# 2025-comprehensive-design/AudioLDM-with-LoRA

Hardware: AMD Instinct MI355X
Metric: unet_denoise_steps_per_sec (higher is better)
Workload: dtype bf16; 1 GPU; audioldm-s-full-v2 UNet + rank-4 LoRA (q,k,v,out), DDIM 200-step schedule, batch 4 x 10 s clips (latent 250x16), CFG 2.5 (UNet batch 8), bf16; per_gpu_batch=4, parallelism=prompt-sharded x1, hip_graph=True, graph_chains=1

## Files before the change

### audioldm_with_lora_amd/_lib.py

```python
import ctypes as C
import os

_HERE = os.path.dirname(os.path.abspath(__file__))
LIB_PATH = os.environ.get("ALDM_LIB") or os.path.join(_HERE, "libaldm_hip.so")

ACT_NONE, ACT_SILU, ACT_LRELU, ACT_TANH, ACT_GELU = 0, 1, 2, 3, 4
OUT_BF16, OUT_F32 = 0, 1
TILE_AUTO, TILE_128x128, TILE_64x64, TILE_128x64, TILE_64x128 = 0, 1, 2, 3, 4


class IgemmArgs(C.Structure):
    _fields_ = [
        ("x", C.c_void_p), ("x2", C.c_void_p),
        ("B", C.c_int), ("IH", C.c_int), ("IW", C.c_int), ("Cin", C.c_int), ("Cin2", C.c_int),
        ("UH", C.c_int), ("UW", C.c_int),
        ("in_dilate", C.c_int),
        ("w", C.c_void_p),
        ("Kpad", C.c_int),
        ("KH", C.c_int), ("KW", C.c_int), ("stride_h", C.c_int), ("stride_w", C.c_int),
        ("pad_h", C.c_int), ("pad_w", C.c_int), ("dil_h", C.c_int), ("dil_w", C.c_int),
        ("OH", C.c_int), ("OW", C.c_int), ("Cout", C.c_int),
        ("in_act", C.c_int), ("in_slope", C.c_float),
        ("ln_s", C.c_void_p), ("ln_sa", C.c_void_p), ("ln_ca", C.c_void_p), ("ln_eps", C.c_float),
        ("lora_a", C.c_void_p), ("lora_b", C.c_void_p),
        ("Rp", C.c_int),
        ("lora_t_out", C.c_void_p),
        ("bias", C.c_void_p), ("rowbias", C.c_void_p),
        ("rowbias_ld", C.c_int),
        ("geglu", C.c_int),
        ("out_act", C.c_int), ("out_slope", C.c_float),
        ("res", C.c_void_p), ("res2", C.c_void_p),
        ("alpha", C.c_float),
        ("post_act", C.c_int), ("post_slope", C.c_float), ("out2", C.c_void_p),
        ("out", C.c_void_p), ("out_dtype", C.c_int), ("out_ld", C.c_int),
        ("out_batch_stride", C.c_longlong),
        ("out_pix_stride", C.c_int), ("out_pix_offset", C.c_int),
        ("vt", C.c_void_p), ("vt_col0", C.c_int), ("vt_ld", C.c_int), ("vt_batch_stride", C.c_longlong),
        ("splits", C.c_int), ("workspace", C.c_void_p),
        ("tile", C.c_int),
        ("ring", C.c_int),
        ("defer_reduce", C.c_int),
        ("rowstat_out", C.c_void_p), ("ln_parts", C.c_void_p), ("ln_nparts", C.c_int),
        ("qstat_out", C.c_void_p),
        ("x3", C.c_void_p), ("x4", C.c_void_p), ("Cin3", C.c_int), ("Cin4", C.c_int),
        ("vt_dual", C.c_int),
        ("gnin_gamma", C.c_void_p), ("gnin_beta", C.c_void_p), ("gnin_q1", C.c_void_p), ("gnin_q2", C.c_void_p),
        ("gnin_bm1", C.c_int), ("gnin_tpi1", C.c_int), ("gnin_bm2", C.c_int), ("gnin_tpi2", C.c_int),
        ("gnin_groups", C.c_int), ("gnin_act", C.c_int), ("gnin_eps", C.c_float),
        ("xcd_map", C.c_int),
        ("lora_gate", C.c_void_p), ("gate_rows", C.c_int),
    ]


class PgemmArgs(C.Structure):
    _fields_ = [
        ("x", C.c_void_p), ("w", C.c_void_p),
        ("M", C.c_int), ("N", C.c_int), ("K", C.c_int),
        ("bias", C.c_void_p),
        ("ln_s", C.c_void_p), ("ln_sa", C.c_void_p), ("ln_ca", C.c_void_p), ("ln_eps", C.c_float),
        ("ln_parts", C.c_void_p), ("ln_nparts", C.c_int),
        ("lora_a", C.c_void_p), ("lora_b", C.c_void_p),
        ("Rp", C.c_int), ("ranks_used", C.c_int),
        ("geglu", C.c_int),
        ("res", C.c_void_p),
        ("out", C.c_void_p), ("out_ld", C.c_int),
        ("vt", C.c_void_p), ("vt_col0", C.c_int), ("vt_ld", C.c_int), ("vt_batch_stride", C.c_longlong), ("OHW", C.c_int),
        ("rowstat_out", C.c_void_p),
        ("mi", C.c_int), ("nt", C.c_int), ("tiles_per_range", C.c_int),
        ("max_ranges", C.c_int),
        ("waves", C.c_int),
        ("lora_t_out", C.c_void_p),
        ("vt_dual", C.c_int),
        ("lora_gate", C.c_void_p), ("gate_rows", C.c_int),
    ]


PROTOTYPES = {
    "aldm_version": (C.c_char_p, []),
    "aldm_last_error": (C.c_char_p, []),
    "aldm_igemm": (C.c_int, [C.POINTER(IgemmArgs), C.c_void_p]),
    "aldm_igemm_workspace_bytes": (C.c_size_t, [C.POINTER(IgemmArgs)]),
    "aldm_igemm_effective_splits": (C.c_int, [C.POINTER(IgemmArgs)]),
    "aldm_pgemm_supported": (C.c_int, [C.c_int]),
    "aldm_pgemm_plan": (C.c_int, [C.POINTER(PgemmArgs)]),
    "aldm_pgemm": (C.c_int, [C.POINTER(PgemmArgs), C.c_void_p]),
    "aldm_groupnorm_partials": (C.c_int, [C.c_void_p, C.c_int, C.c_int, C.c_int, C.c_int, C.c_void_p, C.c_void_p, C.c_int,
                                          C.c_void_p, C.c_void_p, C.c_void_p, C.c_int, C.c_int, C.c_float, C.c_void_p,
                                          C.c_void_p, C.c_int, C.c_void_p, C.c_void_p]),
    "aldm_groupnorm": (C.c_int, [C.c_void_p, C.c_void_p, C.c_int, C.c_int, C.c_int, C.c_int, C.c_int, C.c_float,
                                 C.c_void_p, C.c_void_p, C.c_int, C.c_void_p, C.c_void_p]),
    "aldm_groupnorm_apply": (C.c_int, [C.c_void_p, C.c_void_p, C.c_int, C.c_int, C.c_void_p, C.c_void_p, C.c_int, C.c_int, C.c_int,
                                       C.c_int, C.c_int, C.c_int, C.c_int, C.c_float, C.c_void_p, C.c_void_p, C.c_int, C.c_void_p,
                                       C.c_void_p, C.c_void_p]),
    "aldm_gn_silu_conv3x3_small": (C.c_int, [C.c_void_p, C.c_void_p, C.c_int, C.c_int, C.c_int, C.c_int, C.c_int, C.c_int, C.c_int, C.c_float,
                                             C.c_void_p, C.c_void_p, C.c_void_p, C.c_int, C.c_void_p, C.c_int, C.c_void_p, C.c_void_p]),
    "aldm_layernorm": (C.c_int, [C.c_void_p, C.c_int, C.c_int, C.c_void_p, C.c_void_p, C.c_float, C.c_void_p,
                                 C.c_void_p]),
    "aldm_attention": (C.c_int, [C.c_void_p, C.c_int, C.c_void_p, C.c_int, C.c_void_p, C.c_int, C.c_longlong,
                                 C.c_int, C.c_int, C.c_int, C.c_int, C.c_float, C.c_void_p, C.c_int, C.c_void_p]),
    "aldm_attention_prescaled": (C.c_int, [C.c_void_p, C.c_int, C.c_void_p, C.c_int, C.c_void_p, C.c_int, C.c_longlong,
                                           C.c_int, C.c_int, C.c_int, C.c_int, C.c_void_p, C.c_int, C.c_void_p]),
    "aldm_attn_block64": (C.c_int, [C.c_void_p, C.c_void_p, C.c_int, C.c_void_p, C.c_int, C.c_void_p, C.c_void_p, C.c_void_p, C.c_void_p,
                                    C.c_int, C.c_int, C.c_void_p, C.c_void_p, C.c_float, C.c_int, C.c_int, C.c_int, C.c_int, C.c_void_p,
                                    C.c_void_p]),
    "aldm_attn_block64_fp8": (C.c_int, [C.c_void_p, C.c_void_p, C.c_int, C.c_void_p, C.c_int, C.c_void_p, C.c_void_p, C.c_void_p, C.c_void_p,
                                    C.c_int, C.c_int, C.c_void_p, C.c_void_p, C.c_float, C.c_int, C.c_int, C.c_int, C.c_int, C.c_void_p,
                                    C.c_void_p]),
    "aldm_attn_block64_gated": (C.c_int, [C.c_void_p, C.c_void_p, C.c_int, C.c_void_p, C.c_int, C.c_void_p, C.c_void_p, C.c_void_p, C.c_void_p,
                                     C.c_int, C.c_int, C.c_void_p, C.c_void_p, C.c_float, C.c_int, C.c_int, C.c_int, C.c_int, C.c_void_p,
                                     C.c_void_p, C.c_void_p]),
    "aldm_attn_block64_fp8_gated": (C.c_int, [C.c_void_p, C.c_void_p, C.c_int, C.c_void_p, C.c_int, C.c_void_p, C.c_void_p, C.c_void_p, C.c_void_p,
                                     C.c_int, C.c_int, C.c_void_p, C.c_void_p, C.c_float, C.c_int, C.c_int, C.c_int, C.c_int, C.c_void_p,
                                     C.c_void_p, C.c_void_p]),
    "aldm_attn_block256_gated": (C.c_int, [C.c_void_p, C.c_void_p, C.c_int, C.c_void_p, C.c_int, C.c_void_p, C.c_void_p, C.c_void_p, C.c_void_p,
                                     C.c_int, C.c_int, C.c_void_p, C.c_void_p, C.c_float, C.c_int, C.c_int, C.c_int, C.c_int, C.c_void_p,
                                     C.c_void_p, C.c_void_p]),
    "aldm_attn_block256": (C.c_int, [C.c_void_p, C.c_void_p, C.c_int, C.c_void_p, C.c_int, C.c_void_p, C.c_void_p, C.c_void_p, C.c_void_p,
                                     C.c_int, C.c_int, C.c_void_p, C.c_void_p, C.c_float, C.c_int, C.c_int, C.c_int, C.c_int, C.c_void_p,
                                     C.c_void_p]),
    "aldm_hifigan_respair_supported": (C.c_int, [C.c_int, C.c_int, C.c_int]),
    "aldm_hifigan_respair": (C.c_int, [C.c_void_p, C.c_int, C.c_int, C.c_int, C.c_void_p, C.c_int, C.c_void_p, C.c_int, C.c_void_p, C.c_int,
                                       C.c_void_p, C.c_int, C.c_float, C.c_float, C.c_void_p, C.c_int, C.c_float, C.c_void_p, C.c_void_p]),
    "aldm_conv1d_to1": (C.c_int, [C.c_void_p, C.c_int, C.c_int, C.c_int, C.c_void_p, C.c_void_p, C.c_int, C.c_int, C.c_void_p, C.c_void_p]),
    "aldm_attention_wide": (C.c_int, [C.c_void_p, C.c_int, C.c_void_p, C.c_int, C.c_void_p, C.c_int, C.c_longlong,
                                      C.c_int, C.c_int, C.c_int, C.c_void_p, C.c_int, C.c_void_p]),
    "aldm_attention_fp8": (C.c_int, [C.c_void_p, C.c_int, C.c_void_p, C.c_int, C.c_void_p, C.c_int, C.c_longlong,
                                     C.c_int, C.c_int, C.c_int, C.c_int, C.c_float, C.c_void_p, C.c_int, C.c_void_p]),
    "aldm_attention_varlen": (C.c_int, [C.c_void_p, C.c_int, C.c_void_p, C.c_int, C.c_void_p, C.c_int, C.c_longlong,
                                        C.c_int, C.c_int, C.c_int, C.c_int, C.c_float, C.c_void_p, C.c_void_p, C.c_int,
                                        C.c_void_p]),
    "aldm_embed_layernorm": (C.c_int, [C.c_void_p, C.c_int, C.c_int, C.c_int, C.c_void_p, C.c_int, C.c_void_p, C.c_int,
                                       C.c_void_p, C.c_void_p, C.c_void_p, C.c_float, C.c_int, C.c_void_p, C.c_void_p]),
    "aldm_attention_lse": (C.c_int, [C.c_void_p, C.c_int, C.c_void_p, C.c_int, C.c_void_p, C.c_int, C.c_longlong,
                                     C.c_int, C.c_int, C.c_int, C.c_int, C.c_float, C.c_void_p, C.c_int, C.c_void_p,
                                     C.c_void_p]),
    "aldm_attention_bwd": (C.c_int, [C.c_void_p, C.c_void_p, C.c_void_p, C.c_int, C.c_void_p, C.c_void_p, C.c_void_p,
                                     C.c_int, C.c_longlong, C.c_longlong, C.c_longlong, C.c_void_p, C.c_void_p, C.c_int,
                                     C.c_void_p, C.c_void_p, C.c_int, C.c_int, C.c_int, C.c_int, C.c_float, C.c_void_p,
                                     C.c_void_p, C.c_void_p, C.c_int, C.c_void_p]),
    "aldm_groupnorm_bwd": (C.c_int, [C.c_void_p, C.c_void_p, C.c_void_p, C.c_int, C.c_int, C.c_int, C.c_int, C.c_int,
                                     C.c_float, C.c_void_p, C.c_void_p, C.c_int, C.c_void_p, C.c_void_p, C.c_void_p, C.c_void_p,
                                     C.c_void_p]),
    "aldm_groupnorm_bwd_partials": (C.c_int, [C.c_void_p, C.c_void_p, C.c_void_p, C.c_int, C.c_int, C.c_int, C.c_int, C.c_int,
                                              C.c_int, C.c_float, C.c_void_p, C.c_void_p, C.c_int, C.c_void_p, C.c_void_p,
                                              C.c_void_p, C.c_void_p, C.c_void_p]),
    "aldm_layernorm_bwd": (C.c_int, [C.c_void_p, C.c_void_p, C.c_int, C.c_int, C.c_void_p, C.c_float, C.c_void_p, C.c_void_p,
                                     C.c_void_p]),
    "aldm_geglu_fwd": (C.c_int, [C.c_void_p, C.c_longlong, C.c_int, C.c_void_p, C.c_void_p]),
    "aldm_geglu_bwd": (C.c_int, [C.c_void_p, C.c_void_p, C.c_longlong, C.c_int, C.c_void_p, C.c_void_p]),
    "aldm_add_bf16": (C.c_int, [C.c_void_p, C.c_void_p, C.c_longlong, C.c_void_p, C.c_void_p]),
    "aldm_upsample_nearest_bwd": (C.c_int, [C.c_void_p, C.c_int, C.c_int, C.c_int, C.c_int, C.c_int, C.c_int, C.c_void_p,
                                            C.c_void_p]),
    "aldm_tn_small": (C.c_int, [C.c_void_p, C.c_int, C.c_void_p, C.c_int, C.c_int, C.c_int, C.c_void_p, C.c_void_p]),
    "aldm_tn_batched": (C.c_int, [C.c_void_p, C.c_int, C.c_int, C.c_int, C.c_void_p]),
    "aldm_lora_pack": (C.c_int, [C.c_void_p, C.c_int, C.c_void_p]),
    "aldm_transpose_tokens": (C.c_int, [C.c_void_p, C.c_int, C.c_int, C.c_int, C.c_int, C.c_int, C.c_void_p, C.c_void_p]),
    "aldm_mse_grad": (C.c_int, [C.c_void_p, C.c_void_p, C.c_longlong, C.c_float, C.c_void_p, C.c_void_p, C.c_void_p]),
    "aldm_softmax_rows": (C.c_int, [C.c_void_p, C.c_int, C.c_int, C.c_int, C.c_float, C.c_void_p, C.c_int,
                                    C.c_void_p]),
    "aldm_timestep_embedding": (C.c_int, [C.c_void_p, C.c_int, C.c_int, C.c_int, C.c_void_p, C.c_void_p]),
    "aldm_silu": (C.c_int, [C.c_void_p, C.c_longlong, C.c_void_p, C.c_void_p]),
    "aldm_nchw_f32_to_nhwc": (C.c_int, [C.c_void_p, C.c_int, C.c_int, C.c_int, C.c_void_p, C.c_int, C.c_void_p]),
    "aldm_nhwc_to_nchw_f32": (C.c_int, [C.c_void_p, C.c_int, C.c_int, C.c_int, C.c_int, C.c_void_p, C.c_void_p]),
    "aldm_f32_to_bf16": (C.c_int, [C.c_void_p, C.c_longlong, C.c_float, C.c_void_p, C.c_void_p]),
    "aldm_cfg_ddim_step": (C.c_int, [C.c_void_p, C.c_void_p, C.c_int, C.c_longlong, C.c_int, C.c_float,
                                     C.c_void_p, C.c_void_p, C.c_void_p, C.c_void_p]),
    "aldm_ddim_step_fused": (C.c_int, [C.c_void_p, C.c_void_p, C.c_int, C.c_longlong, C.c_int, C.c_float, C.c_void_p, C.c_void_p, C.c_void_p,
                                       C.c_void_p, C.c_longlong, C.c_void_p, C.c_void_p, C.c_int, C.c_void_p, C.c_void_p, C.c_void_p]),
    "aldm_dpm_step_fused": (C.c_int, [C.c_void_p, C.c_void_p, C.c_int, C.c_longlong, C.c_int, C.c_float, C.c_void_p, C.c_void_p, C.c_void_p,
                                      C.c_void_p, C.c_void_p, C.c_longlong, C.c_void_p, C.c_void_p, C.c_int, C.c_void_p, C.c_void_p,
                                      C.c_void_p]),
# ... 67 lines not shown
```

### audioldm_with_lora_amd/csrc/igemm.hip

```cpp
#include "igemm_core.h"

using namespace aldm_igemm_detail;

int aldm_launch_tile_128x128(const IgemmDev& d, int Rp, bool vt, int ring, hipStream_t st);
int aldm_launch_tile_128x64(const IgemmDev& d, int Rp, bool vt, int ring, hipStream_t st);
int aldm_launch_tile_64x128(const IgemmDev& d, int Rp, bool vt, int ring, hipStream_t st);
int aldm_launch_tile_64x64(const IgemmDev& d, int Rp, bool vt, int ring, hipStream_t st);
int aldm_launch_tile_128x128w8(const IgemmDev& d, int Rp, bool vt, int ring, hipStream_t st);
int aldm_launch_tile_256x128w8(const IgemmDev& d, int Rp, bool vt, int ring, hipStream_t st);
int aldm_launch_tile_256x128ws(const IgemmDev& d, int Rp, bool vt, int ring, hipStream_t st);
int aldm_launch_tile_64x128ws(const IgemmDev& d, int Rp, bool vt, int ring, hipStream_t st);
int aldm_launch_tile_128x64ws(const IgemmDev& d, int Rp, bool vt, int ring, hipStream_t st);
int aldm_launch_tile_64x128w8(const IgemmDev& d, int Rp, bool vt, int ring, hipStream_t st);
int aldm_launch_tile_128x64w8(const IgemmDev& d, int Rp, bool vt, int ring, hipStream_t st);
int aldm_launch_halo(const IgemmDev& d, int tile, int ring, hipStream_t st);

static int pick_tile(int M, int N) {
  auto tiles = [&](int bm, int bn) { return (long long)cdiv(M, bm) * cdiv(N, bn); };
  if (N <= 64) return M >= 4096 ? ALDM_TILE_128x64 : ALDM_TILE_64x64;
  if (tiles(128, 128) >= 224) return ALDM_TILE_128x128;
  if (tiles(128, 64) >= 224) return ALDM_TILE_128x64;
  return ALDM_TILE_64x64;
}


extern "C" size_t aldm_igemm_workspace_bytes(const aldm_igemm_t* p) {
  if (!p || p->splits <= 1) return 0;
  const long long M = (long long)p->B * p->OH * p->OW;
  return (size_t)p->splits * M * p->Cout * sizeof(float);
}

extern "C" int aldm_igemm_effective_splits(const aldm_igemm_t* p) {
  if (!p || p->splits <= 1) return 1;
  const int nkt = cdiv(p->KH * p->KW * (p->Cin + p->Cin2), BK) + (p->x3 ? (p->Cin3 + (p->x4 ? p->Cin4 : 0)) / BK : 0);
  if (p->tile == ALDM_TILE_HALO_128x128 || p->tile == ALDM_TILE_HALO_64x128 || p->tile == ALDM_TILE_HALO_128x128_WS ||
      p->tile == ALDM_TILE_HALO_64x128_WS) {
    const int nch = (p->Cin + p->Cin2) / BK;
    return cdiv(nch, cdiv(nch, p->splits > nch ? nch : p->splits));
  }
  int splits = p->splits > nkt ? nkt : p->splits;
  const int per = cdiv(nkt, splits);
  return cdiv(nkt, per);
}

extern "C" int aldm_igemm(const aldm_igemm_t* p, void* stream) {
  ALDM_CHECK_ARG(p && p->x && p->w && p->out, "igemm: null x/w/out");
  ALDM_CHECK_ARG(p->B > 0 && p->IH > 0 && p->IW > 0 && p->OH > 0 && p->OW > 0 && p->Cout > 0, "igemm: bad dims");
  ALDM_CHECK_ARG(p->Cin > 0 && p->Cin % 8 == 0 && p->Cin2 >= 0 && p->Cin2 % 8 == 0, "igemm: Cin/Cin2 must be multiples of 8 (got %d,%d)", p->Cin, p->Cin2);
  ALDM_CHECK_ARG(p->Cin2 == 0 || p->x2, "igemm: Cin2 without x2");
  ALDM_CHECK_ARG(p->KH > 0 && p->KW > 0, "igemm: bad filter");
  const int Ctot = p->Cin + p->Cin2;
  const int Ktot = p->KH * p->KW * Ctot;
  const int Cext = p->x3 ? p->Cin3 + (p->x4 ? p->Cin4 : 0) : 0;
  ALDM_CHECK_ARG(p->Kpad % BK == 0 && p->Kpad >= Ktot + Cext, "igemm: Kpad %d must be a multiple of 64 and >= %d", p->Kpad, Ktot + Cext);
  ALDM_CHECK_ARG(!p->x3 || (p->Cin3 > 0 && p->Cin3 % 64 == 0 && (!p->x4 || (p->Cin4 > 0 && p->Cin4 % 64 == 0)) && Ktot % 64 == 0 &&
                            p->Cin % 64 == 0 && p->Cin2 % 64 == 0 && p->in_act == ALDM_ACT_NONE && !p->ln_s && !p->vt && !p->geglu &&
                            p->in_dilate == 0 && p->Rp == 0),
                 "igemm: the fused 1x1 second-source segment (x3 | x4) needs the plain LDS-DMA path: every channel count and KH*KW*(Cin+Cin2) a multiple of 64");
  ALDM_CHECK_ARG(p->x3 || !p->x4, "igemm: x4 without x3");
  ALDM_CHECK_ARG(!p->vt_dual || (p->vt && !p->res && !p->res2 && !p->out2 && p->out_act == ALDM_ACT_NONE && p->post_act == ALDM_ACT_NONE &&
                                 p->alpha == 1.f && !p->rowbias && p->out_dtype == ALDM_OUT_BF16),
                 "igemm: vt_dual needs vt and the plain bf16 epilogue (bias only)");
  ALDM_CHECK_ARG(p->Rp == 0 || p->Rp == 32 || p->Rp == 64, "igemm: Rp must be 0/32/64");
  ALDM_CHECK_ARG(p->Rp == 0 || (p->lora_a && p->lora_b), "igemm: Rp without lora_a/lora_b");
  ALDM_CHECK_ARG(!p->lora_gate || p->Rp, "igemm: lora_gate without an adapter");
  ALDM_CHECK_ARG(!p->lora_gate || p->Rp == 32, "igemm: lora_gate needs Rp == 32 (the gate table's width; got %d)", p->Rp);
  ALDM_CHECK_ARG(!p->lora_gate || !p->lora_t_out, "igemm: lora_t_out (the trainer's copy of T) is not combined with lora_gate");
  ALDM_CHECK_ARG(!p->lora_gate || (p->gate_rows > 0 && (p->B * p->OH * p->OW) % p->gate_rows == 0),
                 "igemm: lora_gate needs gate_rows > 0 dividing M (got %d rows per sample, M %d)", p->gate_rows, p->B * p->OH * p->OW);
  ALDM_CHECK_ARG(!p->geglu || (p->Cout % 32 == 0 && !p->rowbias), "igemm: GEGLU needs Cout %% 32 == 0");
  ALDM_CHECK_ARG(!p->vt || (p->vt_col0 % 16 == 0 && p->splits <= 1 && !p->geglu), "igemm: bad vt config");
  ALDM_CHECK_ARG(!p->vt || p->vt_col0 > 0 || p->out, "igemm: out required");
  ALDM_CHECK_ARG(p->splits <= 1 || (p->workspace && p->Cout % 4 == 0), "igemm: split-K needs workspace and Cout %% 4 == 0");
  ALDM_CHECK_ARG(p->out_ld > 0, "igemm: out_ld");
  ALDM_CHECK_ARG(!p->defer_reduce || (!p->geglu && !p->res2 && !p->out2 && p->out_act == ALDM_ACT_NONE && p->post_act == ALDM_ACT_NONE && p->alpha == 1.f),
                 "igemm: defer_reduce leaves bias / row bias / res to the consumer and supports nothing else in the epilogue");
  ALDM_CHECK_ARG(!(p->geglu && p->out2) || (p->Rp == 0 && p->splits <= 1 && !p->res && !p->res2 && p->out_dtype == ALDM_OUT_BF16 &&
                                            p->out_act == ALDM_ACT_NONE && p->post_act == ALDM_ACT_NONE && p->alpha == 1.f &&
                                            p->in_act == ALDM_ACT_NONE && p->Cin % 64 == 0 && p->Cin2 % 64 == 0 && p->Cout % 32 == 0),
                 "igemm: GEGLU with out2 (pre-activation copy) needs the plain LDS-DMA GEGLU launch (no residual / activation / split-K)");
  ALDM_CHECK_ARG(!p->ln_s || (p->KH == 1 && p->KW == 1 && p->Cin2 == 0 && p->splits <= 1 && (p->Rp == 0 || (p->ln_sa && p->ln_ca))),
                 "igemm: folded LayerNorm needs a 1x1 single-source GEMM without split-K (and ln_sa/ln_ca with LoRA)");
  ALDM_CHECK_ARG(!p->rowstat_out || (!p->vt && p->splits <= 1 && !p->geglu && p->out_dtype == ALDM_OUT_BF16 && p->Cout % 64 == 0 && !p->out2),
                 "igemm: rowstat_out needs the standard bf16 epilogue (no V^T / split-K / GEGLU / out2) and Cout %% 64 == 0");
  ALDM_CHECK_ARG(!p->qstat_out || (!p->vt && p->splits <= 1 && !p->geglu && p->out_dtype == ALDM_OUT_BF16 && p->Cout % 8 == 0 &&
                                   p->out_pix_stride <= 1 && p->Rp == 0 && !p->ln_s && !p->rowstat_out),
                 "igemm: qstat_out needs the standard bf16 epilogue (no V^T / split-K / GEGLU / LoRA / LayerNorm hand-over) and Cout %% 8 == 0");
  ALDM_CHECK_ARG(!p->ln_parts || (p->ln_s && p->ln_nparts > 0 && p->ln_nparts <= 64), "igemm: ln_parts needs ln_s and 1..64 partials per row");
  ALDM_CHECK_ARG(p->ring == 0 || (p->ring >= 2 && p->ring <= 4), "igemm: ring must be 0 (auto) or 2..4");
  ALDM_CHECK_ARG(p->in_dilate == 0 || (p->in_dilate == 2 && p->UH == 0), "igemm: in_dilate must be 0 or 2 (and excludes UH/UW)");

  IgemmDev d;
  d.x = (const bf16*)p->x; d.x2 = (const bf16*)p->x2; d.w = (const bf16*)p->w;
  d.lora_a = (const bf16*)p->lora_a; d.lora_b = (const bf16*)p->lora_b; d.lora_t_out = (bf16*)p->lora_t_out;
  d.bias = p->bias; d.rowbias = p->rowbias; d.res = (const bf16*)p->res; d.res2 = (const bf16*)p->res2;
  d.out = p->out; d.vt = (bf16*)p->vt; d.ws = p->workspace;
  d.B = p->B; d.IH = p->IH; d.IW = p->IW; d.Cin = p->Cin; d.Cin2 = p->Cin2; d.Ctot = Ctot; d.UH = p->UH; d.UW = p->UW; d.dilate = p->in_dilate;
  d.KH = p->KH; d.KW = p->KW; d.sh = p->stride_h; d.sw = p->stride_w; d.ph = p->pad_h; d.pw = p->pad_w;
  d.dh = p->dil_h; d.dw = p->dil_w;
  d.OH = p->OH; d.OW = p->OW; d.OHW = p->OH * p->OW; d.N = p->Cout; d.M = p->B * p->OH * p->OW; d.Kpad = p->Kpad;
  d.in_act = p->in_act; d.in_slope = p->in_slope;
  d.rowbias_ld = p->rowbias_ld; d.geglu = p->geglu; d.out_act = p->out_act; d.out_slope = p->out_slope;
  d.alpha = p->alpha;
  d.post_act = p->post_act; d.post_slope = p->post_slope; d.out2 = (bf16*)p->out2;
  d.out_f32 = p->out_dtype == ALDM_OUT_F32; d.out_ld = p->out_ld;
  d.out_bs = p->out_batch_stride; d.out_ps = p->out_pix_stride > 0 ? p->out_pix_stride : 1; d.out_po = p->out_pix_offset;
  d.vt_col0 = p->vt_col0; d.vt_ld = p->vt_ld; d.vt_bs = p->vt_batch_stride; d.vt_dual = p->vt ? p->vt_dual : 0;
  d.x3 = (const bf16*)p->x3; d.x4 = (const bf16*)p->x4; d.Cin3 = p->x3 ? p->Cin3 : 0; d.Cin4 = (p->x3 && p->x4) ? p->Cin4 : 0;
  d.C3tot = d.Cin3 + d.Cin4;
  d.nkt = cdiv(Ktot, BK) + d.C3tot / BK;
  d.splits = p->splits > 1 ? p->splits : 1;
  if (d.splits > d.nkt) d.splits = d.nkt;
  d.kt_per_split = cdiv(d.nkt, d.splits);
  d.splits = cdiv(d.nkt, d.kt_per_split);
  d.ws_rows = d.M;
  d.lora_gate = p->lora_gate; d.fd_gate = make_fastdiv((unsigned)(p->lora_gate ? p->gate_rows : 1)); d.gate_m1 = d.M - 1;
  d.tiles_n = 0; d.tiles_m = 0; d.nwg = 0;
  ALDM_CHECK_ARG(p->xcd_map >= 0 && p->xcd_map <= 2, "igemm: xcd_map must be 0 (auto), 1 (activation-stationary) or 2 (weight-stationary)");
  {
    const unsigned long long act = 2ull * p->B * p->IH * p->IW * Ctot + 2ull * p->B * p->OH * p->OW * Cext;
    const unsigned long long wgt = 2ull * p->Cout * p->Kpad;
    d.xmap = p->xcd_map ? p->xcd_map - 1 : ((wgt > act && p->splits <= 1) ? 1 : 0);
  }
  {
    const unsigned long long xb = 2ull * p->B * p->IH * p->IW * p->Cin, x2b = 2ull * p->B * p->IH * p->IW * p->Cin2;
    const unsigned long long wb = 2ull * p->Cout * p->Kpad, lb = 2ull * p->Rp * p->Kpad;
    ALDM_CHECK_ARG(wb < 0xFFFFFFFFull, "igemm: weight matrix too large for 32-bit offsets");
    const unsigned long long x3b = 2ull * p->B * p->OH * p->OW * d.Cin3, x4b = 2ull * p->B * p->OH * p->OW * d.Cin4;
    ALDM_CHECK_ARG(x3b < 0x80000000ull && x4b < 0x80000000ull, "igemm: x3 / x4 too large for 32-bit offsets");
    d.x3_bytes = (unsigned)x3b; d.x4_bytes = (unsigned)x4b;
    d.x_bytes = xb < 0xFFFFFFFFull ? (unsigned)xb : 0xFFFFFFFFu;
    d.x2_bytes = x2b < 0xFFFFFFFFull ? (unsigned)x2b : 0xFFFFFFFFu;
    d.w_bytes = (unsigned)wb;
    d.la_bytes = (unsigned)lb;
    d.lb_bytes = (unsigned)(2ull * p->Cout * p->Rp);
    d.fd_ohw = make_fastdiv((unsigned)d.OHW); d.fd_ow = make_fastdiv((unsigned)d.OW); d.fd_halo = make_fastdiv((unsigned)d.OW + 2u);
    d.fd_ctot = make_fastdiv((unsigned)d.Ctot); d.fd_kw = make_fastdiv((unsigned)d.KW);
    d.ln_s = p->ln_s; d.ln_sa = p->ln_sa; d.ln_ca = p->ln_ca; d.ln_eps = p->ln_eps;
    d.rowstat = p->rowstat_out; d.ln_parts = p->ln_parts; d.ln_np = p->ln_nparts;
    d.qstat = p->qstat_out; d.qtile = -1;
    d.gi_gamma = p->gnin_gamma; d.gi_beta = p->gnin_beta; d.gi_q1 = p->gnin_q1; d.gi_q2 = p->gnin_q2;
    d.gi_bm1 = p->gnin_bm1; d.gi_tpi1 = p->gnin_tpi1; d.gi_bm2 = p->gnin_bm2; d.gi_tpi2 = p->gnin_tpi2;
    d.gi_groups = p->gnin_groups; d.gi_act = p->gnin_act; d.gi_eps = p->gnin_eps;
#ifdef ALDM_DIAG
    d.diag = (p->splits <= 1) ? (unsigned long long*)p->workspace : nullptr;
#else
    d.diag = nullptr;
#endif
  }
  hipStream_t st = (hipStream_t)stream;

  int tile = p->tile ? p->tile : pick_tile(d.M, d.N);
  if (p->gnin_gamma) {
    ALDM_CHECK_ARG(tile == ALDM_TILE_HALO_128x128 || tile == ALDM_TILE_HALO_64x128 || tile == ALDM_TILE_HALO_128x128_WS || tile == ALDM_TILE_HALO_64x128_WS, "igemm: gnin_* (GroupNorm of the input inside the launch) needs a halo tile");
    const int Ct = p->Cin + p->Cin2;
    ALDM_CHECK_ARG(p->gnin_beta && p->gnin_q1 && (p->Cin2 == 0 || p->gnin_q2) && p->gnin_groups > 0 && p->gnin_groups <= 64 && Ct % p->gnin_groups == 0 &&
                   (Ct / p->gnin_groups) % 4 == 0 && Ct <= 512 && p->UH == 0 &&
                   (p->gnin_tpi1 > 0 || (p->gnin_bm1 > 0 && p->gnin_bm1 <= p->IH * p->IW)) &&
                   (p->Cin2 == 0 || p->gnin_tpi2 > 0 || (p->gnin_bm2 > 0 && p->gnin_bm2 <= p->IH * p->IW)) &&
                   (p->gnin_act == ALDM_ACT_NONE || p->gnin_act == ALDM_ACT_SILU),
                   "igemm: gnin_*: tables for every source, group width a multiple of 4, at most 512 input channels, no up-sampling, act NONE / SILU");
  }
  const bool vt = p->vt != nullptr;
  int rc;
  switch (tile) {
    case ALDM_TILE_128x128: rc = aldm_launch_tile_128x128(d, p->Rp, vt, p->ring, st); break;
    case ALDM_TILE_128x64: rc = aldm_launch_tile_128x64(d, p->Rp, vt, p->ring, st); break;
    case ALDM_TILE_64x128: rc = aldm_launch_tile_64x128(d, p->Rp, vt, p->ring, st); break;
    case ALDM_TILE_64x64: rc = aldm_launch_tile_64x64(d, p->Rp, vt, p->ring, st); break;
    case ALDM_TILE_128x128_W8: rc = aldm_launch_tile_128x128w8(d, p->Rp, vt, p->ring, st); break;
    case ALDM_TILE_256x128_W8: rc = aldm_launch_tile_256x128w8(d, p->Rp, vt, p->ring, st); break;
    case ALDM_TILE_256x128_WS: rc = aldm_launch_tile_256x128ws(d, p->Rp, vt, p->ring, st); break;
    case ALDM_TILE_64x128_WS: rc = aldm_launch_tile_64x128ws(d, p->Rp, vt, p->ring, st); break;
    case ALDM_TILE_128x64_WS: rc = aldm_launch_tile_128x64ws(d, p->Rp, vt, p->ring, st); break;
    case ALDM_TILE_64x128_W8: rc = aldm_launch_tile_64x128w8(d, p->Rp, vt, p->ring, st); break;
    case ALDM_TILE_128x64_W8: rc = aldm_launch_tile_128x64w8(d, p->Rp, vt, p->ring, st); break;
    case ALDM_TILE_HALO_128x128:
    case ALDM_TILE_HALO_64x128:
    case ALDM_TILE_HALO_128x128_WS:
    case ALDM_TILE_HALO_64x128_WS:
      if (p->Rp || vt || p->rowstat_out || (p->x3 && tile != ALDM_TILE_HALO_128x128_WS && tile != ALDM_TILE_HALO_64x128_WS)) {
        aldm_set_error("igemm: the halo tiles take no LoRA / V^T / row statistics (and a second-source segment only in the wave-specialised forms)");
        return ALDM_E_UNSUPPORTED;
      }
      if (d.splits > 1) {
        const int nch = (d.Cin + d.Cin2) / BK;
        const int cps = cdiv(nch, d.splits > nch ? nch : d.splits);
        d.kt_per_split = d.KH * d.KW * cps;
        d.splits = cdiv(nch, cps);
      }
      rc = aldm_launch_halo(d, tile, p->ring, st);
      break;
    default: aldm_set_error("igemm: unknown tile %d", tile); return ALDM_E_UNSUPPORTED;
  }
  if (rc != ALDM_OK) return rc;
  if (d.splits > 1 && !p->defer_reduce) {
    const int ncols = d.geglu ? d.N / 2 : d.N;
    const long long work = (long long)d.M * (ncols / 4);
    hipLaunchKernelGGL(igemm_reduce_kernel, dim3((unsigned)cdivll(work, 256)), dim3(256), 0, st, d);
    return aldm_launch_status("igemm_reduce");
  }
  return ALDM_OK;
}
```

### audioldm_with_lora_amd/csrc/igemm_core.h

```cpp
#pragma once
#include <type_traits>

#include "common.h"

namespace aldm_igemm_detail {

constexpr int BK = 64;
constexpr int THREADS = 256;

struct FastDiv { unsigned mul, shift; };
__device__ __forceinline__ int fdiv(int n, FastDiv d) {
  return (int)(((unsigned long long)__umulhi((unsigned)n, d.mul) + (unsigned)n) >> d.shift);
}
static inline FastDiv make_fastdiv(unsigned d) {
  FastDiv f;
  unsigned s = 0;
  while ((1ull << s) < d) ++s;
  f.shift = s;
  f.mul = (unsigned)((((1ull << s) - d) << 32) / d + 1);
  return f;
}

struct IgemmDev {
  const bf16* x; const bf16* x2; const bf16* w; const bf16* lora_a; const bf16* lora_b;
  bf16* lora_t_out;
  const float* bias; const float* rowbias; const bf16* res; const bf16* res2;
  void* out; bf16* vt; float* ws;
  int B, IH, IW, Cin, Cin2, Ctot, UH, UW, dilate;
  int KH, KW, sh, sw, ph, pw, dh, dw;
  int OH, OW, OHW, N, M, Kpad;
  int in_act; float in_slope;
  int rowbias_ld, geglu, out_act; float out_slope; float alpha;
  int post_act; float post_slope; bf16* out2;
  int out_f32, out_ld; long long out_bs; int out_ps, out_po;
  int vt_col0, vt_ld; long long vt_bs; int vt_dual;
  int splits, kt_per_split, nkt;
  int tiles_n;
  int tiles_m, nwg, xmap;
  FastDiv fd_tiles_m, fd_splits;
  unsigned x_bytes, x2_bytes, w_bytes, la_bytes, lb_bytes;
  unsigned long long* diag;
  FastDiv fd_ohw, fd_ow, fd_halo;
  FastDiv fd_tiles_n, fd_ctot, fd_kw;
  const float* ln_s; const float* ln_sa; const float* ln_ca; float ln_eps;
  const bf16* x3; const bf16* x4; int Cin3, Cin4, C3tot; unsigned x3_bytes, x4_bytes;
  float* qstat; int qtile;
  float* rowstat;
  const float* ln_parts; int ln_np;
  const float* gi_gamma; const float* gi_beta; const float* gi_q1; const float* gi_q2;
  int gi_bm1, gi_tpi1, gi_bm2, gi_tpi2, gi_groups, gi_act; float gi_eps;
  int ws_rows;
  const float* lora_gate;
  FastDiv fd_gate;
  int gate_m1;
};

__device__ __forceinline__ int swz(int row, int chunk) { return chunk ^ ((row >> 1) & 7); }

__device__ __forceinline__ void igemm_work_item(const IgemmDev& p, int& tile_m, int& tile_n, int& split) {
  const int nwg = p.nwg, bid = blockIdx.x;
  const int xcd = bid & 7, q = nwg >> 3, r = nwg & 7;
  const int w = (xcd < r ? xcd * (q + 1) : r * (q + 1) + (xcd - r) * q) + (bid >> 3);
  if (p.xmap) {
    const int sn = fdiv(w, p.fd_tiles_m);
    tile_m = w - sn * p.tiles_m;
    split = fdiv(sn, p.fd_tiles_n);
    tile_n = sn - split * p.tiles_n;
  } else {
    const int t = fdiv(w, p.fd_splits);
    split = w - t * p.splits;
    tile_m = fdiv(t, p.fd_tiles_n);
    tile_n = t - tile_m * p.tiles_n;
  }
}

__device__ __forceinline__ void igemm_gate4(const IgemmDev& p, f32x4& t, int m, int col, int rp) {
  const int mm = m < p.gate_m1 ? m : p.gate_m1;
  const f32x4 g = *reinterpret_cast<const f32x4*>(p.lora_gate + (long long)fdiv(mm, p.fd_gate) * rp + col);
#pragma unroll
  for (int e = 0; e < 4; ++e) t[e] *= g[e];
}

__device__ __forceinline__ void finish_store4(const IgemmDev& p, int m, int n, int ncols, float* v) {
  const int b = m / p.OHW;
  const int pix = m - b * p.OHW;
  const long long row = (long long)b * p.out_bs + (long long)(pix * p.out_ps + p.out_po) * p.out_ld;
  const bool vec = (n + 3 < ncols) && ((p.out_ld & 3) == 0) && ((p.out_bs & 3) == 0);
#pragma unroll
  for (int j = 0; j < 4; ++j) v[j] = apply_act(v[j], p.out_act, p.out_slope);
  if (p.res) {
    if (vec) {
      bf16x4 r = *reinterpret_cast<const bf16x4*>(p.res + row + n);
#pragma unroll
      for (int j = 0; j < 4; ++j) v[j] += (float)r[j];
    } else {
      for (int j = 0; j < 4; ++j) if (n + j < ncols) v[j] += (float)p.res[row + n + j];
    }
  }
#pragma unroll
  for (int j = 0; j < 4; ++j) v[j] *= p.alpha;
  if (p.res2) {
    if (vec) {
      bf16x4 r = *reinterpret_cast<const bf16x4*>(p.res2 + row + n);
#pragma unroll
      for (int j = 0; j < 4; ++j) v[j] += (float)r[j];
    } else {
      for (int j = 0; j < 4; ++j) if (n + j < ncols) v[j] += (float)p.res2[row + n + j];
    }
  }
  if (p.out2) {
    bf16* o2 = p.out2 + row + n;
    if (vec) {
      *reinterpret_cast<bf16x4*>(o2) = bf16x4{(bf16)apply_act(v[0], p.post_act, p.post_slope), (bf16)apply_act(v[1], p.post_act, p.post_slope),
                                              (bf16)apply_act(v[2], p.post_act, p.post_slope), (bf16)apply_act(v[3], p.post_act, p.post_slope)};
    } else {
      for (int j = 0; j < 4; ++j) if (n + j < ncols) o2[j] = (bf16)apply_act(v[j], p.post_act, p.post_slope);
    }
  } else if (p.post_act) {
#pragma unroll
    for (int j = 0; j < 4; ++j) v[j] = apply_act(v[j], p.post_act, p.post_slope);
  }
  if (p.out_f32) {
    float* o = reinterpret_cast<float*>(p.out) + row + n;
    if (vec) {
      *reinterpret_cast<f32x4*>(o) = f32x4{v[0], v[1], v[2], v[3]};
    } else {
      for (int j = 0; j < 4; ++j) if (n + j < ncols) o[j] = v[j];
    }
  } else {
    bf16* o = reinterpret_cast<bf16*>(p.out) + row + n;
    if (vec) {
      *reinterpret_cast<bf16x4*>(o) = bf16x4{(bf16)v[0], (bf16)v[1], (bf16)v[2], (bf16)v[3]};
    } else {
      for (int j = 0; j < 4; ++j) if (n + j < ncols) o[j] = (bf16)v[j];
    }
  }
}

// ... 19 lines not shown

__device__ __forceinline__ void epi8(const IgemmDev& p, int m, int n, int ncols, float* v) {
  const int b = fdiv(m, p.fd_ohw);
  const int pix = m - b * p.OHW;
  const long long row = (long long)b * p.out_bs + (long long)(pix * p.out_ps + p.out_po) * p.out_ld;
  const bool vec = (n + 7 < ncols) && ((p.out_ld & 7) == 0) && ((p.out_bs & 7) == 0);
  if (p.out_act) {
#pragma unroll
    for (int j = 0; j < 8; ++j) v[j] = apply_act(v[j], p.out_act, p.out_slope);
  }
  if (p.res) {
    if (vec) {
      const bf16x8 r = *reinterpret_cast<const bf16x8*>(p.res + row + n);
#pragma unroll
      for (int j = 0; j < 8; ++j) v[j] += (float)r[j];
    } else {
      for (int j = 0; j < 8; ++j) if (n + j < ncols) v[j] += (float)p.res[row + n + j];
    }
  }
#pragma unroll
  for (int j = 0; j < 8; ++j) v[j] *= p.alpha;
  if (p.res2) {
    if (vec) {
      const bf16x8 r = *reinterpret_cast<const bf16x8*>(p.res2 + row + n);
#pragma unroll
      for (int j = 0; j < 8; ++j) v[j] += (float)r[j];
    } else {
      for (int j = 0; j < 8; ++j) if (n + j < ncols) v[j] += (float)p.res2[row + n + j];
    }
  }
  if (p.out2) {
    bf16* o2 = p.out2 + row + n;
    if (vec) {
      bf16x8 t;
#pragma unroll
      for (int j = 0; j < 8; ++j) t[j] = (bf16)apply_act(v[j], p.post_act, p.post_slope);
      *reinterpret_cast<bf16x8*>(o2) = t;
    } else {
      for (int j = 0; j < 8; ++j) if (n + j < ncols) o2[j] = (bf16)apply_act(v[j], p.post_act, p.post_slope);
    }
  } else if (p.post_act) {
#pragma unroll
    for (int j = 0; j < 8; ++j) v[j] = apply_act(v[j], p.post_act, p.post_slope);
  }
  if (p.out_f32) {
    float* o = reinterpret_cast<float*>(p.out) + row + n;
    if (vec) {
      *reinterpret_cast<f32x4*>(o) = f32x4{v[0], v[1], v[2], v[3]};
      *reinterpret_cast<f32x4*>(o + 4) = f32x4{v[4], v[5], v[6], v[7]};
    } else {
      for (int j = 0; j < 8; ++j) if (n + j < ncols) o[j] = v[j];
    }
  } else {
    bf16* o = reinterpret_cast<bf16*>(p.out) + row + n;
    if (vec) {
      bf16x8 t;
#pragma unroll
      for (int j = 0; j < 8; ++j) t[j] = (bf16)v[j];
      *reinterpret_cast<bf16x8*>(o) = t;
    } else {
      for (int j = 0; j < 8; ++j) if (n + j < ncols) o[j] = (bf16)v[j];
    }
  }
}

template <int BM, int BN>
struct EpiCfg {
  static constexpr int LD = BN + 4;
  static constexpr int LDT = BM + 4;
  static constexpr int BYTES = (BM * LD > BN * LDT ? BM * LD : BN * LDT) * 4;
};

template <int BM, int BN, int MI, int NI, bool VT, int NT = 256, int EPI = 0>
__device__ __forceinline__ void igemm_epilogue(const IgemmDev& p, f32x4 (&acc)[MI][NI], char* smem, bool vt_wg, int m0,
                                               int n0, int wm_off, int wn_off, int lrow, int lq, int split, int tid,
                                               const float* lnst = nullptr) {
  using E = EpiCfg<BM, BN>;
  constexpr bool LEAN = EPI == 1 || EPI == 4, GLEAN = EPI == 2, SLEAN = EPI == 3;
  constexpr bool QS = EPI == 0 || EPI == 4;
#ifndef ALDM_NO_KA_PREFETCH
  aldm_prefetch_next_kernargs<sizeof(IgemmDev)>(tid);
#endif
  if constexpr (SLEAN) {
#pragma unroll
    for (int i = 0; i < MI; ++i) {
      const int m = m0 + wm_off + i * 16 + lrow;
#pragma unroll
      for (int j = 0; j < NI; ++j) {
        const int n = n0 + wn_off + j * 16 + lq * 4;
        if (m < p.M && n < p.N) *reinterpret_cast<f32x4*>(p.ws + ((long long)split * p.ws_rows + m) * p.N + n) = acc[i][j];
      }
    }
    return;
  }
  float* Cs = reinterpret_cast<float*>(smem);
  if constexpr (LEAN && !VT) lnst = nullptr;

  constexpr int GPR = BN / 8, RSTEP = NT / GPR, ITERS = BM / RSTEP, CH = ITERS < 4 ? ITERS : 4;
  static_assert(NT % GPR == 0 && BM % RSTEP == 0 && ITERS % CH == 0, "epilogue row walk");
  const int r0 = tid / GPR, c = (tid % GPR) * 8, n = n0 + c;
  const bool dual = VT && vt_wg && p.vt_dual;
  const bool std_path = !GLEAN && !SLEAN && (!(VT && vt_wg) || dual) && (LEAN || (p.splits <= 1 && !p.geglu));
  const bool vec = (n + 7 < p.N) && ((p.out_ld & 7) == 0) && ((p.out_bs & 7) == 0);
  const bool rbvec = vec && ((p.rowbias_ld & 3) == 0);
  float colb[8], lns[8];
  long long rowo[CH];
  bool ok[CH];
  f32x4 rb0[CH], rb1[CH];
  bf16x8 r1[CH], r2[CH];
  int slot[CH];
  float qacc[2][2][2] = {{{0.f, 0.f}, {0.f, 0.f}}, {{0.f, 0.f}, {0.f, 0.f}}};
  const int qb0 = (QS && p.qstat) ? fdiv(min(m0, p.M - 1), p.fd_ohw) : 0;
  auto phaseA = [&](int it0) {
#pragma unroll
    for (int u = 0; u < CH; ++u) {
      const int m = m0 + r0 + (it0 + u) * RSTEP;
      ok[u] = m < p.M;
      rb0[u] = rb1[u] = f32x4{0.f, 0.f, 0.f, 0.f};
      r1[u] = r2[u] = bf16x8{0, 0, 0, 0, 0, 0, 0, 0};
      rowo[u] = 0;
      slot[u] = 0;
      if (!ok[u]) continue;
      const int b = fdiv(m, p.fd_ohw);
      const int pix = m - b * p.OHW;
      slot[u] = b != qb0;
      rowo[u] = (long long)b * p.out_bs + (long long)(pix * p.out_ps + p.out_po) * p.out_ld;
      if (p.rowbias) {
        const float* rb = p.rowbias + (long long)b * p.rowbias_ld + n;
        if (rbvec) {
          rb0[u] = *reinterpret_cast<const f32x4*>(rb);
          rb1[u] = *reinterpret_cast<const f32x4*>(rb + 4);
        } else {
#pragma unroll
          for (int q = 0; q < 4; ++q) {
            if (n + q < p.N) rb0[u][q] = rb[q];
            if (n + 4 + q < p.N) rb1[u][q] = rb[4 + q];
          }
        }
      }
      if (vec) {
        if (p.res) r1[u] = *reinterpret_cast<const bf16x8*>(p.res + rowo[u] + n);
        if (p.res2) r2[u] = *reinterpret_cast<const bf16x8*>(p.res2 + rowo[u] + n);
      } else {
#pragma unroll
        for (int q = 0; q < 8; ++q) {
          if (p.res && n + q < p.N) r1[u][q] = p.res[rowo[u] + n + q];
          if (p.res2 && n + q < p.N) r2[u][q] = p.res2[rowo[u] + n + q];
        }
      }
    }
  };
  auto phaseB = [&](auto ACT, int it0) {
    constexpr bool kAct = decltype(ACT)::value;
#pragma unroll
    for (int u = 0; u < CH; ++u) {
      if (!ok[u]) continue;
      const int r = r0 + (it0 + u) * RSTEP;
      float v[8];
      if (VT && vt_wg) {
#pragma unroll
        for (int q = 0; q < 8; ++q) v[q] = Cs[(c + q) * E::LDT + r];
      } else {
        const float* src = Cs + r * E::LD + c;
#pragma unroll
        for (int q = 0; q < 8; ++q) v[q] = src[q];
      }
      if (lnst) {
        const float mu = lnst[r], rs = lnst[BM + r];
#pragma unroll
        for (int q = 0; q < 8; ++q) v[q] = rs * (v[q] - mu * lns[q]);
      }
#pragma unroll
      for (int q = 0; q < 4; ++q) { v[q] += colb[q] + rb0[u][q]; v[4 + q] += colb[4 + q] + rb1[u][q]; }
// ... 68 lines not shown
  if (std_path && n < p.N) {
#pragma unroll
    for (int q = 0; q < 8; ++q) colb[q] = lns[q] = 0.f;
    if (n + 7 < p.N) {
      if (p.bias) {
        const f32x4 b0 = *reinterpret_cast<const f32x4*>(p.bias + n), b1 = *reinterpret_cast<const f32x4*>(p.bias + n + 4);
#pragma unroll
        for (int q = 0; q < 4; ++q) { colb[q] = b0[q]; colb[4 + q] = b1[q]; }
      }
      if (lnst) {
        const f32x4 s0 = *reinterpret_cast<const f32x4*>(p.ln_s + n), s1 = *reinterpret_cast<const f32x4*>(p.ln_s + n + 4);
#pragma unroll
        for (int q = 0; q < 4; ++q) { lns[q] = s0[q]; lns[4 + q] = s1[q]; }
      }
    } else {
      for (int q = 0; q < 8; ++q) {
        if (p.bias && n + q < p.N) colb[q] = p.bias[n + q];
        if (lnst && n + q < p.N) lns[q] = p.ln_s[n + q];
      }
    }
    phaseA(0);
  }

  __syncthreads();
  if (VT && vt_wg) {
#pragma unroll
    for (int i = 0; i < MI; ++i)
#pragma unroll
      for (int j = 0; j < NI; ++j)
        *reinterpret_cast<f32x4*>(Cs + (wn_off + j * 16 + lrow) * E::LDT + wm_off + i * 16 + lq * 4) = acc[i][j];
  } else {
#pragma unroll
    for (int i = 0; i < MI; ++i)
#pragma unroll
      for (int j = 0; j < NI; ++j)
        *reinterpret_cast<f32x4*>(Cs + (wm_off + i * 16 + lrow) * E::LD + wn_off + j * 16 + lq * 4) = acc[i][j];
  }
  __syncthreads();

  if (VT && vt_wg) {
    for (int g = tid; g < BN * (BM / 8); g += NT) {
      const int rn = g / (BM / 8), cm = (g - rn * (BM / 8)) * 8;
      const int n = n0 + rn, m = m0 + cm;
      if (n >= p.N || m >= p.M) continue;
      const float bb = p.bias ? p.bias[n] : 0.f;
      const float lsn = lnst ? p.ln_s[n] : 0.f;
      const float* src = Cs + rn * E::LDT + cm;
      const int b = fdiv(m, p.fd_ohw), pix = m - b * p.OHW;
      bf16* o = p.vt + (long long)b * p.vt_bs + (long long)(n - p.vt_col0) * p.vt_ld + pix;
      if (m + 7 < p.M && pix + 7 < p.OHW && ((p.vt_ld & 7) == 0) && ((pix & 7) == 0) && ((p.vt_bs & 7) == 0)) {
        bf16x8 t;
        float mu8[8], rs8[8];
        if (lnst) {
          const f32x4 m0v = *reinterpret_cast<const f32x4*>(lnst + cm), m1v = *reinterpret_cast<const f32x4*>(lnst + cm + 4);
          const f32x4 r0v = *reinterpret_cast<const f32x4*>(lnst + BM + cm), r1v = *reinterpret_cast<const f32x4*>(lnst + BM + cm + 4);
#pragma unroll
          for (int q = 0; q < 4; ++q) { mu8[q] = m0v[q]; mu8[4 + q] = m1v[q]; rs8[q] = r0v[q]; rs8[4 + q] = r1v[q]; }
        } else {
#pragma unroll
          for (int q = 0; q < 8; ++q) { mu8[q] = 0.f; rs8[q] = 1.f; }
        }
#pragma unroll
        for (int q = 0; q < 8; ++q) t[q] = (bf16)(rs8[q] * (src[q] - mu8[q] * lsn) + bb);
        *reinterpret_cast<bf16x8*>(o) = t;
      } else {
        for (int q = 0; q < 8; ++q) {
          const int mq = m + q;
          if (mq >= p.M) break;
          const int bq = fdiv(mq, p.fd_ohw), pq = mq - bq * p.OHW;
          float val = src[q];
          if (lnst) val = lnst[BM + cm + q] * (val - lnst[cm + q] * lsn);
          p.vt[(long long)bq * p.vt_bs + (long long)(n - p.vt_col0) * p.vt_ld + pq] = (bf16)(val + bb);
        }
      }
    }
    if (!dual) return;
  }
  if constexpr (!LEAN) {
  if (!GLEAN && (SLEAN || p.splits > 1)) {
    for (int g = tid; g < BM * (BN / 8); g += NT) {
      const int r = g / (BN / 8), c = (g - r * (BN / 8)) * 8;
      const int m = m0 + r, n = n0 + c;
      if (m >= p.M || n >= p.N) continue;
      float* o = p.ws + ((long long)split * p.ws_rows + m) * p.N + n;
      const float* src = Cs + r * E::LD + c;
      if (n + 7 < p.N) {
        *reinterpret_cast<f32x4*>(o) = *reinterpret_cast<const f32x4*>(src);
        *reinterpret_cast<f32x4*>(o + 4) = *reinterpret_cast<const f32x4*>(src + 4);
      } else {
        for (int q = 0; q < 8; ++q) if (n + q < p.N) o[q] = src[q];
      }
    }
    return;
  }
  if (!SLEAN && (GLEAN || p.geglu)) {
    constexpr int CG = BN / 16, RS = NT / CG;
    static_assert(NT % CG == 0 && BM % RS == 0, "GEGLU row walk");
    const int jo = (tid % CG) * 8;
    const int cv = ((jo >> 4) << 5) + (jo & 15);
    const int nv = n0 + cv;
    if (nv >= p.N) return;
    float bv[8], bg[8], sv[8], sg[8];
#pragma unroll
    for (int q = 0; q < 8; ++q) bv[q] = bg[q] = sv[q] = sg[q] = 0.f;
    if (p.bias) {
      const f32x4 a0 = *reinterpret_cast<const f32x4*>(p.bias + nv), a1 = *reinterpret_cast<const f32x4*>(p.bias + nv + 4);
      const f32x4 g0 = *reinterpret_cast<const f32x4*>(p.bias + nv + 16), g1 = *reinterpret_cast<const f32x4*>(p.bias + nv + 20);
#pragma unroll
      for (int q = 0; q < 4; ++q) { bv[q] = a0[q]; bv[4 + q] = a1[q]; bg[q] = g0[q]; bg[4 + q] = g1[q]; }
    }
    if (lnst) {
      const f32x4 a0 = *reinterpret_cast<const f32x4*>(p.ln_s + nv), a1 = *reinterpret_cast<const f32x4*>(p.ln_s + nv + 4);
      const f32x4 g0 = *reinterpret_cast<const f32x4*>(p.ln_s + nv + 16), g1 = *reinterpret_cast<const f32x4*>(p.ln_s + nv + 20);
#pragma unroll
      for (int q = 0; q < 4; ++q) { sv[q] = a0[q]; sv[4 + q] = a1[q]; sg[q] = g0[q]; sg[4 + q] = g1[q]; }
    }
    for (int r = tid / CG; r < BM; r += RS) {
      const int m = m0 + r;
      if (m >= p.M) break;
      const float* src = Cs + r * E::LD + cv;
      const float mu = lnst ? lnst[r] : 0.f, rs = lnst ? lnst[BM + r] : 1.f;
      float val[8], gate[8], v[8];
#pragma unroll
      for (int q = 0; q < 8; ++q) {
        val[q] = rs * (src[q] - mu * sv[q]) + bv[q];
        gate[q] = rs * (src[16 + q] - mu * sg[q]) + bg[q];
        v[q] = val[q] * gelu_erf_f(gate[q]);
      }
      if constexpr (GLEAN) {
        if (p.out2) {
          bf16* hrow = p.out2 + (long long)m * p.N + nv;
          bf16x8 hv, hg;
#pragma unroll
          for (int q = 0; q < 8; ++q) { hv[q] = (bf16)val[q]; hg[q] = (bf16)gate[q]; }
          *reinterpret_cast<bf16x8*>(hrow) = hv;
          *reinterpret_cast<bf16x8*>(hrow + 16) = hg;
        }
        const int b = fdiv(m, p.fd_ohw), pix = m - b * p.OHW, no = (n0 >> 1) + jo, ncols = p.N >> 1;
        bf16* o = reinterpret_cast<bf16*>(p.out) + (long long)b * p.out_bs + (long long)(pix * p.out_ps + p.out_po) * p.out_ld + no;
        bf16x8 t;
#pragma unroll
        for (int q = 0; q < 8; ++q) t[q] = (bf16)v[q];
        if (no + 7 < ncols && ((p.out_ld & 7) == 0) && ((p.out_bs & 7) == 0)) *reinterpret_cast<bf16x8*>(o) = t;
        else
          for (int q = 0; q < 8; ++q) if (no + q < ncols) o[q] = t[q];
      } else {
        epi8(p, m, (n0 >> 1) + jo, p.N >> 1, v);
      }
    }
    return;
  }
  }
  if (n >= p.N) return;
  if (!LEAN && (p.out_act | p.post_act)) {
    phaseB(std::true_type{}, 0);
#pragma unroll
    for (int it0 = CH; it0 < ITERS; it0 += CH) {
      phaseA(it0);
      phaseB(std::true_type{}, it0);
    }
  } else {
    phaseB(std::false_type{}, 0);
#pragma unroll
    for (int it0 = CH; it0 < ITERS; it0 += CH) {
      phaseA(it0);
      phaseB(std::false_type{}, it0);
    }
  }
// ... 755 lines not shown
```

### audioldm_with_lora_amd/csrc/norm.hip

```cpp
#include <cstdlib>
#include "common.h"
#include "gn_stats.h"

namespace {

constexpr int GN_THREADS = 512;
constexpr int GN_MAXCG = 256;
constexpr int GN_LDS_QUADS = 16384;

__device__ __forceinline__ float block_sum(float v, float* red, int tid, int nthreads) {
  v = wave_sum(v);
  __syncthreads();
  if ((tid & 63) == 0) red[tid >> 6] = v;
  __syncthreads();
  float t = 0.f;
  for (int i = 0; i < nthreads / 64; ++i) t += red[i];
  return t;
}

__device__ __forceinline__ void block_sum_pair(float& a, float& b, float* red, int tid, int nthreads) {
  a = wave_sum(a);
  b = wave_sum(b);
  __syncthreads();
  const int nw = nthreads / 64;
// ... 51 lines not shown
    const int pix = aldm_div(q, dqpp), j = q - pix * qpp;
    const int c = c0 + 4 * j;
    bf16x4 o;
#pragma unroll
    for (int k = 0; k < 4; ++k) {
      const float gm = gamma[c + k] * rstd;
      float t = ((float)v[k] - mean) * gm + beta[c + k];
      if (act == ALDM_ACT_SILU) t = silu_f(t);
      o[k] = (bf16)t;
    }
    *reinterpret_cast<bf16x4*>(y + ((long long)b * HW + pix) * C + c) = o;
  }
}

template <int QPT>
__global__ __launch_bounds__(GN_THREADS) void groupnorm_reg_kernel(const bf16* __restrict__ x, const bf16* __restrict__ x2,
                                                                   int HW, int C1, int C2, int groups, float eps,
                                                                   const float* __restrict__ gamma,
                                                                   const float* __restrict__ beta, int act,
                                                                   bf16* __restrict__ y, AldmDiv dqpp) {
  aldm_touch_kernargs<96>();
#ifndef ALDM_NO_KA_PREFETCH
  aldm_prefetch_next_kernargs<96>(threadIdx.x);
#endif
  __shared__ float red[2 * GN_THREADS / 64];
  __shared__ __attribute__((aligned(16))) float sgm[GN_MAXCG], sbt[GN_MAXCG];
  const int C = C1 + C2;
  const int Cg = C / groups, qpp = Cg >> 2;
  const int nb = gridDim.x / groups;
  const int g = blockIdx.x / nb, b = blockIdx.x - g * nb;
  const int c0 = g * Cg;
  const int nquads = HW * qpp;
  const int tid = threadIdx.x;
  if (tid < Cg) { sgm[tid] = gamma[c0 + tid]; sbt[tid] = beta[c0 + tid]; }
  const float pivot = (float)((c0 < C1) ? x[(long long)b * HW * C1 + c0] : x2[(long long)b * HW * C2 + (c0 - C1)]);

  bf16x4 v[QPT];
  float s = 0.f;
#pragma unroll
  for (int i = 0; i < QPT; ++i) {
    const int q = tid + i * GN_THREADS;
    bf16x4 t = {0, 0, 0, 0};
    if (q < nquads) {
      const int pix = aldm_div(q, dqpp), j = q - pix * qpp;
      const int c = c0 + 4 * j;
      t = (c < C1) ? *reinterpret_cast<const bf16x4*>(x + ((long long)b * HW + pix) * C1 + c)
                   : *reinterpret_cast<const bf16x4*>(x2 + ((long long)b * HW + pix) * C2 + (c - C1));
    }
    v[i] = t;
  }
  float ss = 0.f;
#pragma unroll
  for (int i = 0; i < QPT; ++i) {
    if (tid + i * GN_THREADS < nquads) {
#pragma unroll
      for (int k = 0; k < 4; ++k) { const float d = (float)v[i][k] - pivot; s += d; ss = fmaf(d, d, ss); }
    }
  }
  const float n = (float)nquads * 4.f;
  block_sum_pair(s, ss, red, tid, GN_THREADS);
  const float dm = s / n;
  const float mean = pivot + dm;
  const float rstd = rsqrtf(fmaxf(ss / n - dm * dm, 0.f) + eps);
#pragma unroll
  for (int i = 0; i < QPT; ++i) {
    const int q = tid + i * GN_THREADS;
    if (q < nquads) {
      const int pix = aldm_div(q, dqpp), j = q - pix * qpp;
      const int c = c0 + 4 * j;
      const f32x4 gm = *reinterpret_cast<const f32x4*>(sgm + 4 * j);
      const f32x4 bt = *reinterpret_cast<const f32x4*>(sbt + 4 * j);
      bf16x4 o;
#pragma unroll
      for (int k = 0; k < 4; ++k) {
        float t = ((float)v[i][k] - mean) * (gm[k] * rstd) + bt[k];
        if (act == ALDM_ACT_SILU) t = silu_f(t);
        o[k] = (bf16)t;
      }
      *reinterpret_cast<bf16x4*>(y + ((long long)b * HW + pix) * C + c) = o;
    }
  }
}

template <int QPT>
__global__ __launch_bounds__(GN_THREADS) void groupnorm_partials_kernel(const float* __restrict__ ws, int splits, long long sstride,
                                                                        int HW, int C, int groups, float eps,
                                                                        const float* __restrict__ bias,
                                                                        const float* __restrict__ rowbias, int rowbias_ld,
                                                                        const bf16* __restrict__ res, bf16* __restrict__ sum_out,
                                                                        const bf16* __restrict__ x2, int C2,
                                                                        const float* __restrict__ gamma,
                                                                        const float* __restrict__ beta, int act,
                                                                        bf16* __restrict__ y, AldmDiv dqpp) {
  aldm_touch_kernargs<160>();
#ifndef ALDM_NO_KA_PREFETCH
  aldm_prefetch_next_kernargs<160>(threadIdx.x);
#endif
  __shared__ float red[2 * GN_THREADS / 64];
  __shared__ __attribute__((aligned(16))) float sgm[GN_MAXCG], sbt[GN_MAXCG], sadd[GN_MAXCG];
  const int Ct = C + C2;
  const int Cg = Ct / groups, qpp = Cg >> 2;
  const int nb = gridDim.x / groups;
  const int g = blockIdx.x / nb, b = blockIdx.x - g * nb;
  const int c0 = g * Cg;
  const int nquads = HW * qpp;
  const int tid = threadIdx.x;
  if (tid < Cg) {
    const int c = c0 + tid;
    sgm[tid] = gamma[c];
    sbt[tid] = beta[c];
    float a = 0.f;
    if (c < C) {
      if (bias) a = bias[c];
      if (rowbias) a += rowbias[(long long)b * rowbias_ld + c];
    }
    sadd[tid] = a;
  }

  f32x4 v[QPT];
  bf16x4 rv[QPT];
  long long off[QPT], yoff[QPT];
  int ch[QPT];
  const bool second = c0 >= C;
#pragma unroll
  for (int i = 0; i < QPT; ++i) {
    const int q = tid + i * GN_THREADS;
    const int qq = q < nquads ? q : 0;
    const int pix = aldm_div(qq, dqpp), j = qq - pix * qpp;
    ch[i] = c0 + 4 * j;
    off[i] = ((long long)b * HW + pix) * C + ch[i];
    yoff[i] = ((long long)b * HW + pix) * Ct + ch[i];
    v[i] = f32x4{0.f, 0.f, 0.f, 0.f};
    rv[i] = bf16x4{0, 0, 0, 0};
    if (second) {
      if (q < nquads) rv[i] = *reinterpret_cast<const bf16x4*>(x2 + ((long long)b * HW + pix) * C2 + (ch[i] - C));
    } else if (res && q < nquads) {
      rv[i] = *reinterpret_cast<const bf16x4*>(res + off[i]);
    }
  }
  if (second) splits = 0;
  int sp = 0;
  for (; sp + 4 <= splits; sp += 4) {
#pragma unroll
    for (int i = 0; i < QPT; ++i) {
      if (tid + i * GN_THREADS < nquads) {
        const float* w0 = ws + off[i] + sp * sstride;
        const f32x4 a0 = *reinterpret_cast<const f32x4*>(w0), a1 = *reinterpret_cast<const f32x4*>(w0 + sstride);
        const f32x4 a2 = *reinterpret_cast<const f32x4*>(w0 + 2 * sstride), a3 = *reinterpret_cast<const f32x4*>(w0 + 3 * sstride);
#pragma unroll
        for (int k = 0; k < 4; ++k) v[i][k] = (((v[i][k] + a0[k]) + a1[k]) + a2[k]) + a3[k];
      }
    }
  }
  if (sp < splits) {
    const int rem = splits - sp;
#pragma unroll
    for (int i = 0; i < QPT; ++i) {
      if (tid + i * GN_THREADS < nquads) {
        const float* w0 = ws + off[i] + sp * sstride;
        const f32x4 a0 = *reinterpret_cast<const f32x4*>(w0);
        const f32x4 a1 = *reinterpret_cast<const f32x4*>(w0 + (rem > 1 ? 1 : 0) * sstride);
        const f32x4 a2 = *reinterpret_cast<const f32x4*>(w0 + (rem > 2 ? 2 : 0) * sstride);
        v[i] += a0;
        if (rem > 1) v[i] += a1;
        if (rem > 2) v[i] += a2;
      }
    }
  }
  __syncthreads();
  const float pivot = sadd[0];
  float s = 0.f, ss = 0.f;
#pragma unroll
  for (int i = 0; i < QPT; ++i) {
    if (tid + i * GN_THREADS < nquads) {
      const int c = ch[i];
      if (!second) v[i] += *reinterpret_cast<const f32x4*>(sadd + (c - c0));
      if (second || res) {
#pragma unroll
        for (int k = 0; k < 4; ++k) v[i][k] += (float)rv[i][k];
      }
      if (sum_out && !second) {
        bf16x4 o;
#pragma unroll
        for (int k = 0; k < 4; ++k) o[k] = (bf16)v[i][k];
        *reinterpret_cast<bf16x4*>(sum_out + off[i]) = o;
      }
#pragma unroll
      for (int k = 0; k < 4; ++k) { const float d = v[i][k] - pivot; s += d; ss = fmaf(d, d, ss); }
    }
  }
  const float n = (float)nquads * 4.f;
  block_sum_pair(s, ss, red, tid, GN_THREADS);
  const float dm = s / n;
  const float mean = pivot + dm;
  const float rstd = rsqrtf(fmaxf(ss / n - dm * dm, 0.f) + eps);
#pragma unroll
  for (int i = 0; i < QPT; ++i) {
    if (tid + i * GN_THREADS < nquads) {
      const int c = ch[i];
      const f32x4 gm = *reinterpret_cast<const f32x4*>(sgm + (c - c0));
      const f32x4 bt = *reinterpret_cast<const f32x4*>(sbt + (c - c0));
      bf16x4 o;
#pragma unroll
      for (int k = 0; k < 4; ++k) {
        float t = (v[i][k] - mean) * (gm[k] * rstd) + bt[k];
        if (act == ALDM_ACT_SILU) t = silu_f(t);
        o[k] = (bf16)t;
      }
      *reinterpret_cast<bf16x4*>(y + yoff[i]) = o;
    }
  }
}

constexpr int LN_MAXC = 4;
template <int LPR>
__device__ __forceinline__ float row_sum(float v) {
#pragma unroll
  for (int o = LPR / 2; o > 0; o >>= 1) v += __shfl_xor(v, o, 64);
  return v;
}
template <int LPR>
__global__ __launch_bounds__(256) void layernorm_kernel(const bf16* __restrict__ x, int M, int C,
                                                        const float* __restrict__ gamma,
                                                        const float* __restrict__ beta, float eps,
                                                        bf16* __restrict__ y) {
  constexpr int RPW = 64 / LPR;
  const int lane = threadIdx.x & (LPR - 1);
  const int row = (blockIdx.x * (blockDim.x >> 6) + (threadIdx.x >> 6)) * RPW + ((threadIdx.x & 63) / LPR);
  const bool live = row < M;
  const int nch = C >> 3;
  const bf16* xr = x + (long long)(live ? row : 0) * C;
  bf16x8 v[LN_MAXC];
  f32x4 g0[LN_MAXC], g1[LN_MAXC], b0[LN_MAXC], b1[LN_MAXC];
  float s = 0.f;
#pragma unroll
  for (int i = 0; i < LN_MAXC; ++i) {
    const int ch = lane + LPR * i;
    if (ch < nch) {
      v[i] = *reinterpret_cast<const bf16x8*>(xr + ch * 8);
      g0[i] = *reinterpret_cast<const f32x4*>(gamma + ch * 8); g1[i] = *reinterpret_cast<const f32x4*>(gamma + ch * 8 + 4);
      b0[i] = *reinterpret_cast<const f32x4*>(beta + ch * 8); b1[i] = *reinterpret_cast<const f32x4*>(beta + ch * 8 + 4);
    }
// ... 228 lines not shown
  __syncthreads();
  {
    const int gA = c / Cg, gB = (c + 4) / Cg;
    const float mA = sm[gA], rA = sr[gA], mB = sm[gB], rB = sr[gB];
    const f32x4 g0 = *reinterpret_cast<const f32x4*>(gamma + c), g1 = *reinterpret_cast<const f32x4*>(gamma + c + 4);
    const f32x4 b0 = *reinterpret_cast<const f32x4*>(beta + c), b1 = *reinterpret_cast<const f32x4*>(beta + c + 4);
    float sc[8], sh[8];
#pragma unroll
    for (int k = 0; k < 4; ++k) {
      sc[k] = g0[k] * rA; sh[k] = b0[k] - mA * sc[k];
      sc[4 + k] = g1[k] * rB; sh[4 + k] = b1[k] - mB * sc[4 + k];
    }
#pragma unroll
    for (int j = 0; j < PPT; ++j) {
      const int pl = (tid >> 4) + 16 * j;
      const int rowi = pl / GC_W, col = pl % GC_W;
      bf16x8 o;
#pragma unroll
      for (int k = 0; k < 8; ++k) o[k] = inimg[j] ? (bf16)silu_f(fmaf((float)v[j][k], sc[k], sh[k])) : (bf16)0.f;
      *reinterpret_cast<bf16x8*>(Xs + (rowi * (GC_W + 2) + col + 1) * GC_PIX + cu * 16) = o;
    }
  }
  __syncthreads();
  const int m = lane & 15, q = lane >> 4;
  f32x4 acc[2] = {f32x4{0.f, 0.f, 0.f, 0.f}, f32x4{0.f, 0.f, 0.f, 0.f}};
  const bf16x8 zero8 = {0, 0, 0, 0, 0, 0, 0, 0};
#pragma unroll
  for (int tap = 0; tap < 9; ++tap) {
    const int dy = tap / 3, dx = tap % 3;
#pragma unroll
    for (int ks = 0; ks < C / 32; ++ks) {
      const bf16x8 wf = m < Cout ? *reinterpret_cast<const bf16x8*>(Ws + m * WROW + (tap * C + ks * 32 + q * 8) * 2) : zero8;
#pragma unroll
      for (int t = 0; t < 2; ++t) {
        const int rowi = 2 * wave + t + dy;
        const bf16x8 xf = *reinterpret_cast<const bf16x8*>(Xs + (rowi * (GC_W + 2) + m + dx) * GC_PIX + (ks * 32 + q * 8) * 2);
        acc[t] = __builtin_amdgcn_mfma_f32_16x16x32_bf16(xf, wf, acc[t], 0, 0, 0);
      }
    }
  }
  if (m < Cout) {
    const float bb = bias ? bias[m] : 0.f;
#pragma unroll
    for (int t = 0; t < 2; ++t) {
      const int row = r0 + 2 * wave + t;
      if (row < H) {
#pragma unroll
        for (int i = 0; i < 4; ++i)
          out[((long long)b * HW + (long long)row * GC_W + 4 * q + i) * Cout + m] = acc[t][i] + bb;
      }
    }
  }
}

}

extern "C" int aldm_groupnorm(const void* x, const void* x2, int B, int HW, int C1, int C2, int groups, float eps,
                              const float* gamma, const float* beta, int act, void* y, void* stream) {
  ALDM_CHECK_ARG(x && y && gamma && beta, "groupnorm: null pointer");
  ALDM_CHECK_ARG(B > 0 && HW > 0 && C1 > 0 && C2 >= 0 && groups > 0, "groupnorm: bad dims");
  const int C = C1 + C2;
  ALDM_CHECK_ARG(C % groups == 0 && (C / groups) % 4 == 0 && C1 % 4 == 0, "groupnorm: group width %d / C1 %d must be multiples of 4", C / groups, C1);
  ALDM_CHECK_ARG(C2 == 0 || x2, "groupnorm: C2 without x2");
  const size_t lds = (size_t)GN_LDS_QUADS * 8 + 64;
  static unsigned long long attr_done = 0;
  if (int rc = aldm_set_max_lds(reinterpret_cast<const void*>(groupnorm_kernel), (int)lds, &attr_done, "groupnorm")) return rc;
  const long long nquads = (long long)HW * (C / groups / 4);
  const AldmDiv dq = aldm_make_div((unsigned)(C / groups / 4));
#define ALDM_GN_REG(QPT)                                                                                               \
  hipLaunchKernelGGL(groupnorm_reg_kernel<QPT>, dim3(B * groups), dim3(GN_THREADS), 0, (hipStream_t)stream,            \
                     (const bf16*)x, (const bf16*)x2, HW, C1, C2, groups, eps, gamma, beta, act, (bf16*)y, dq)
  const bool reg_ok = C / groups <= GN_MAXCG;
  if (reg_ok && nquads <= 4 * GN_THREADS) ALDM_GN_REG(4);
  else if (reg_ok && nquads <= 8 * GN_THREADS) ALDM_GN_REG(8);
  else if (reg_ok && nquads <= 16 * GN_THREADS) ALDM_GN_REG(16);
  else if (reg_ok && nquads <= 32 * GN_THREADS) ALDM_GN_REG(32);
  else
    hipLaunchKernelGGL(groupnorm_kernel, dim3(B * groups), dim3(GN_THREADS), lds, (hipStream_t)stream, (const bf16*)x,
                       (const bf16*)x2, HW, C1, C2, groups, eps, gamma, beta, act, (bf16*)y, dq);
#undef ALDM_GN_REG
  return aldm_launch_status("groupnorm");
}

extern "C" int aldm_groupnorm_partials(const float* ws, int splits, int B, int HW, int C, const float* bias,
                                       const float* rowbias, int rowbias_ld, const void* res, void* sum_out,
                                       const void* x2, int C2, int groups, float eps, const float* gamma, const float* beta,
                                       int act, void* y, void* stream) {
  ALDM_CHECK_ARG(ws && y && gamma && beta && splits >= 1, "groupnorm_partials: null pointer / bad splits");
  ALDM_CHECK_ARG(B > 0 && HW > 0 && C > 0 && C2 >= 0 && groups > 0 && (C2 == 0 || x2), "groupnorm_partials: bad dims");
  const int Ct = C + C2;
  ALDM_CHECK_ARG(Ct % groups == 0 && (Ct / groups) % 4 == 0 && C % (Ct / groups) == 0,
                 "groupnorm_partials: group width %d must be a multiple of 4 and divide the first source's %d channels", Ct / groups, C);
  ALDM_CHECK_ARG(!rowbias || rowbias_ld >= C, "groupnorm_partials: rowbias_ld");
  ALDM_CHECK_ARG(Ct / groups <= GN_MAXCG, "groupnorm_partials: at most %d channels per group", GN_MAXCG);
  const long long nquads = (long long)HW * (Ct / groups / 4);
  ALDM_CHECK_ARG(nquads <= 8 * GN_THREADS, "groupnorm_partials: strip of %lld quads exceeds the register-resident limit %d", nquads, 8 * GN_THREADS);
  const AldmDiv dq = aldm_make_div((unsigned)(Ct / groups / 4));
  const long long sstride = (long long)B * HW * C;
#define ALDM_GNP(QPT)                                                                                                  \
  hipLaunchKernelGGL(groupnorm_partials_kernel<QPT>, dim3(B * groups), dim3(GN_THREADS), 0, (hipStream_t)stream, ws,   \
                     splits, sstride, HW, C, groups, eps, bias, rowbias, rowbias_ld, (const bf16*)res, (bf16*)sum_out,        \
                     (const bf16*)x2, C2, gamma, beta, act, (bf16*)y, dq)
  if (nquads <= GN_THREADS) ALDM_GNP(1);
  else if (nquads <= 2 * GN_THREADS) ALDM_GNP(2);
  else if (nquads <= 4 * GN_THREADS) ALDM_GNP(4);
  else ALDM_GNP(8);
#undef ALDM_GNP
  return aldm_launch_status("groupnorm_partials");
}

extern "C" int aldm_layernorm(const void* x, int M, int C, const float* gamma, const float* beta, float eps, void* y,
                              void* stream) {
  ALDM_CHECK_ARG(x && y && gamma && beta && M > 0, "layernorm: null pointer / bad M");
  ALDM_CHECK_ARG(C % 8 == 0 && C <= 64 * 8 * LN_MAXC, "layernorm: C=%d must be a multiple of 8 and <= %d", C, 64 * 8 * LN_MAXC);
  if (C <= 256)
    hipLaunchKernelGGL(layernorm_kernel<32>, dim3(cdiv(M, 8)), dim3(256), 0, (hipStream_t)stream, (const bf16*)x, M, C, gamma,
                       beta, eps, (bf16*)y);
  else
    hipLaunchKernelGGL(layernorm_kernel<64>, dim3(cdiv(M, 4)), dim3(256), 0, (hipStream_t)stream, (const bf16*)x, M, C, gamma,
                       beta, eps, (bf16*)y);
  return aldm_launch_status("layernorm");
}

extern "C" int aldm_embed_layernorm(const long long* ids, int B, int L, int C, const float* word, int vocab,
                                    const float* pos, int npos, const float* type0, const float* gamma,
                                    const float* beta, float eps, int pad_idx, void* y, void* stream) {
  ALDM_CHECK_ARG(ids && word && pos && type0 && gamma && beta && y && B > 0 && L > 0, "embed_layernorm: null pointer / bad dims");
  ALDM_CHECK_ARG(C % 8 == 0 && C <= 64 * 8 * LN_MAXC, "embed_layernorm: C=%d must be a multiple of 8 and <= %d", C, 64 * 8 * LN_MAXC);
  ALDM_CHECK_ARG(vocab > 0 && npos > pad_idx + 1 && L + pad_idx + 1 <= npos, "embed_layernorm: %d tokens do not fit %d positions (pad %d)", L, npos, pad_idx);
  const int M = B * L;
  hipLaunchKernelGGL(embed_layernorm_kernel, dim3(cdiv(M, 4)), dim3(256), 0, (hipStream_t)stream, ids, M, L, C, word, vocab,
                     pos, npos, type0, gamma, beta, eps, pad_idx, (bf16*)y);
  return aldm_launch_status("embed_layernorm");
}

static int gn_apply_bytes() {
  static const int v = getenv("ALDM_GN_APPLY_BYTES") ? atoi(getenv("ALDM_GN_APPLY_BYTES")) : 32768;
  return v;
}

extern "C" int aldm_groupnorm_apply(const void* x, const float* qstat, int bm, int tpi, const void* x2, const float* qstat2, int bm2,
                                    int tpi2, int B, int HW, int C1, int C2, int groups, float eps, const float* gamma,
                                    const float* beta, int act, void* y, float* stat_ws, void* stream) {
  ALDM_CHECK_ARG(x && qstat && y && gamma && beta, "groupnorm_apply: null pointer");
  ALDM_CHECK_ARG(B > 0 && HW > 0 && C1 > 0 && C2 >= 0 && groups > 0 && groups <= 64 && (C2 == 0 || (x2 && qstat2)), "groupnorm_apply: bad dims");
  const int C = C1 + C2;
  ALDM_CHECK_ARG(C % groups == 0 && (C / groups) % 4 == 0 && C1 % 8 == 0 && C2 % 8 == 0,
                 "groupnorm_apply: group width %d must be a multiple of 4; C1 = %d, C2 = %d multiples of 8", C / groups, C1, C2);
  ALDM_CHECK_ARG(C / 8 <= 256, "groupnorm_apply: at most 2048 channels (a workgroup walks %d 16-byte units per pixel with 256 threads)", C / 8);
  ALDM_CHECK_ARG((tpi > 0 || (bm > 0 && bm <= HW)) && (C2 == 0 || tpi2 > 0 || (bm2 > 0 && bm2 <= HW)),
                 "groupnorm_apply: an M-tile of the producer may span at most two images (tile rows <= H*W)");
  int lpg = 1;
  while (lpg * 2 * groups <= 256 && lpg < 64) lpg *= 2;
  int pxb = 16;
  while (pxb < 256 && pxb * C * 2 < gn_apply_bytes()) pxb *= 2;
  GnSrc s1{(const bf16*)x, qstat, C1, bm, tpi}, s2{(const bf16*)x2, qstat2, C2, bm2, tpi2};
  const int tiles = max(tpi > 0 ? tpi : HW / bm + 1, C2 ? (tpi2 > 0 ? tpi2 : HW / bm2 + 1) : 0);
  const bool two_phase = stat_ws && tiles >= ALDM_GN_FINALIZE_MIN_TILES;
  if (two_phase) {
    hipLaunchKernelGGL(groupnorm_finalize_kernel, dim3(B), dim3(256), 0, (hipStream_t)stream, s1, s2, HW, groups, eps, lpg, stat_ws);
    if (int rc = aldm_launch_status("groupnorm_finalize")) return rc;
  }
  hipLaunchKernelGGL(groupnorm_apply_kernel, dim3(cdiv(HW, pxb), B), dim3(256), 0, (hipStream_t)stream, s1, s2, HW, groups, eps, gamma,
                     beta, act, (bf16*)y, pxb, lpg, aldm_make_div((unsigned)(C >> 3)), two_phase ? (const float*)stat_ws : nullptr);
  return aldm_launch_status("groupnorm_apply");
}

extern "C" int aldm_gn_silu_conv3x3_small(const void* x, const float* qstat, int bm, int tpi, int B, int H, int W, int C, int groups,
                                          float eps, const float* gamma, const float* beta, const void* w, int w_ld, const float* bias,
                                          int Cout, float* out, void* stream) {
  ALDM_CHECK_ARG(x && qstat && gamma && beta && w && out, "gn_silu_conv3x3_small: null pointer");
  ALDM_CHECK_ARG(B > 0 && H > 0 && W == GC_W && C == 128 && Cout >= 1 && Cout <= 16 && w_ld >= 9 * C && w_ld % 8 == 0,
                 "gn_silu_conv3x3_small: built for W = 16, C = 128, Cout <= 16 (got W %d, C %d, Cout %d)", W, C, Cout);
  ALDM_CHECK_ARG(groups > 0 && groups <= 64 && C % groups == 0 && (C / groups) % 4 == 0, "gn_silu_conv3x3_small: bad groups");
  ALDM_CHECK_ARG(tpi > 0 || (bm > 0 && bm <= H * W), "gn_silu_conv3x3_small: an M-tile of the producer may span at most two images");
  int lpg = 1;
  while (lpg * 2 * groups <= 256 && lpg < 64) lpg *= 2;
  const int lds = (GC_RB + 2) * (GC_W + 2) * GC_PIX + 16 * (9 * 128 * 2 + 16);
  auto kern = gn_silu_conv3x3_small_kernel<128>;
  static unsigned long long attr_done = 0;
  if (int rc = aldm_set_max_lds(reinterpret_cast<const void*>(kern), lds, &attr_done, "gn_silu_conv3x3_small")) return rc;
  GnSrc s1{(const bf16*)x, qstat, C, bm, tpi};
  hipLaunchKernelGGL(kern, dim3(cdiv(H, GC_RB), B), dim3(256), lds, (hipStream_t)stream, s1, H, groups, eps, gamma, beta, (const bf16*)w, w_ld,
                     bias, Cout, out, lpg);
  return aldm_launch_status("gn_silu_conv3x3_small");
}
```

### audioldm_with_lora_amd/ops.py

```python
import ctypes as C
import json
import math
import os
import sys
from dataclasses import dataclass
from typing import Optional

import torch

from . import _lib
from ._lib import (ACT_GELU, ACT_LRELU, ACT_NONE, ACT_SILU, ACT_TANH, OUT_BF16, OUT_F32, IgemmArgs, check)

BK = 64


def _stream():
    return C.c_void_p(torch.cuda.current_stream().cuda_stream)


def _p(t: Optional[torch.Tensor]):
    return None if t is None else C.c_void_p(t.data_ptr())


def _require_gpu(t):
# ... 161 lines not shown
    fit = ((160 * 1024) // per_cu - extra) // stage
    want = 4 if nwg <= 512 else (2 if ktiles <= 24 else 3)
    return max(2, min(want, fit))


TILE_DIMS = {1: (128, 128), 2: (64, 64), 3: (128, 64), 4: (64, 128), 6: (128, 128), 7: (128, 128), 8: (64, 128), 9: (256, 128), 10: (64, 128), 11: (128, 64), 12: (256, 128), 13: (64, 128), 14: (128, 64), 15: (128, 128), 16: (64, 128)}
HALO_ROWS = {7: 320, 8: 128, 15: 320, 16: 128}


def halo_tiles(OW, eligible):
    if not eligible:
        return []
    return [t for t in (7, 8, 15, 16) if TILE_DIMS[t][0] % OW == 0 and (TILE_DIMS[t][0] // OW + 2) * (OW + 2) <= HALO_ROWS[t]]

TUNED_PATH = os.path.join(os.path.dirname(os.path.abspath(__file__)), "tuned_gfx950.json")
TUNED = {}
TUNED_LEGACY_KEYS = False
TUNER = None
if os.path.exists(TUNED_PATH) and os.environ.get("ALDM_NO_TUNED") != "1":
    with open(TUNED_PATH) as _f:
        TUNED = {k: tuple(v) for k, v in json.load(_f)["igemm"].items()}
if os.environ.get("ALDM_TUNED_PATCH"):
    with open(os.environ["ALDM_TUNED_PATCH"]) as _f:
        TUNED.update({k: tuple(v) for k, v in json.load(_f).items()})
TUNED_LEGACY_KEYS = any(" k3x3 " in k and " ow" not in k for k in TUNED)


def tune_key(M, N, c1, c2, kh, kw, stride, up, dilate, rp, vt, geglu, ln, fast, ow=None, pad=None, dil=None):
    key = (f"M{M} N{N} C{c1}+{c2} k{kh}x{kw} s{stride[0]} up{int(up)} d{dilate} r{rp} vt{int(vt)} g{int(bool(geglu))} "
           f"ln{int(ln)} f{int(fast)}")
    if ow is not None and (kh > 1 or kw > 1):
        key += f" ow{ow} p{pad[0]}x{pad[1]} dl{dil[0]}x{dil[1]}"
    return key


def heuristic_cfg(M, pw, ktiles, can_split, fast_path, has_vt, splits=None):
    if splits is None:
        splits = auto_splits(M, pw.N, ktiles) if can_split else 1
    tile = _lib.TILE_64x64 if pw.Rp else pick_tile(M, pw.N)
    if tile == 6 and (not fast_path or has_vt or ktiles < 16):
        tile = _lib.TILE_128x64
    bm, bn = TILE_DIMS[tile]
    nwg = math.ceil(M / bm) * math.ceil(pw.N / bn) * max(1, splits)
    return tile, pick_ring(tile, bm, bn, pw.Rp, nwg, ktiles), splits


class Tuner:

    def __init__(self, shortlist=5, reps=4, verbose=False):
        self.shortlist, self.reps, self.verbose = shortlist, reps, verbose
        self.cands = {}
        self.times = {}
        self.slot = None

    def isolated(self, a, key, M, pw, ktiles, can_split, forced_splits, fast_path, has_vt, device, halo=()):
        lib = _lib.load()
        default = heuristic_cfg(M, pw, ktiles, can_split, fast_path, has_vt, forced_splits)
        cands = []
        for t in [2, 3, 1, 4] + ([6] if (fast_path and not has_vt and ktiles >= 8) else []) + (
                [9, 12] if (fast_path and not has_vt and not pw.Rp and ktiles >= 8 and M >= 32768 and pw.N % 128 == 0 and pw.ln_s is None
                            and not pw.geglu and not pw.Cext) else []) + (
                [10, 11] if (fast_path and not has_vt and not pw.Rp and ktiles >= 8 and M <= 8192) else []) + (
                [13, 14] if (fast_path and not has_vt and not pw.Rp and ktiles >= 8 and M <= 8192 and pw.ln_s is None and not pw.geglu) else []):
            bm, bn = TILE_DIMS[t]
            if has_vt and a.vt_col0 % bn:
                continue
            base = math.ceil(M / bm) * math.ceil(pw.N / bn)
            sp_list = [forced_splits or 1]
            if can_split and base <= 640:
                sp_list += [sp for sp in (2, 3, 4, 6, 8, 12, 16)
                            if sp <= ktiles // 2 and base * sp <= 2560 and sp * M * pw.N * 4 <= (1 << 28)]
            for sp in sp_list:
                for rg in ((3,) if t == 12 else (3, 4) if t in (13, 14) else (2, 3) if t in (6, 9) else (2, 3, 4)):
                    cands.append((t, rg, sp))
        if forced_splits in (None, 1):
            cands += [(t, rg, 1) for t in halo for rg in (2, 3, 4)]
            if can_split and " gi" not in key:
                nch = ktiles // 9
                for t in halo:
                    base = math.ceil(M / TILE_DIMS[t][0]) * math.ceil(pw.N / TILE_DIMS[t][1])
                    cands += [(t, rg, sp) for sp in (2, 3, 4, 5, 6, 8, 10) for rg in (3, 4)
                              if sp <= nch and base * sp <= 2560 and sp * M * pw.N * 4 <= (1 << 28)]
        max_sp = max(c[2] for c in cands)
        ws = _workspace(max_sp * M * pw.N * 4, device) if max_sp > 1 else None
        results = []
        for t, rg, sp in cands:
            a.tile, a.ring, a.splits = t, rg, sp
            a.workspace = ws.data_ptr() if sp > 1 else None
            a.defer_reduce = 1 if (sp > 1 and key.endswith(" gn")) else 0
            if lib.aldm_igemm(C.byref(a), _stream()) != 0:
                continue
            e0, e1 = torch.cuda.Event(enable_timing=True), torch.cuda.Event(enable_timing=True)
            sleep_us(60)
            e0.record()
            for _ in range(self.reps):
                lib.aldm_igemm(C.byref(a), _stream())
            e1.record()
            results.append(((t, rg, sp), e0, e1))
        torch.cuda.synchronize()
        ranked = sorted(results, key=lambda r: r[1].elapsed_time(r[2]))
        short = [default] + [r[0] for r in ranked if r[0] != default][: self.shortlist]
        self.cands[key] = short
        if self.verbose:
            print(f"[autotune] {key}: isolated best {ranked[0][0]} {ranked[0][1].elapsed_time(ranked[0][2]) / self.reps * 1e3:.1f} us, "
                  f"default {default}, {len(results)} valid", flush=True)
        return default

    def choose(self, key, *args):
        if key not in self.cands:
            return self.isolated(args[0], key, *args[1:])
        c = self.cands[key]
        return c[self.slot % len(c)] if self.slot is not None else c[0]

    def record(self, key, cfg, e0, e1):
        self.times.setdefault(key, {}).setdefault(cfg, []).append((e0, e1))

    def finish(self):
        torch.cuda.synchronize()
        out = {}
        for key, per in self.times.items():
            avg = {cfg: sum(a.elapsed_time(b) for a, b in evs) / len(evs) for cfg, evs in per.items()}
            best = min(avg, key=avg.get)
            default = self.cands[key][0]
            if default in avg and avg[best] > 0.97 * avg[default]:
                best = default
            out[key] = (best, avg[best], avg.get(default))
        return out


def save_tuned(path=TUNED_PATH):
    with open(path, "w") as f:
        json.dump({"device": "MI355X gfx950", "format": "key -> [tile, ring, splits]",
                   "igemm": {k: list(v) for k, v in sorted(TUNED.items())}}, f, indent=0)


TILE_NAMES = {1: "128x128", 2: "64x64", 3: "128x64", 4: "64x128", 6: "128x128w8", 7: "halo128x128", 8: "halo64x128", 9: "256x128w8", 10: "64x128w8", 11: "128x64w8", 12: "256x128ws", 13: "64x128ws", 14: "128x64ws", 15: "halo128x128ws", 16: "halo64x128ws"}

PROFILE = None
SITE = None

LORA_GATE = None


class lora_gate_scope:

    def __init__(self, table):
        self.table = table

    def __enter__(self):
        global LORA_GATE
        self.prev, LORA_GATE = LORA_GATE, self.table
        return self.table

    def __exit__(self, *exc):
        global LORA_GATE
        LORA_GATE = self.prev
        return False


def _gate_for(pw, M, lora_gate, lora_t_out=None):
    g = lora_gate if lora_gate is not None else LORA_GATE
    if g is None or not pw.Rp:
        if lora_gate is not None:
            raise _lib.AldmError("lora_gate given for a weight pack without an adapter")
        return None, 0
    if lora_t_out is not None:
        raise _lib.AldmError("lora_t_out (the trainer's copy of T) is not combined with a gate table")
    if not (g.is_cuda and g.dtype == torch.float32 and g.is_contiguous() and g.dim() == 2 and g.shape[1] == pw.Rp):
        raise _lib.AldmError(f"gate table must be a contiguous fp32 device tensor [samples][{pw.Rp}] (got {tuple(g.shape)} {g.dtype})")
    if M % g.shape[0]:
        raise _lib.AldmError(f"gate table has {g.shape[0]} rows, which does not divide the launch's {M} rows")
    return g, M // g.shape[0]
KEYLOG = None


def _launch(label, flops, nbytes, fn):
    if PROFILE is None:
        return fn()
    s, e = torch.cuda.Event(enable_timing=True), torch.cuda.Event(enable_timing=True)
    s.record()
    rc = fn()
    e.record()
    PROFILE.append((label, flops, nbytes, s, e, SITE))
    return rc


_ws_cache = {}


def _workspace(nbytes, device):
    key = (device, torch.cuda.current_stream().cuda_stream)
    t = _ws_cache.get(key)
    if t is None or t.numel() * 4 < nbytes:
        t = torch.empty(max(nbytes // 4, 1 << 22), dtype=torch.float32, device=device)
        _ws_cache[key] = t
    return t


GN_FINALIZE_MIN_TILES = 96


@dataclass
class QStats:
    table: torch.Tensor
    bm: int
    tpi: int


QSTATS_MIN_HW = 2048


XCD_MAP = int(os.environ.get("ALDM_XCD_MAP", "0"))


class Deferred:
    __slots__ = ("out", "ws", "eff", "bias", "rowbias", "rowbias_ld", "res", "keep")

    def __init__(self, out, ws, eff, bias, rowbias, rowbias_ld, res, keep):
        global DEFERRED_COUNT
        DEFERRED_COUNT += 1
        self.out, self.ws, self.eff, self.bias, self.rowbias, self.rowbias_ld, self.res = out, ws, eff, bias, rowbias, rowbias_ld, res
        self.keep = keep

    @property
    def shape(self):
        return self.out.shape


DEFERRED_COUNT = 0


class _PendingMap(dict):

    def key(self, t):
        return (t.device.index, torch.cuda.current_stream(t.device).cuda_stream)


_PENDING_BY_STREAM = _PendingMap()


def _pending_get(t):
    return _PENDING_BY_STREAM.get(_PENDING_BY_STREAM.key(t))


def _pending_set(t, d):
    k = _PENDING_BY_STREAM.key(t)
    if d is None:
        _PENDING_BY_STREAM.pop(k, None)
    else:
        _PENDING_BY_STREAM[k] = d


def drop_pending(t=None):
    if t is None:
        _PENDING_BY_STREAM.clear()
    else:
        _pending_set(t, None)


def tensor_of(x):
    return x.out if isinstance(x, Deferred) else x


def conv(x: torch.Tensor, pw: PackedW, *, x2: Optional[torch.Tensor] = None, stride=(1, 1), pad=(0, 0), dil=(1, 1),
         up_size=None, in_dilate=0, out_hw=None, in_act=ACT_NONE, in_slope=0.0, rowbias=None, rowbias_ld=0, out_act=ACT_NONE,
         out_slope=0.0, res=None, res2=None, alpha=1.0, post_act=ACT_NONE, post_slope=0.0, out2=None, out=None, out_f32=False, out_ld=None, out_batch_stride=None,
         out_pix_stride=1, out_pix_offset=0, vt=None, vt_col0=0, vt_ld=0, vt_batch_stride=0, lora_t_out=None,
         splits=None, tile=0, ring=0, gn=None, gn_keep=False, defer=False, rowstats=False, ln_parts=None, x3=None, x4=None,
         vt_dual=False, qstats=False, gn_in=None, lora_gate=None):
    _require_gpu(x)
    if _pending_get(x) is not None:
        raise _lib.AldmError("conv: a deferred split-K reduce is pending on this stream -- its consumer groupnorm() must be the next launch")
    assert x.dtype == torch.bfloat16 and x.is_contiguous() and x.dim() == 4
    B, IH, IW, C1 = x.shape
    C2 = 0
    if x2 is not None:
        assert x2.dtype == torch.bfloat16 and x2.is_contiguous() and x2.shape[:3] == x.shape[:3]
        C2 = x2.shape[3]
    assert C1 + C2 == pw.Cin, f"conv: input channels {C1}+{C2} != packed {pw.Cin}"
    C3 = x3.shape[3] if x3 is not None else 0
    C4 = x4.shape[3] if x4 is not None else 0
    assert C3 + C4 == pw.Cext, f"conv: fused 1x1 segment channels {C3}+{C4} != packed {pw.Cext}"
    KH, KW = pw.KH, pw.KW
    VH, VW = (up_size if up_size is not None else (IH, IW))
    if out_hw is None:
        OH = (VH + 2 * pad[0] - dil[0] * (KH - 1) - 1) // stride[0] + 1
        OW = (VW + 2 * pad[1] - dil[1] * (KW - 1) - 1) // stride[1] + 1
    else:
        OH, OW = out_hw
    ncols = pw.N // 2 if pw.geglu else pw.N
    if vt is not None and not vt_dual:
        ncols = vt_col0
    if out_ld is None:
        out_ld = ncols
    if out is None:
        out = torch.empty(B, OH, OW, out_ld, dtype=torch.float32 if out_f32 else torch.bfloat16, device=x.device)
    if out_batch_stride is None:
        assert out_pix_stride == 1 and out_pix_offset == 0, "strided output rows need an explicit batch stride"
        out_batch_stride = OH * OW * out_ld
    if (PGEMM and tile == 0 and ring == 0 and KH == 1 and KW == 1 and stride == (1, 1) and pad == (0, 0) and up_size is None
            and not in_dilate and in_act == ACT_NONE and x2 is None and x3 is None and pw.Kpad == C1 and C1 in PGEMM_K
            and pw.N % 64 == 0 and out.dtype == torch.bfloat16 and out_pix_stride == 1 and out_pix_offset == 0
            and out_batch_stride == OH * OW * out_ld and out_ld % 8 == 0 and rowbias is None and out_act == ACT_NONE
            and post_act == ACT_NONE and res2 is None and out2 is None and alpha == 1.0 and (lora_t_out is None or pw.Rp)
            and splits in (None, 1) and gn is None and (not vt_dual or vt is not None)
            and not (qstats and OH * OW >= QSTATS_MIN_HW)
            and (not pw.Rp or getattr(pw, "ranks_used", 99) <= 32)
            and (pw.ln_s is None or (ln_parts is not None and ln_parts.shape[1] <= 16))
            and not (pw.geglu and (res is not None or vt is not None or pw.Rp or rowstats))
            and not (vt is not None and (res is not None or rowstats or vt_col0 % 32 or (vt_col0 <= 0 and not vt_dual) or vt_col0 < 0))
            and (res is None or (res.is_contiguous() and res.numel() == B * OH * OW * out_ld))
            and PGEMM_CFG.get(_pgemm_key(B * OH * OW, pw, C1, res, vt, rowstats, lora_t_out is not None, vt_dual)) != PGEMM_USE_IGEMM):
        return _pgemm(x, pw, out, out_ld, B * OH * OW, C1, OH * OW, res, vt, vt_col0, vt_ld, vt_batch_stride, rowstats, ln_parts, lora_t_out, vt_dual,
                      lora_gate=lora_gate)
    a = IgemmArgs()
    if x3 is not None:
        for t in (x3, x4):
            assert t is None or (t.dtype == torch.bfloat16 and t.is_contiguous() and tuple(t.shape[:3]) == (B, OH, OW))
        a.x3, a.Cin3 = x3.data_ptr(), C3
        if x4 is not None:
            a.x4, a.Cin4 = x4.data_ptr(), C4
    a.x, a.x2 = x.data_ptr(), (x2.data_ptr() if x2 is not None else None)
    a.B, a.IH, a.IW, a.Cin, a.Cin2 = B, IH, IW, C1, C2
    a.UH, a.UW = (up_size if up_size is not None else (0, 0))
    a.in_dilate = in_dilate
    a.w, a.Kpad = pw.w.data_ptr(), pw.Kpad
    a.KH, a.KW = KH, KW
    a.stride_h, a.stride_w = stride
    a.pad_h, a.pad_w = pad
    a.dil_h, a.dil_w = dil
    a.OH, a.OW, a.Cout = OH, OW, pw.N
    a.in_act, a.in_slope = in_act, in_slope
    if pw.Rp:
        a.lora_a, a.lora_b, a.Rp = pw.lora_a.data_ptr(), pw.lora_b.data_ptr(), pw.Rp
        a.lora_t_out = lora_t_out.data_ptr() if lora_t_out is not None else None
    gate, gate_rows = _gate_for(pw, B * OH * OW, lora_gate, lora_t_out)
    if gate is not None:
        a.lora_gate, a.gate_rows = gate.data_ptr(), gate_rows
    a.bias = pw.bias.data_ptr() if pw.bias is not None else None
    if pw.ln_s is not None:
        a.ln_s, a.ln_eps = pw.ln_s.data_ptr(), pw.ln_eps
        if pw.Rp:
            a.ln_sa, a.ln_ca = pw.ln_sa.data_ptr(), pw.ln_ca.data_ptr()
        if ln_parts is not None:
            assert ln_parts.dtype == torch.float32 and ln_parts.is_contiguous() and ln_parts.dim() == 3 and ln_parts.shape[2] == 2
            assert ln_parts.shape[0] == B * IH * IW and KH == 1 and KW == 1, "ln_parts: one row of partials per GEMM row"
            a.ln_parts, a.ln_nparts = ln_parts.data_ptr(), ln_parts.shape[1]
    elif ln_parts is not None:
        raise _lib.AldmError("conv: ln_parts without a LayerNorm-folded weight pack (pack_linear_ln)")
    if rowstats:
        if vt is not None or pw.geglu or out_f32 or out2 is not None or pw.N % 64 or gn is not None or defer:
            raise _lib.AldmError("conv: rowstats needs the standard bf16 epilogue and N % 64 == 0")
# ... 25 lines not shown
        gn_defer = pw.N % gn[2] == 0 and (pw.N // gn[2]) % 4 == 0 and OH * OW * (pw.N // gn[2] // 4) <= 4096
    elif gn_defer:
        ct, ng = defer if isinstance(defer, tuple) else (pw.N, 32)
        cg = ct // ng
        gn_defer = ct % ng == 0 and cg % 4 == 0 and pw.N % cg == 0 and OH * OW * (cg // 4) <= 4096
    fast_path = not (pw.Cin % 64 or (x2 is not None and x2.shape[3] % 64) or in_act)
    tuning = False
    key = None
    if tile == 0 and ring == 0:
        sfx = (("" if splits is None else f" sp{splits}") + (" gn" if gn_defer else "") + (" rs" if rowstats else "")
               + (" lp" if ln_parts is not None else "") + (f" e{C3}+{C4}" if x3 is not None else "") + (" vd" if vt_dual else "")
               + (" gi" if gn_in is not None else ""))
        key = tune_key(M, pw.N, C1, C2, KH, KW, stride, up_size is not None, in_dilate, pw.Rp, vt is not None, pw.geglu,
                       pw.ln_s is not None, fast_path, OW, pad, dil) + sfx
        halo = halo_tiles(OW, KH == 3 and KW == 3 and stride == (1, 1) and pad == (1, 1) and dil == (1, 1) and fast_path
                          and not in_dilate and not pw.Rp and vt is None and not pw.geglu and pw.ln_s is None)
        if (KH == 1 and IH == 1 and KW % 2 == 1 and KW > 1 and stride == (1, 1) and pad == (0, (KW - 1) * dil[1] // 2) and dil[0] == 1 and fast_path
                and not in_dilate and not pw.Rp and vt is None and not pw.geglu and pw.ln_s is None and up_size is None and x3 is None and gn_in is None):
            halo = [t for t in (15, 16) if TILE_DIMS[t][0] + (KW - 1) * dil[1] <= HALO_ROWS[t]]
        if x3 is not None:
            halo = [t for t in halo if t in (15, 16) and up_size is None and C3 % 64 == 0 and C4 % 64 == 0
                    and (TILE_DIMS[t][0] // OW + 2) * (OW + 2) <= (192 if t == 15 else 128)]
        cfg = TUNED.get(key)
        if cfg is None and TUNED_LEGACY_KEYS:
            cfg = TUNED.get(tune_key(M, pw.N, C1, C2, KH, KW, stride, up_size is not None, in_dilate, pw.Rp, vt is not None,
                                     pw.geglu, pw.ln_s is not None, fast_path) + sfx)
        if cfg is not None and cfg[0] in HALO_ROWS and cfg[0] not in halo:
            if os.environ.get("ALDM_VERBOSE_TUNED") == "1":
                print(f"[ops] table entry {cfg} of '{key}' names a halo tile this geometry cannot take: heuristics instead", file=sys.stderr)
            cfg = None
        tuning = TUNER is not None and not torch.cuda.is_current_stream_capturing()
        if tuning:
            cfg = TUNER.choose(key, a, M, pw, ktiles, can_split and splits is None, splits, fast_path, vt is not None, x.device, halo)
        if cfg is not None:
            tile, ring, splits = cfg
            if x3 is not None and tile in HALO_ROWS:
                ring = 3
    if gn_in is not None:
        q1, q2 = getattr(x, "qstats", None), (getattr(x2, "qstats", None) if x2 is not None else None)
        if not gn_in_ok(x, x2, pw, stride, pad, dil, up_size, x3):
            raise _lib.AldmError("conv: gn_in needs a 3x3 / stride 1 / pad 1 launch that fits a halo tile and inputs with .qstats (gn_in_ok)")
        if tile not in HALO_ROWS:
            tile, ring = (15 if (128 % OW == 0 and (128 // OW + 2) * (OW + 2) <= HALO_ROWS[15]) else 16), GNIN_RING
        splits = 1
        gm_, bt_, a.gnin_groups, a.gnin_eps, a.gnin_act = gn_in
        a.gnin_gamma, a.gnin_beta = gm_.data_ptr(), bt_.data_ptr()
        a.gnin_q1, a.gnin_bm1, a.gnin_tpi1 = q1.table.data_ptr(), q1.bm, q1.tpi
        if q2 is not None:
            a.gnin_q2, a.gnin_bm2, a.gnin_tpi2 = q2.table.data_ptr(), q2.bm, q2.tpi
    if splits is None:
        splits = auto_splits(M, pw.N, ktiles) if (can_split and tile not in HALO_ROWS) else 1
    if tile == 0:
        tile = heuristic_cfg(M, pw, ktiles, can_split, fast_path, vt is not None, splits)[0]
    if not ring:
        bm, bn = TILE_DIMS[tile]
        ring = pick_ring(tile, bm, bn, pw.Rp, math.ceil(M / bm) * math.ceil(pw.N / bn) * max(1, splits), ktiles)
    qs = None
    if (qstats and splits == 1 and vt is None and not pw.geglu and not out_f32 and out2 is None and out_pix_stride == 1
            and not pw.Rp and pw.ln_s is None and not rowstats
            and pw.N % 8 == 0 and pw.N % TILE_DIMS[tile][1] == 0 and out_ld == pw.N and OH * OW >= QSTATS_MIN_HW):
        bm = TILE_DIMS[tile][0]
        if tile in HALO_ROWS:
            tpi = math.ceil(OH / (bm // OW))
            qs = QStats(torch.empty(B * tpi, 2, pw.N // 4, 2, dtype=torch.float32, device=x.device), 0, tpi)
        elif OH * OW >= bm:
            qs = QStats(torch.empty(math.ceil(M / bm), 2, pw.N // 4, 2, dtype=torch.float32, device=x.device), bm, 0)
        if qs is not None:
            a.qstat_out = qs.table.data_ptr()
    stats = None
    if rowstats:
        if tile in HALO_ROWS or pw.N % TILE_DIMS[tile][1] or splits != 1:
            tile, splits = _lib.TILE_64x64, 1
            ring = pick_ring(tile, 64, 64, pw.Rp, math.ceil(M / 64) * (pw.N // 64), ktiles)
        stats = torch.empty(M, pw.N // TILE_DIMS[tile][1], 2, dtype=torch.float32, device=x.device)
        a.rowstat_out = stats.data_ptr()
    a.splits = splits
    if splits > 1:
        a.workspace = _workspace(splits * M * pw.N * 4, x.device).data_ptr()
    a.tile = tile
    a.ring = ring
    a.xcd_map = XCD_MAP
    lib = _lib.load()
    eff = lib.aldm_igemm_effective_splits(C.byref(a)) if (gn_defer and splits > 1) else 1
    a.defer_reduce = 1 if eff > 1 else 0
    ktot = KH * KW * pw.Cin + pw.Cext
    flops = 2.0 * M * pw.N * ktot + (2.0 * M * pw.Rp * (ktot + pw.N) if pw.Rp else 0.0)
    nbytes = 2.0 * (B * IH * IW * pw.Cin + M * pw.Cext + pw.N * ktot + M * ncols)
    label = (f"igemm_{TILE_NAMES[tile]}_r{pw.Rp}{'_vt' if vt is not None else ''}{'_sk' if splits > 1 else ''}"
             f"|M{M} N{pw.N} K{ktot}{' geglu' if pw.geglu else ''}")

    if qs is not None:
        out.qstats = qs
    elif hasattr(out, "qstats"):
        del out.qstats

    def finish():
        if gn is None:
            if eff > 1:
                d = Deferred(out, a.workspace, eff, a.bias, a.rowbias, a.rowbias_ld, a.res, (pw, rowbias, res, x3, x4))
                _pending_set(out, d)
                return d
            return (out, stats) if rowstats else out
        gamma, beta, groups, eps, act = gn
        if eff <= 1:
            y = groupnorm(out, gamma, beta, groups, eps, act)
            return (out, y) if gn_keep else y
        y = torch.empty(B, OH, OW, pw.N, dtype=torch.bfloat16, device=x.device)
        n = M * pw.N
        check(_launch(f"groupnorm_partials|HW{OH * OW} C{pw.N} S{eff}", 10.0 * n, (4.0 * eff + 2.0) * n, lambda: lib.aldm_groupnorm_partials(
            a.workspace, eff, B, OH * OW, pw.N, a.bias, a.rowbias, a.rowbias_ld, a.res, (a.out if gn_keep else None), None, 0,
            groups, eps, _p(gamma), _p(beta), act, _p(y), _stream())), "aldm_groupnorm_partials")
        return (out, y) if gn_keep else y

    if tuning and TUNER.slot is not None:
        e0, e1 = torch.cuda.Event(enable_timing=True), torch.cuda.Event(enable_timing=True)
        e0.record()
        rc = lib.aldm_igemm(C.byref(a), _stream())
        check(rc, "aldm_igemm")
        y = finish() if gn_defer else None
        e1.record()
        TUNER.record(key, (tile, ring, splits), e0, e1)
        return y if gn_defer else finish()
    if KEYLOG is not None and PROFILE is not None:
        KEYLOG.append((len(PROFILE), (key, (tile, ring, splits))))
    check(_launch(label, flops, nbytes, lambda: lib.aldm_igemm(C.byref(a), _stream())), "aldm_igemm")
    return finish()


PGEMM = os.environ.get("ALDM_NO_PGEMM") != "1"
PGEMM_K = (256, 384, 640)
PGEMM_CFG = {}
PGEMM_TUNED_PATH = os.path.join(os.path.dirname(os.path.abspath(__file__)), "pgemm_gfx950.json")
if os.path.exists(PGEMM_TUNED_PATH) and os.environ.get("ALDM_NO_TUNED") != "1":
    with open(PGEMM_TUNED_PATH) as _f:
        for _k, _v in json.load(_f)["pgemm"].items():
            _m, _n, _kk, _kind = _k.split("|")
            PGEMM_CFG[(int(_m), int(_n), int(_kk), _kind)] = tuple(_v)


if os.environ.get("ALDM_PGEMM_PATCH"):
    with open(os.environ["ALDM_PGEMM_PATCH"]) as _f:
        for _k, _v in json.load(_f).items():
            _m, _n, _kk, _kind = _k.split("|")
            if _v is None:
                PGEMM_CFG.pop((int(_m), int(_n), int(_kk), _kind), None)
            else:
                PGEMM_CFG[(int(_m), int(_n), int(_kk), _kind)] = tuple(_v)
PGEMM_USE_IGEMM = (0, 0, 0, 0)


def _pgemm_key(M, pw, K, res, vt, rowstats=False, lora_t=False, dual=False):
    kind = (("g" if pw.geglu else "") + ("v" if vt is not None else "") + ("r" if res is not None else "") + (f"l{pw.Rp}" if pw.Rp else "")
            + ("s" if rowstats else "") + ("t" if lora_t else "") + ("d" if dual else ""))
    return (M, pw.N, K, kind)


def _pgemm(x, pw, out, out_ld, M, K, OHW, res, vt, vt_col0, vt_ld, vt_bs, rowstats, ln_parts, lora_t_out=None, vt_dual=False, lora_gate=None):
    lib = _lib.load()
    a = _lib.PgemmArgs()
    a.x, a.w, a.M, a.N, a.K = x.data_ptr(), pw.w.data_ptr(), M, pw.N, K
    a.bias = pw.bias.data_ptr() if pw.bias is not None else None
    if pw.ln_s is not None:
        assert ln_parts.dtype == torch.float32 and ln_parts.is_contiguous() and ln_parts.dim() == 3 and ln_parts.shape[2] == 2
        assert ln_parts.shape[0] == M, "ln_parts: one row of partials per GEMM row"
        a.ln_s, a.ln_eps, a.ln_parts, a.ln_nparts = pw.ln_s.data_ptr(), pw.ln_eps, ln_parts.data_ptr(), ln_parts.shape[1]
        if pw.Rp:
            a.ln_sa, a.ln_ca = pw.ln_sa.data_ptr(), pw.ln_ca.data_ptr()
    elif ln_parts is not None:
        raise _lib.AldmError("conv: ln_parts without a LayerNorm-folded weight pack (pack_linear_ln)")
    if pw.Rp:
        a.lora_a, a.lora_b, a.Rp, a.ranks_used = pw.lora_a.data_ptr(), pw.lora_b.data_ptr(), pw.Rp, pw.ranks_used
        if lora_t_out is not None:
            assert lora_t_out.dtype == torch.bfloat16 and lora_t_out.is_contiguous() and tuple(lora_t_out.shape) == (M, pw.Rp)
            a.lora_t_out = lora_t_out.data_ptr()
    gate, gate_rows = _gate_for(pw, M, lora_gate, lora_t_out)
    if gate is not None:
        a.lora_gate, a.gate_rows = gate.data_ptr(), gate_rows
    a.geglu = 1 if pw.geglu else 0
    a.res = res.data_ptr() if res is not None else None
    a.out, a.out_ld = out.data_ptr(), out_ld
    if vt is not None:
        a.vt, a.vt_col0, a.vt_ld, a.vt_batch_stride, a.OHW = vt.data_ptr(), vt_col0, vt_ld, vt_bs, OHW
        a.vt_dual = 1 if vt_dual else 0
    cfg = PGEMM_CFG.get(_pgemm_key(M, pw, K, res, vt, rowstats, lora_t_out is not None, vt_dual))
    if cfg is not None and rowstats and pw.N // (cfg[1] * cfg[2]) > 16:
        cfg = None
    if cfg is not None:
        a.mi, a.nt, a.tiles_per_range = cfg[:3]
        a.waves = cfg[3] if len(cfg) > 3 else 4
    if rowstats:
        a.max_ranges = 16
    check(lib.aldm_pgemm_plan(C.byref(a)), "aldm_pgemm_plan")
    stats = None
    if rowstats:
        stats = torch.empty(M, pw.N // (a.nt * a.tiles_per_range), 2, dtype=torch.float32, device=x.device)
        a.rowstat_out = stats.data_ptr()
    ncols = pw.N // 2 if pw.geglu else (vt_col0 if (vt is not None and not vt_dual) else pw.N)
    flops = 2.0 * M * pw.N * K + (2.0 * M * pw.Rp * (K + pw.N) if pw.Rp else 0.0)
    nbytes = 2.0 * (M * K + pw.N * K + M * ncols)
    label = (f"pgemm_{16 * a.mi * a.waves}x{a.nt}x{a.tiles_per_range}w{a.waves}_r{pw.Rp}{'_vt' if vt is not None else ''}{'d' if vt_dual else ''}"
             f"|M{M} N{pw.N} K{K}{' geglu' if pw.geglu else ''}")
    if hasattr(out, "qstats"):
        del out.qstats
    if KEYLOG is not None and PROFILE is not None:
        KEYLOG.append((len(PROFILE), ("pg:" + "|".join(str(v) for v in _pgemm_key(M, pw, K, res, vt, rowstats, lora_t_out is not None, vt_dual)),
                                      (a.mi, a.nt, a.tiles_per_range, a.waves))))
    check(_launch(label, flops, nbytes, lambda: lib.aldm_pgemm(C.byref(a), _stream())), "aldm_pgemm")
    return (out, stats) if rowstats else out


def linear(x2d: torch.Tensor, pw: PackedW, **kw):
    M, K = x2d.shape
    out = kw.pop("out", None)
    y = conv(x2d.view(1, 1, M, K), pw, out=(None if out is None else out), **kw)
    if kw.get("rowstats"):
        return (y[0] if out is not None else y[0].view(M, -1)), y[1]
    return y if out is not None else y.view(M, -1)


def groupnorm(x, gamma, beta, groups, eps, act=ACT_NONE, x2=None):
    if isinstance(x, Deferred):
        if x is not _pending_get(x.out):
            raise _lib.AldmError("groupnorm: this deferred convolution's partial tiles are gone (not the one pending on this stream)")
        B, H, W, C1 = x.out.shape
        C2 = x2.shape[3] if x2 is not None else 0
        Cg = (C1 + C2) // groups
        if (C1 + C2) % groups or Cg % 4 or C1 % Cg or H * W * (Cg // 4) > 4096:
            raise _lib.AldmError(f"groupnorm: deferred input [{B} x {H * W} x {C1}+{C2} / {groups} groups] does not fit aldm_groupnorm_partials")
        y = torch.empty(B, H, W, C1 + C2, dtype=torch.bfloat16, device=x.out.device)
        lib = _lib.load()
        n = B * H * W * (C1 + C2)
        check(_launch(f"groupnorm_partials|HW{H * W} C{C1}+{C2} S{x.eff}", 10.0 * n, (4.0 * x.eff + 2.0) * n, lambda: lib.aldm_groupnorm_partials(
            x.ws, x.eff, B, H * W, C1, x.bias, x.rowbias, x.rowbias_ld, x.res, _p(x.out), _p(x2), C2, groups, eps,
            _p(gamma), _p(beta), act, _p(y), _stream())), "aldm_groupnorm_partials")
        _pending_set(x.out, None)
        return y
    _require_gpu(x)
    B, H, W, C1 = x.shape
    C2 = x2.shape[3] if x2 is not None else 0
    y = torch.empty(B, H, W, C1 + C2, dtype=torch.bfloat16, device=x.device)
    lib = _lib.load()
    n = B * H * W * (C1 + C2)
    q1, q2 = getattr(x, "qstats", None), (getattr(x2, "qstats", None) if x2 is not None else None)
    Cg = (C1 + C2) // groups
    if (q1 is not None and (x2 is None or q2 is not None) and (C1 + C2) % groups == 0 and Cg % 4 == 0
            and C1 % 8 == 0 and C2 % 8 == 0 and groups <= 64 and (C1 + C2) // 8 <= 256
            and x.is_contiguous() and (x2 is None or x2.is_contiguous())):
        tiles = max(q.tpi if q.tpi > 0 else H * W // q.bm + 1 for q in (q1, q2) if q is not None)
        ws = torch.empty(B, 64, 2, dtype=torch.float32, device=x.device) if tiles >= GN_FINALIZE_MIN_TILES else None
        check(_launch(f"groupnorm_apply|HW{H * W} C{C1 + C2}", 10.0 * n, 4.0 * n, lambda: lib.aldm_groupnorm_apply(
            _p(x), _p(q1.table), q1.bm, q1.tpi, _p(x2), _p(q2.table) if q2 is not None else None, q2.bm if q2 is not None else 0,
            q2.tpi if q2 is not None else 0, B, H * W, C1, C2, groups, eps, _p(gamma), _p(beta), act, _p(y), _p(ws), _stream())),
            "aldm_groupnorm_apply")
        return y
    check(_launch(f"groupnorm|HW{H * W} C{C1 + C2}", 10.0 * n, 4.0 * n, lambda: lib.aldm_groupnorm(
        _p(x), _p(x2), B, H * W, C1, C2, groups, eps, _p(gamma), _p(beta), act, _p(y), _stream())), "aldm_groupnorm")
    return y


GNIN_RING = int(os.environ.get("ALDM_GNIN_RING", "0"))


def gn_in_ok(x, x2, pw, stride=(1, 1), pad=(1, 1), dil=(1, 1), up_size=None, x3=None):
    if not isinstance(x, torch.Tensor) or getattr(x, "qstats", None) is None or x.dim() != 4:
        return False
    if x2 is not None and (not isinstance(x2, torch.Tensor) or getattr(x2, "qstats", None) is None):
        return False
    B, IH, IW, C1 = x.shape
    C2 = x2.shape[3] if x2 is not None else 0
    hw = IH * IW
    for q in (x.qstats, x2.qstats if x2 is not None else None):
        if q is not None and not (q.tpi > 0 or q.bm <= hw):
            return False
    fits = any(bm % IW == 0 and (bm // IW + 2) * (IW + 2) <= HALO_ROWS[t] for t, bm in ((7, 128), (8, 64)))
    return (pw.KH == 3 and pw.KW == 3 and tuple(stride) == (1, 1) and tuple(pad) == (1, 1) and tuple(dil) == (1, 1) and up_size is None
            and x3 is None and not pw.Rp and not pw.geglu and pw.ln_s is None and C1 % 64 == 0 and C2 % 64 == 0 and C1 + C2 <= 512
            and pw.Cin == C1 + C2 and fits)


def gn_silu_conv_out_ok(x, pw, groups):
    q = getattr(x, "qstats", None) if isinstance(x, torch.Tensor) else None
    return (q is not None and x.dim() == 4 and x.shape[2] == 16 and x.shape[3] == 128 and x.is_contiguous() and x.dtype == torch.bfloat16
            and pw.KH == 3 and pw.KW == 3 and pw.N <= 16 and pw.Cin == 128 and not pw.Rp and 128 % groups == 0 and (128 // groups) % 4 == 0
            and groups <= 64 and (q.tpi > 0 or q.bm <= x.shape[1] * x.shape[2]))


def gn_silu_conv_out(x, gamma, beta, groups, eps, pw):
    _require_gpu(x)
    B, H, W, Cc = x.shape
    q = x.qstats
    out = torch.empty(B, H, W, pw.N, dtype=torch.float32, device=x.device)
    lib = _lib.load()
    n = B * H * W
    check(_launch(f"gn_silu_conv3x3|HW{H * W} C{Cc} N{pw.N}", 2.0 * n * pw.N * 9 * Cc + 10.0 * n * Cc, 2.0 * n * Cc + 4.0 * n * pw.N,
                  lambda: lib.aldm_gn_silu_conv3x3_small(_p(x), _p(q.table), q.bm, q.tpi, B, H, W, Cc, groups, eps, _p(gamma), _p(beta), _p(pw.w),
                                                         pw.Kpad, _p(pw.bias), pw.N, _p(out), _stream())), "aldm_gn_silu_conv3x3_small")
    return out


def layernorm(x2d, gamma, beta, eps=1e-5):
    _require_gpu(x2d)
    M, Cc = x2d.shape
    y = torch.empty_like(x2d)
    lib = _lib.load()
    check(_launch(f"layernorm|M{M} C{Cc}", 10.0 * M * Cc, 4.0 * M * Cc, lambda: lib.aldm_layernorm(
        _p(x2d), M, Cc, _p(gamma), _p(beta), eps, _p(y), _stream())), "aldm_layernorm")
    return y


LOG2E = 1.4426950408889634


def attention(qk, vt, B, N, H, d, out=None, kv_len=None, fp8=False, prescaled=False):
    _require_gpu(qk)
    Cc = H * d
    if out is None:
        out = torch.empty(B * N, Cc, dtype=torch.bfloat16, device=qk.device)
# ... 361 lines not shown

def gaussian_sample(params_nchw, noise):
    _require_gpu(params_nchw)
    B, C2 = params_nchw.shape[:2]
    pf, nf = params_nchw.float().contiguous(), noise.float().contiguous()
    out = torch.empty_like(nf)
    check(_lib.load().aldm_gaussian_sample(_p(pf), _p(nf), B, nf.numel() // B, _p(out), _stream()), "aldm_gaussian_sample")
    return out


def sleep_us(us):
    check(_lib.load().aldm_sleep_us(int(us), _stream()), "aldm_sleep_us")


def gather_row(table, idx, out):
    row = table[0].numel()
    assert table.dtype == torch.float32 and out.dtype == torch.float32 and out.numel() == row and idx.dtype == torch.int32
    check(_launch("gather_row", 0.0, 8.0 * row, lambda: _lib.load().aldm_gather_row(_p(table), _p(idx), row, _p(out), _stream())),
          "aldm_gather_row")


def advance_step(step_idx, timesteps_f32, t_out):
    check(_launch("advance_step", 0.0, 16.0, lambda: _lib.load().aldm_advance_step(_p(step_idx), _p(timesteps_f32), timesteps_f32.numel(),
                                                                                    _p(t_out), _stream())), "aldm_advance_step")


def adamw_flat(p, g, m, v, lr, beta1, beta2, eps, wd, step, grad_scale=1.0):
    check(_lib.load().aldm_adamw_flat(_p(p), _p(g), _p(m), _p(v), p.numel(), lr, beta1, beta2, eps, wd, step,
                                      grad_scale, _stream()), "aldm_adamw_flat")


def transpose_tokens(x2d, B, N, Cc, npad=None):
    _require_gpu(x2d)
    npad = npad or (N + 7) // 8 * 8
    out = torch.empty(B, Cc, npad, dtype=torch.bfloat16, device=x2d.device)
    check(_lib.load().aldm_transpose_tokens(_p(x2d), x2d.stride(0), B, N, Cc, npad, _p(out), _stream()), "aldm_transpose_tokens")
    return out


def attention_train(qkv, qkvT, B, N, H, d):
    Cc = H * d
    out = torch.empty(B * N, Cc, dtype=torch.bfloat16, device=qkv.device)
    lse = torch.empty(B, H, N, dtype=torch.float32, device=qkv.device)
    base, tb = qkv.data_ptr(), qkvT.data_ptr()
    npad = qkvT.shape[2]
    check(_lib.load().aldm_attention_lse(C.c_void_p(base), 3 * Cc, C.c_void_p(base + 2 * Cc), 3 * Cc,
                                         C.c_void_p(tb + 2 * (2 * Cc) * npad), npad, 3 * Cc * npad, B, N, H, d,
                                         1.0 / math.sqrt(d), _p(out), Cc, _p(lse), _stream()), "aldm_attention_lse")
    return out, lse


def attention_bwd(qkv, qkvT, dO, O, lse, B, N, H, d, dOT=None):
    Cc = H * d
    npad = qkvT.shape[2]
    if dOT is None:
        dOT = transpose_tokens(dO, B, N, Cc, npad)
    assert tuple(dOT.shape) == (B, Cc, npad)
    dqkv = torch.empty(B * N, 3 * Cc, dtype=torch.bfloat16, device=qkv.device)
    delta = torch.empty(B, H, N, dtype=torch.float32, device=qkv.device)
    base, tb, gb = qkv.data_ptr(), qkvT.data_ptr(), dqkv.data_ptr()
    check(_lib.load().aldm_attention_bwd(
        C.c_void_p(base), C.c_void_p(base + 2 * Cc), C.c_void_p(base + 4 * Cc), 3 * Cc,
        C.c_void_p(tb), C.c_void_p(tb + 2 * Cc * npad), _p(dOT), npad, 3 * Cc * npad, 3 * Cc * npad, Cc * npad,
        _p(dO), _p(O), Cc, _p(lse), _p(delta), B, N, H, d, 1.0 / math.sqrt(d),
        C.c_void_p(gb), C.c_void_p(gb + 2 * Cc), C.c_void_p(gb + 4 * Cc), 3 * Cc, _stream()), "aldm_attention_bwd")
    return dqkv


def _like(buf, like):
    assert buf.is_contiguous() and buf.numel() == like.numel() and buf.dtype == like.dtype
    return buf


def groupnorm_bwd(x, dy, gamma, beta, groups, eps, act, x2=None, need_dx2=True, dx_add=None, dx2_add=None):
    B, H, W, C1 = x.shape
    C2 = x2.shape[3] if x2 is not None else 0
    dx = torch.empty_like(x)
    dx2 = torch.empty_like(x2) if (x2 is not None and need_dx2) else None
    a1 = _like(dx_add, x) if dx_add is not None else None
    a2 = _like(dx2_add, x2) if (dx2 is not None and dx2_add is not None) else None
    if isinstance(dy, Deferred):
        if dy is not _pending_get(dy.out) or dy.bias is not None or dy.rowbias is not None or dy.res is not None:
            raise _lib.AldmError("groupnorm_bwd: deferred dY must be the pending split-K launch, without bias / residual")
        assert tuple(dy.out.shape) == (B, H, W, C1 + C2)
        check(_lib.load().aldm_groupnorm_bwd_partials(_p(x), _p(x2), dy.ws, dy.eff, B, H * W, C1, C2, groups, eps, _p(gamma), _p(beta),
                                                      act, _p(dx), _p(dx2), _p(a1), _p(a2), _stream()), "aldm_groupnorm_bwd_partials")
        _pending_set(dy.out, None)
        return dx, dx2
    check(_lib.load().aldm_groupnorm_bwd(_p(x), _p(x2), _p(dy), B, H * W, C1, C2, groups, eps, _p(gamma), _p(beta), act,
                                         _p(dx), _p(dx2), _p(a1), _p(a2), _stream()), "aldm_groupnorm_bwd")
    return dx, dx2


def layernorm_bwd(x2d, dy, gamma, eps=1e-5, dx_add=None):
    M, Cc = x2d.shape
    dx = torch.empty_like(x2d)
    a = _like(dx_add, x2d) if dx_add is not None else None
    check(_lib.load().aldm_layernorm_bwd(_p(x2d), _p(dy), M, Cc, _p(gamma), eps, _p(dx), _p(a), _stream()), "aldm_layernorm_bwd")
    return dx


def geglu_fwd(h):
    M, two_i = h.shape
    out = torch.empty(M, two_i // 2, dtype=torch.bfloat16, device=h.device)
    check(_lib.load().aldm_geglu_fwd(_p(h), M, two_i // 2, _p(out), _stream()), "aldm_geglu_fwd")
    return out


def geglu_bwd(h, dout):
    dh = torch.empty_like(h)
    check(_lib.load().aldm_geglu_bwd(_p(h), _p(dout), h.shape[0], h.shape[1] // 2, _p(dh), _stream()), "aldm_geglu_bwd")
    return dh


def add_bf16(a, b):
    c = torch.empty_like(a)
    check(_lib.load().aldm_add_bf16(_p(a), _p(b), a.numel(), _p(c), _stream()), "aldm_add_bf16")
    return c


def upsample_nearest_bwd(dy, ih, iw):
    B, OH, OW, Cc = dy.shape
    dx = torch.empty(B, ih, iw, Cc, dtype=torch.bfloat16, device=dy.device)
    check(_lib.load().aldm_upsample_nearest_bwd(_p(dy), B, ih, iw, OH, OW, Cc, _p(dx), _stream()), "aldm_upsample_nearest_bwd")
    return dx


def tn_small(P, Q, rows_dev, Qc=None):
    M, Rp = P.shape
    check(_lib.load().aldm_tn_small(_p(P), Rp, _p(Q), Q.stride(0), Qc or Q.shape[1], M, _p(rows_dev), _stream()), "aldm_tn_small")



class TnBatch:
    REC = 48

    def __init__(self, capacity, device):
        self.capacity = capacity
        self.tab = {rp: torch.zeros(capacity * self.REC, dtype=torch.uint8, device=device) for rp in (32, 64)}
        self.jobs = {32: [], 64: []}
        self.keep = []
        self._packed = {}
        self.owner = None

    def add(self, P, Q, rows_dev, Qc):
        M, Rp = P.shape
        ldq = Q.stride(0)
        if ldq % 8 or Qc % 8 or P.data_ptr() % 16 or Q.data_ptr() % 16 or len(self.jobs[Rp]) >= self.capacity:
            tn_small(P, Q, rows_dev, Qc=Qc)
            return
        qt = -(-Qc // 128)
        msplit = max(1, 24 // qt)
        mpb = max(64, -(-(-(-M // msplit)) // 32) * 32)
        self.jobs[Rp].append((P.data_ptr(), Q.data_ptr(), rows_dev.data_ptr(), M, ldq, Qc, qt, mpb, qt * (-(-M // mpb))))
        self.keep += [P, Q, rows_dev]

    def _pack(self):
        import struct
        self._packed = {}
        for rp, jobs in self.jobs.items():
            if not jobs:
                continue
            wg0, recs = 0, []
            for (pp, qq, rr, M, ldq, Qc, qt, mpb, nwg) in jobs:
                recs.append(struct.pack("<qqqiiiiii", pp, qq, rr, M, ldq, Qc, qt, mpb, wg0))
                wg0 += nwg
# ... 45 lines not shown
```

### audioldm_with_lora_amd/unet.py

```python
import json
import math
import os
from types import SimpleNamespace

import torch
from torch import nn

from . import ops
from ._lib import ACT_NONE, ACT_SILU
from .configs import UNET
from .lora import GATE_COLS, AdapterRouting, LoraLinear, lora_layout


class ResnetBlock2D(nn.Module):
    def __init__(self, cin, cout, temb, groups, eps):
        super().__init__()
        self.norm1 = nn.GroupNorm(groups, cin, eps=eps)
        self.conv1 = nn.Conv2d(cin, cout, 3, padding=1)
        if temb:
            self.time_emb_proj = nn.Linear(temb, cout)
        self.norm2 = nn.GroupNorm(groups, cout, eps=eps)
        self.conv2 = nn.Conv2d(cout, cout, 3, padding=1)
        if cin != cout:
            self.conv_shortcut = nn.Conv2d(cin, cout, 1)
# ... 116 lines not shown
        g1=_f32(r.norm1.weight), b1=_f32(r.norm1.bias), g2=_f32(r.norm2.weight), b2=_f32(r.norm2.bias),
        conv1=ops.pack_conv(r.conv1.weight, r.conv1.bias), conv2=ops.pack_conv(r.conv2.weight, r.conv2.bias),
        shortcut=ops.pack_conv(sc.weight, sc.bias) if sc is not None else None,
        conv2s=ops.pack_conv_shortcut(r.conv2.weight, r.conv2.bias, sc.weight, sc.bias) if fuse else None,
        groups=r.groups, eps=r.eps, cout=r.cout, temb_off=0)


LN_FOLD_MIN_C = 64


def pack_attention(a: Attention, ln=None, layout=None):
    wq, bq, lq = _lin(a.to_q)
    wk, bk, lk = _lin(a.to_k)
    wv, bv, lv = _lin(a.to_v)
    wo, bo, lo = _lin(a.to_out[0])
    c = wq.shape[0]
    qs = ops.LOG2E / math.sqrt(a.dim_head)
    wq = wq.detach().float() * qs
    bq = None if bq is None else bq.detach().float() * qs
    lq = [(n, A, Bm, sc * qs) for n, A, Bm, sc in lq]
    bias = None
    if bq is not None:
        bias = torch.cat([bq, bk.detach().float(), bv.detach().float()])
    fold = ln is not None and c % 64 == 0 and c >= LN_FOLD_MIN_C
    wqkv = torch.cat([wq, wk.detach().float(), wv.detach().float()])
    qkv = ops.pack_linear_ln(wqkv, bias, ln[0], ln[1]) if fold else ops.pack_linear(wqkv, bias)
    ops.attach_lora(qkv, [(i * c, c, A, Bm, sc, n) for i, l in enumerate((lq, lk, lv)) for n, A, Bm, sc in l], layout)
    out = ops.pack_linear(wo, bo)
    ops.attach_lora(out, [(0, wo.shape[0], A, Bm, sc, n) for n, A, Bm, sc in lo], layout)
    return SimpleNamespace(qkv=qkv, out=out, heads=a.heads, d=a.dim_head, c=c, ln_folded=fold)


def _merge_ff2_proj_out(t: Transformer2DModel):
    blk = t.transformer_blocks[0]
    w2, b2 = blk.ff.net[2].weight.detach().float(), blk.ff.net[2].bias.detach().float()
    wp = t.proj_out.weight.detach().float().flatten(1)
    bp = t.proj_out.bias.detach().float()
    wm = torch.cat([wp @ w2, wp], dim=1)
    return ops.pack_conv(wm[:, :, None, None].contiguous(), (wp @ b2 + bp).contiguous())


def pack_transformer(t: Transformer2DModel, layout=None):
    blk = t.transformer_blocks[0]
    merged = (t.channels % 64 == 0 and not isinstance(blk.ff.net[2], LoraLinear) and not isinstance(t.proj_out, LoraLinear))
    return SimpleNamespace(
        ff2_proj=_merge_ff2_proj_out(t) if merged else None,
        gn_g=_f32(t.norm.weight), gn_b=_f32(t.norm.bias), groups=t.groups,
        proj_in=ops.pack_conv(t.proj_in.weight, t.proj_in.bias), proj_out=ops.pack_conv(t.proj_out.weight, t.proj_out.bias),
        ln=[(_f32(n.weight), _f32(n.bias)) for n in (blk.norm1, blk.norm2, blk.norm3)],
        attn1=pack_attention(blk.attn1, (blk.norm1.weight, blk.norm1.bias), layout),
        attn2=pack_attention(blk.attn2, (blk.norm2.weight, blk.norm2.bias), layout),
        ff1=(ops.pack_linear_ln(blk.ff.net[0].proj.weight, blk.ff.net[0].proj.bias, blk.norm3.weight, blk.norm3.bias, geglu=True)
             if (t.channels % 64 == 0 and t.channels >= LN_FOLD_MIN_C) else ops.pack_geglu(blk.ff.net[0].proj.weight, blk.ff.net[0].proj.bias)),
        ff2=ops.pack_linear(blk.ff.net[2].weight, blk.ff.net[2].bias))


GN_IN = os.environ.get("ALDM_NO_GN_IN") is None


def _gn_in_pays(x, x2, pw):
    if not (GN_IN and pw.N <= 128 and pw.Cin <= 384 and ops.gn_in_ok(x, x2, pw)):
        return False
    hw = x.shape[1] * x.shape[2]
    return all((q.tpi if q.tpi > 0 else hw // q.bm + 1) < ops.GN_FINALIZE_MIN_TILES for q in (x.qstats, x2.qstats if x2 is not None else None) if q is not None)


def run_resnet(P, x, x2=None, rowbias=None, rowbias_ld=0, next_gn=None, defer=None):
    rb = rowbias[:, P.temb_off:] if rowbias is not None else None
    gn2 = (P.g2, P.b2, P.groups, P.eps, ACT_SILU)
    h1 = None
    if _gn_in_pays(x, x2, P.conv1):
        h1 = ops.conv(x, P.conv1, x2=x2, pad=(1, 1), rowbias=rb, rowbias_ld=rowbias_ld, qstats=True,
                      gn_in=(P.g1, P.b1, P.groups, P.eps, ACT_SILU))
        if not (P.conv2s is None and getattr(h1, "qstats", None) is not None and _gn_in_pays(h1, None, P.conv2)):
            h, h1 = ops.groupnorm(h1, *gn2), None
    else:
        h = ops.groupnorm(x, P.g1, P.b1, P.groups, P.eps, ACT_SILU, x2=x2)
        x = ops.tensor_of(x)
        h = ops.conv(h, P.conv1, pad=(1, 1), rowbias=rb, rowbias_ld=rowbias_ld, gn=gn2, qstats=True)
    x = ops.tensor_of(x)
    if P.conv2s is not None and (x2 is None or x2.shape[3] % 64 == 0) and x.shape[3] % 64 == 0:
        if next_gn is not None:
            return ops.conv(h, P.conv2s, pad=(1, 1), x3=x, x4=x2, gn=next_gn, gn_keep=True, qstats=True)
        return ops.conv(h, P.conv2s, pad=(1, 1), x3=x, x4=x2, defer=(defer or False), qstats=True)
    if P.shortcut is not None:
        xs = ops.conv(x, P.shortcut, x2=x2)
    else:
        assert x2 is None
        xs = x
    src, fold = (h1, dict(gn_in=gn2)) if h1 is not None else (h, {})
    if next_gn is not None:
        return ops.conv(src, P.conv2, pad=(1, 1), res=xs, gn=next_gn, gn_keep=True, qstats=True, **fold)
    return ops.conv(src, P.conv2, pad=(1, 1), res=xs, defer=(defer or False), qstats=True, **fold)


def run_attention(P, hn, h_res, B, N, fp8=False, ln_parts=None, rowstats=False):
    C = P.c
    ops.SITE = f"attn C{C} N{N}"
    kind = ops.attn_block_ok(P.qkv, N, P.heads, P.d, ln_parts)
    if kind == 64 or (kind and not fp8):
        a = ops.attn_block(hn, P.qkv, ln_parts, B, N, P.heads, P.d, fp8=fp8)
        y = ops.linear(a, P.out, res=h_res, rowstats=rowstats)
        ops.SITE = None
        return y
    npad = (N + 7) // 8 * 8
    vt = torch.empty(B, C, npad, dtype=torch.bfloat16, device=hn.device)
    qk = ops.conv(hn.view(B, 1, N, C), P.qkv, vt=vt, vt_col0=2 * C, vt_ld=npad, vt_batch_stride=C * npad, ln_parts=ln_parts)
    a = ops.attention(qk.view(B * N, 2 * C), vt, B, N, P.heads, P.d, fp8=fp8, prescaled=True)
    y = ops.linear(a, P.out, res=h_res, rowstats=rowstats)
    ops.SITE = None
    return y


def transformer_gn(P):
    return (P.gn_g, P.gn_b, P.groups, 1e-6, ACT_NONE)


def run_transformer(P, x, fp8=False, xn=None, defer=None):
    B, H, W, C = x.shape
    N = H * W
    h = xn if xn is not None else ops.groupnorm(x, *transformer_gn(P))
    f1, f2, f3 = P.attn1.ln_folded, P.attn2.ln_folded, P.ff1.ln_s is not None
    st = None
    h = ops.conv(h, P.proj_in, rowstats=f1)
    if f1:
        h, st = h
    h = h.view(B * N, C)
    h = run_attention(P.attn1, h if f1 else ops.layernorm(h, *P.ln[0]), h, B, N, fp8, ln_parts=st, rowstats=f2)
    st = None
    if f2:
        h, st = h
    h = run_attention(P.attn2, h if f2 else ops.layernorm(h, *P.ln[1]), h, B, N, fp8, ln_parts=st, rowstats=f3)
    st = None
    if f3:
        h, st = h
    g = ops.linear(h if f3 else ops.layernorm(h, *P.ln[2]), P.ff1, ln_parts=st)
    if P.ff2_proj is not None:
        return ops.conv(g.view(B, H, W, 4 * C), P.ff2_proj, x2=h.view(B, H, W, C), res=x, defer=(defer or False), qstats=True)
    h = ops.linear(g, P.ff2, res=h)
    return ops.conv(h.view(B, H, W, C), P.proj_out, res=x, defer=(defer or False), qstats=True)


class UNet2DConditionModel(AdapterRouting, nn.Module):
    config_name = "config.json"

    def __init__(self, **cfg_over):
        super().__init__()
        cfg = dict(UNET)
        cfg.update({k: v for k, v in cfg_over.items() if k in UNET})
        self.cfg = cfg
        self.config = SimpleNamespace(**cfg)
        boc = cfg["block_out_channels"]
        groups, eps, heads = cfg["norm_num_groups"], cfg["norm_eps"], cfg["num_heads"]
        assert cfg["class_embeddings_concat"], "AudioLDM concatenates the class embedding"
        ted = boc[0] * 4
        self.time_embedding = TimestepEmbedding(boc[0], ted)
        self.class_embedding = nn.Linear(cfg["class_embed_input_dim"], ted)
        temb = ted * 2
        self.conv_in = nn.Conv2d(cfg["in_channels"], boc[0], 3, padding=1)
        downs, out_c = [], boc[0]
        for i, typ in enumerate(cfg["down_block_types"]):
            in_c, out_c = out_c, boc[i]
            downs.append(DownBlock(in_c, out_c, temb, cfg["layers_per_block"], groups, eps, heads,
                                   cfg["cross_attention_dim"][i], typ.startswith("CrossAttn"), i != len(boc) - 1))
        self.down_blocks = nn.ModuleList(downs)
        self.mid_block = MidBlock(boc[-1], temb, groups, eps, heads, cfg["cross_attention_dim"][-1])
        ups, rev, rev_cross = [], list(reversed(boc)), list(reversed(cfg["cross_attention_dim"]))
        out_c = rev[0]
        for i, typ in enumerate(cfg["up_block_types"]):
            prev, out_c = out_c, rev[i]
            in_c = rev[min(i + 1, len(boc) - 1)]
            ups.append(UpBlock(in_c, out_c, prev, temb, cfg["layers_per_block"] + 1, groups, eps, heads, rev_cross[i],
                               typ.startswith("CrossAttn"), i != len(boc) - 1))
        self.up_blocks = nn.ModuleList(ups)
        self.conv_norm_out = nn.GroupNorm(groups, boc[0], eps=eps)
        self.conv_out = nn.Conv2d(boc[0], cfg["out_channels"], 3, padding=1)
        self.num_upsamplers = len(boc) - 1
        self._plan = None
        self._plan_version = 0
        self._weights_version = 0

    @classmethod
    def from_pretrained(cls, path, subfolder=None, torch_dtype=None, **kw):
        d = os.path.join(path, subfolder) if subfolder else path
        cfg_path = os.path.join(d, cls.config_name)
        if not os.path.isfile(cfg_path):
            raise FileNotFoundError(f"{cfg_path} not found: hub downloads are unavailable, pass a local directory")
        raw = json.load(open(cfg_path))
        over = dict(in_channels=raw["in_channels"], out_channels=raw["out_channels"],
                    block_out_channels=tuple(raw["block_out_channels"]), layers_per_block=raw["layers_per_block"],
                    num_heads=raw.get("num_attention_heads") or raw["attention_head_dim"],
                    cross_attention_dim=tuple(raw["cross_attention_dim"]),
                    class_embed_input_dim=raw["projection_class_embeddings_input_dim"],
                    norm_num_groups=raw["norm_num_groups"], norm_eps=raw["norm_eps"],
                    down_block_types=tuple(raw["down_block_types"]), up_block_types=tuple(raw["up_block_types"]),
                    sample_size=raw.get("sample_size", 128))
        m = cls(**over)
        from safetensors.torch import load_file
        m.load_state_dict(load_file(os.path.join(d, "diffusion_pytorch_model.safetensors")), strict=True)
        return m

    def _has_trainable_lora(self):
        return any(isinstance(m, LoraLinear) and any(a.weight.requires_grad for a in m.lora_A.values()) for m in self.modules())

    def invalidate_packed(self):
        self._plan = None
        self._plan_version += 1

    @property
    def plan_version(self):
        return self._plan_version

    def _apply(self, fn, *a, **k):
        self.invalidate_packed()
        self._weights_version += 1
        return super()._apply(fn, *a, **k)

    def load_state_dict(self, *a, **k):
        self.invalidate_packed()
        self._weights_version += 1
        return super().load_state_dict(*a, **k)

    def plan(self):
# ... 38 lines not shown
            bs.append(r.time_emb_proj.bias)
        P.temb_all = ops.pack_linear(torch.cat(ws), torch.cat(bs))
        P.temb_total = off
        P.gn_out = (_f32(self.conv_norm_out.weight), _f32(self.conv_norm_out.bias))
        P.conv_out = ops.pack_conv(self.conv_out.weight, self.conv_out.bias)
        P.version = self._plan_version
        self._plan = P
        return P

    def temb_table(self, timesteps_f32, class_labels_bf16):
        cfg, P = self.cfg, self.plan()
        boc = cfg["block_out_channels"]
        ted = boc[0] * 4
        n, b = timesteps_f32.numel(), class_labels_bf16.shape[0]
        temb = ops.timestep_embedding(timesteps_f32.contiguous(), n, boc[0])
        e2 = ops.linear(ops.linear(temb, P.te1, out_act=ACT_SILU), P.te2, out_act=ACT_SILU)
        c = ops.linear(class_labels_bf16, P.cls, out_act=ACT_SILU)
        semb = torch.cat([e2[:, None, :].expand(n, b, ted), c[None].expand(n, b, ted)], dim=2).reshape(n * b, 2 * ted).contiguous()
        return ops.linear(semb, P.temb_all, out_f32=True).view(n, b, P.temb_total)

    def forward_nhwc(self, x, t_dev, class_labels_bf16, rowbias=None, gate=None):
        if gate is not None and tuple(gate.shape) != (x.shape[0], GATE_COLS):
            raise ValueError(f"gate table must be [{x.shape[0]}][{GATE_COLS}], got {tuple(gate.shape)}")
        with ops.lora_gate_scope(gate):
            return self._forward_nhwc(x, t_dev, class_labels_bf16, rowbias)

    def device_gate(self, adapter_names=None, batch=1, adapter_weights=None, **kw):
        if adapter_weights is None and self.routing_is_plain(adapter_names):
            return None
        g = self.gate_table(adapter_names, batch, **kw)
        if adapter_weights is not None:
            w = torch.as_tensor(adapter_weights, dtype=torch.float32).reshape(-1)
            if not bool(torch.isfinite(w).all()):
                raise ValueError("adapter_weights must be finite")
            reps = g.shape[0] // max(1, w.numel())
            if w.numel() * reps != g.shape[0]:
                raise ValueError(f"adapter_weights needs one entry per prompt, got {w.numel()} for a batch of {g.shape[0]}")
            nw = kw.get("num_waveforms_per_prompt", 1)
            w = w.repeat_interleave(nw)
            g = g * (torch.cat([w, w]) if kw.get("do_classifier_free_guidance") else w)[:, None]
        return g.to(self.conv_in.weight.device).contiguous()

    def _forward_nhwc(self, x, t_dev, class_labels_bf16, rowbias=None):
        ops.drop_pending(x)
        cfg, P = self.cfg, self.plan()
        fp8 = bool(getattr(self, "attention_fp8", False))
        b, H, W, _ = x.shape
        boc = cfg["block_out_channels"]
        ted = boc[0] * 4
        groups, eps = cfg["norm_num_groups"], cfg["norm_eps"]
        factor = 2 ** self.num_upsamplers
        forward_upsample_size = (H % factor != 0) or (W % factor != 0)

        ld = P.temb_total
        if rowbias is None:
            temb = ops.timestep_embedding(t_dev, b, boc[0])
            e1 = ops.linear(temb, P.te1, out_act=ACT_SILU)
            semb = torch.empty(b, 2 * ted, dtype=torch.bfloat16, device=x.device)
            ops.linear(e1, P.te2, out_act=ACT_SILU, out=semb, out_ld=2 * ted)
            ops.linear(class_labels_bf16, P.cls, out_act=ACT_SILU, out=semb[:, ted:], out_ld=2 * ted)
            rowbias = ops.linear(semb, P.temb_all, out_f32=True)

        h = ops.conv(x, P.conv_in, pad=(1, 1), qstats=True)
        skips = [h]
        def norm1_of(r):
            return (r.g1.numel(), r.groups)

        for bi, blk in enumerate(P.down):
            nr = len(blk.resnets)
            for i, r in enumerate(blk.resnets):
                if i + 1 < nr:
                    nxt = norm1_of(blk.resnets[i + 1])
                elif blk.down is not None:
                    nxt = None
                else:
                    nxt = norm1_of(P.mid.resnets[0])
                if blk.attns is not None:
                    h, hn = run_resnet(r, h, None, rowbias, ld, next_gn=transformer_gn(blk.attns[i]))
                    h = run_transformer(blk.attns[i], h, fp8, xn=hn, defer=nxt)
                else:
                    h = run_resnet(r, h, None, rowbias, ld, defer=nxt)
                skips.append(ops.tensor_of(h))
            if blk.down is not None:
                h = ops.conv(h, blk.down, stride=(2, 2), pad=(1, 1), defer=norm1_of(P.down[bi + 1].resnets[0]), qstats=True)
                skips.append(ops.tensor_of(h))
        h, hn = run_resnet(P.mid.resnets[0], h, None, rowbias, ld, next_gn=transformer_gn(P.mid.attns[0]))
        h = run_transformer(P.mid.attns[0], h, fp8, xn=hn, defer=norm1_of(P.mid.resnets[1]))
        h = run_resnet(P.mid.resnets[1], h, None, rowbias, ld, defer=norm1_of(P.up[0].resnets[0]))
        for bi, blk in enumerate(P.up):
            nr = len(blk.resnets)
            for i, r in enumerate(blk.resnets):
                if i + 1 < nr:
                    nxt = norm1_of(blk.resnets[i + 1])
                elif blk.up is not None:
                    nxt = None
                else:
                    nxt = (P.gn_out[0].numel(), groups)
                if blk.attns is not None:
                    h, hn = run_resnet(r, h, skips.pop(), rowbias, ld, next_gn=transformer_gn(blk.attns[i]))
                    h = run_transformer(blk.attns[i], h, fp8, xn=hn, defer=nxt)
                else:
                    h = run_resnet(r, h, skips.pop(), rowbias, ld, defer=nxt)
            if blk.up is not None:
                if forward_upsample_size:
                    size = (skips[-1].shape[1], skips[-1].shape[2])
                else:
                    size = (h.shape[1] * 2, h.shape[2] * 2)
                h = ops.conv(h, blk.up, pad=(1, 1), up_size=size, defer=norm1_of(P.up[bi + 1].resnets[0]), qstats=True)
        if ops.gn_silu_conv_out_ok(h, P.conv_out, groups):
            return ops.gn_silu_conv_out(h, P.gn_out[0], P.gn_out[1], groups, eps, P.conv_out)
        h = ops.groupnorm(h, P.gn_out[0], P.gn_out[1], groups, eps, ACT_SILU)
        return ops.conv(h, P.conv_out, pad=(1, 1), out_f32=True)

    def forward(self, sample, timestep, encoder_hidden_states=None, class_labels=None, cross_attention_kwargs=None,
                return_dict=False, adapter_names=None, adapter_weights=None, **kw):
        assert encoder_hidden_states is None, "AudioLDM conditions through class_labels only"
        if not sample.is_cuda:
            raise ops._lib.AldmError("UNet2DConditionModel.forward needs CUDA/HIP tensors (no CPU fallback)")
        b = sample.shape[0]
        if not torch.is_tensor(timestep):
            timestep = torch.tensor([timestep], device=sample.device)
        t = timestep.to(device=sample.device, dtype=torch.float32).reshape(-1)
        if t.numel() not in (1, b):
            raise ValueError("timestep must be a scalar or have one entry per sample")
        gate = self.device_gate(adapter_names, b, adapter_weights)
        if self.training and torch.is_grad_enabled() and self._has_trainable_lora():
            if gate is not None:
                raise ops._lib.AldmError("training runs the single active adapter: no adapter_names / weights / several adapters")
            from .training import trainer_of
            out = trainer_of(self).autograd_forward(sample, t, class_labels)
            return SimpleNamespace(sample=out) if return_dict else (out,)
        x = ops.nchw_to_nhwc(sample.float())
        cls_bf16 = ops.f32_to_bf16(class_labels.to(device=sample.device, dtype=torch.float32).contiguous())
        eps = self.forward_nhwc(x, t.contiguous(), cls_bf16, gate=gate)
        out = ops.nhwc_to_nchw_f32(eps).to(sample.dtype)
        if return_dict:
            return SimpleNamespace(sample=out)
        return (out,)
```

### include/aldm_hip.h

```cpp
#ifndef ALDM_HIP_H
#define ALDM_HIP_H

#include <stddef.h>
#include <stdint.h>

#ifdef __cplusplus
extern "C" {
#endif

#define ALDM_OK 0
#define ALDM_E_ARG (-1)
#define ALDM_E_ALIGN (-2)
#define ALDM_E_UNSUPPORTED (-3)

enum { ALDM_ACT_NONE = 0, ALDM_ACT_SILU = 1, ALDM_ACT_LRELU = 2, ALDM_ACT_TANH = 3, ALDM_ACT_GELU = 4  };
enum { ALDM_OUT_BF16 = 0, ALDM_OUT_F32 = 1 };

const char* aldm_version(void);
const char* aldm_last_error(void);

typedef struct {
  const void* x;  const void* x2;
  int B, IH, IW, Cin, Cin2;
  int UH, UW;
  int in_dilate;
  const void* w;
  int Kpad;
  int KH, KW, stride_h, stride_w, pad_h, pad_w, dil_h, dil_w;
  int OH, OW, Cout;
  int in_act;  float in_slope;
  const float* ln_s; const float* ln_sa; const float* ln_ca; float ln_eps;
  const void* lora_a;
  const void* lora_b;
  int Rp;
  void* lora_t_out;
  const float* bias;
  const float* rowbias;
  int rowbias_ld;
  int geglu;
  int out_act;  float out_slope;
  const void* res;  const void* res2;
  float alpha;
  int post_act;  float post_slope;  void* out2;
  void* out;  int out_dtype;  int out_ld;
  long long out_batch_stride;
  int out_pix_stride, out_pix_offset;
  void* vt;  int vt_col0;  int vt_ld;  long long vt_batch_stride;
  int splits;  float* workspace;
  int tile;
  int ring;
  int defer_reduce;
  float* rowstat_out;
  const float* ln_parts;  int ln_nparts;
  float* qstat_out;
  const void* x3;  const void* x4;  int Cin3, Cin4;
  int vt_dual;
  const float* gnin_gamma; const float* gnin_beta; const float* gnin_q1; const float* gnin_q2;
  int gnin_bm1, gnin_tpi1, gnin_bm2, gnin_tpi2, gnin_groups, gnin_act; float gnin_eps;
  int xcd_map;
  const float* lora_gate; int gate_rows;
} aldm_igemm_t;

enum { ALDM_TILE_AUTO = 0, ALDM_TILE_128x128 = 1, ALDM_TILE_64x64 = 2, ALDM_TILE_128x64 = 3, ALDM_TILE_64x128 = 4,
       ALDM_TILE_32x64 = 5, ALDM_TILE_128x128_W8 = 6 ,
       ALDM_TILE_HALO_128x128 = 7, ALDM_TILE_HALO_64x128 = 8,
       ALDM_TILE_HALO_128x128_WS = 15, ALDM_TILE_HALO_64x128_WS = 16 ,
       ALDM_TILE_256x128_W8 = 9 ,
       ALDM_TILE_256x128_WS = 12 ,
       ALDM_TILE_64x128_WS = 13, ALDM_TILE_128x64_WS = 14 ,
       ALDM_TILE_64x128_W8 = 10, ALDM_TILE_128x64_W8 = 11  };

int aldm_igemm(const aldm_igemm_t* p, void* stream);
size_t aldm_igemm_workspace_bytes(const aldm_igemm_t* p);
int aldm_igemm_effective_splits(const aldm_igemm_t* p);

typedef struct {
  const void* x;
  const void* w;
  int M, N, K;
  const float* bias;
  const float* ln_s; const float* ln_sa; const float* ln_ca; float ln_eps;
  const float* ln_parts; int ln_nparts;
  const void* lora_a;
  const void* lora_b;
  int Rp, ranks_used;
  int geglu;
  const void* res;
  void* out; int out_ld;
  void* vt; int vt_col0; int vt_ld; long long vt_batch_stride; int OHW;
  float* rowstat_out;
  int mi, nt, tiles_per_range;
  int max_ranges;
  int waves;
  void* lora_t_out;
  int vt_dual;
  const float* lora_gate; int gate_rows;
} aldm_pgemm_t;

int aldm_pgemm_supported(int K);
int aldm_pgemm_plan(aldm_pgemm_t* p);
int aldm_pgemm(const aldm_pgemm_t* p, void* stream);

int aldm_groupnorm(const void* x, const void* x2, int B, int HW, int C1, int C2, int groups, float eps,
                   const float* gamma, const float* beta, int act, void* y, void* stream);

int aldm_groupnorm_apply(const void* x, const float* qstat, int bm, int tpi, const void* x2, const float* qstat2, int bm2, int tpi2,
                         int B, int HW, int C1, int C2, int groups, float eps, const float* gamma, const float* beta, int act,
                         void* y, float* stat_ws, void* stream);

int aldm_gn_silu_conv3x3_small(const void* x, const float* qstat, int bm, int tpi, int B, int H, int W, int C, int groups, float eps,
                               const float* gamma, const float* beta, const void* w, int w_ld, const float* bias, int Cout, float* out,
                               void* stream);

int aldm_layernorm(const void* x, int M, int C, const float* gamma, const float* beta, float eps, void* y,
                   void* stream);
int aldm_groupnorm_partials(const float* ws, int splits, int B, int HW, int C, const float* bias, const float* rowbias,
                            int rowbias_ld, const void* res, void* sum_out, const void* x2, int C2, int groups, float eps,
                            const float* gamma, const float* beta, int act, void* y,
                            void* stream);
int aldm_embed_layernorm(const long long* ids, int B, int L, int C, const float* word, int vocab, const float* pos,
                         int npos, const float* type0, const float* gamma, const float* beta, float eps, int pad_idx,
                         void* y, void* stream);

int aldm_attention(const void* q, int ldq, const void* k, int ldk, const void* vt, int vt_ld,
                   long long vt_batch_stride, int B, int N, int H, int d, float scale, void* out, int out_ld,
                   void* stream);

int aldm_attention_prescaled(const void* q, int ldq, const void* k, int ldk, const void* vt, int vt_ld,
                             long long vt_batch_stride, int B, int N, int H, int d, void* out, int out_ld, void* stream);

int aldm_attention_wide(const void* q, int ldq, const void* k, int ldk, const void* vt, int vt_ld, long long vt_batch_stride,
                        int B, int N, int d, void* out, int out_ld, void* stream);

int aldm_attn_block64(const void* x, const float* ln_parts, int ln_nparts, const void* w, int Kpad, const float* bias,
                      const float* ln_s, const void* lora_a, const void* lora_b, int Rp, int ranks_used, const float* ln_sa,
                      const float* ln_ca, float ln_eps, int B, int N, int H, int d, void* out, void* stream);
int aldm_attn_block64_fp8(const void* x, const float* ln_parts, int ln_nparts, const void* w, int Kpad, const float* bias,
                          const float* ln_s, const void* lora_a, const void* lora_b, int Rp, int ranks_used, const float* ln_sa,
                          const float* ln_ca, float ln_eps, int B, int N, int H, int d, void* out, void* stream);
int aldm_attn_block64_gated(const void* x, const float* ln_parts, int ln_nparts, const void* w, int Kpad, const float* bias,
                            const float* ln_s, const void* lora_a, const void* lora_b, int Rp, int ranks_used, const float* ln_sa,
                            const float* ln_ca, float ln_eps, int B, int N, int H, int d, void* out, void* stream, const float* lora_gate);
int aldm_attn_block64_fp8_gated(const void* x, const float* ln_parts, int ln_nparts, const void* w, int Kpad, const float* bias,
                                const float* ln_s, const void* lora_a, const void* lora_b, int Rp, int ranks_used, const float* ln_sa,
                                const float* ln_ca, float ln_eps, int B, int N, int H, int d, void* out, void* stream, const float* lora_gate);
int aldm_attn_block256_gated(const void* x, const float* ln_parts, int ln_nparts, const void* w, int Kpad, const float* bias,
                             const float* ln_s, const void* lora_a, const void* lora_b, int Rp, int ranks_used, const float* ln_sa,
                             const float* ln_ca, float ln_eps, int B, int N, int H, int d, void* out, void* stream, const float* lora_gate);

int aldm_attn_block256(const void* x, const float* ln_parts, int ln_nparts, const void* w, int Kpad, const float* bias,
                       const float* ln_s, const void* lora_a, const void* lora_b, int Rp, int ranks_used, const float* ln_sa,
                       const float* ln_ca, float ln_eps, int B, int N, int H, int d, void* out, void* stream);

int aldm_attention_varlen(const void* q, int ldq, const void* k, int ldk, const void* vt, int vt_ld,
                          long long vt_batch_stride, int B, int N, int H, int d, float scale, const int* kv_len,
                          void* out, int out_ld, void* stream);

int aldm_attention_fp8(const void* q, int ldq, const void* k, int ldk, const void* vt, int vt_ld,
                       long long vt_batch_stride, int B, int N, int H, int d, float scale, void* out, int out_ld,
                       void* stream);

int aldm_attention_lse(const void* q, int ldq, const void* k, int ldk, const void* vt, int vt_ld,
                       long long vt_batch_stride, int B, int N, int H, int d, float scale, void* out, int out_ld,
                       float* lse, void* stream);
int aldm_attention_bwd(const void* q, const void* k, const void* v, int ld, const void* qT, const void* kT,
                       const void* dOT, int ldt, long long qT_batch_stride, long long kT_batch_stride,
                       long long dOT_batch_stride, const void* dO, const void* O, int ldo, const float* lse,
                       float* delta, int B, int N, int H, int d, float scale, void* dq, void* dk, void* dv,
                       int ldg, void* stream);

int aldm_hifigan_respair_supported(int C, int K, int dil);
int aldm_hifigan_respair(const void* x, int B, int T, int C, const void* w1, int ld1, const float* b1, int dil, const void* w2, int ld2,
                         const float* b2, int K, float slope, float alpha, const void* res2, int post_act, float post_slope, void* out,
                         void* stream);

int aldm_conv1d_to1(const void* x, int B, int T, int C, const void* w, const float* bias, int K, int act, float* out, void* stream);

int aldm_softmax_rows(const float* s, int rows, int cols, int ld_in, float scale, void* p, int ld_out, void* stream);

int aldm_timestep_embedding(const float* t, int t_stride, int B, int dim, void* out, void* stream);
int aldm_silu(const void* x, long long n, void* y, void* stream);
int aldm_nchw_f32_to_nhwc(const float* x, int B, int C, int HW, void* y, int y_is_f32, void* stream);
int aldm_nhwc_to_nchw_f32(const void* x, int x_is_f32, int B, int C, int HW, float* y, void* stream);
int aldm_f32_to_bf16(const float* x, long long n, float mul, void* y, void* stream);
int aldm_cfg_ddim_step(const float* eps, float* x, int B, long long n_per_sample, int cfg, float guidance,
                       const float* coef, const int* step_idx, void* x_in_bf16, void* stream);
int aldm_ddim_step_fused(const float* eps, float* x, int B, long long n_per_sample, int cfg, float guidance, const float* coef,
                         int* step_idx, void* x_in_bf16, const float* table, long long row_elems, float* rowbias,
                         const float* timesteps, int n_steps, float* t_out, unsigned* ticket, void* stream);
int aldm_dpm_step_fused(const float* eps, float* x, int B, long long n_per_sample, int cfg, float guidance, const float* coef,
                        int* step_idx, void* x_in_bf16, float* hist, const float* table, long long row_elems, float* rowbias,
                        const float* timesteps, int n_steps, float* t_out, unsigned* ticket, void* stream);
int aldm_ddim_step_fused_masked(const float* eps, float* x, int B, long long n_per_sample, int cfg, float guidance, const float* coef,
                                int* step_idx, void* x_in_bf16, const float* table, long long row_elems, float* rowbias,
                                const float* timesteps, int n_steps, float* t_out, unsigned* ticket, const float* x0, const float* noise,
                                const float* mask, const float* blend, int channels, void* stream);
int aldm_dpm_step_fused_masked(const float* eps, float* x, int B, long long n_per_sample, int cfg, float guidance, const float* coef,
                               int* step_idx, void* x_in_bf16, float* hist, const float* table, long long row_elems, float* rowbias,
                               const float* timesteps, int n_steps, float* t_out, unsigned* ticket, const float* x0, const float* noise,
                               const float* mask, const float* blend, int channels, void* stream);
int aldm_philox_u32(unsigned* out, long long n, const unsigned* state, unsigned long long first_block, void* stream);
int aldm_randn(float* out, long long n, unsigned* state, int advance, void* stream);
// ... 60 lines not shown
```

Baseline: 339.4 denoise_steps/s.

## Add planar split-K slab layout and write-through stores for deferred GroupNorm reduce

```diff
diff --git a/audioldm_with_lora_amd/_lib.py b/audioldm_with_lora_amd/_lib.py
--- a/audioldm_with_lora_amd/_lib.py
+++ b/audioldm_with_lora_amd/_lib.py
@@ -7,6 +7,8 @@
 ACT_NONE, ACT_SILU, ACT_LRELU, ACT_TANH, ACT_GELU = 0, 1, 2, 3, 4
 OUT_BF16, OUT_F32 = 0, 1
 TILE_AUTO, TILE_128x128, TILE_64x64, TILE_128x64, TILE_64x128 = 0, 1, 2, 3, 4
+DEFER_ROWMAJOR, DEFER_PLANAR, DEFER_WRITE_THROUGH = 1, 2, 4
+SLAB_ROWMAJOR, SLAB_PLANAR = 0, 1
 
 
 class IgemmArgs(C.Structure):
@@ -87,6 +89,10 @@
     "aldm_groupnorm_partials": (C.c_int, [C.c_void_p, C.c_int, C.c_int, C.c_int, C.c_int, C.c_void_p, C.c_void_p, C.c_int,
                                           C.c_void_p, C.c_void_p, C.c_void_p, C.c_int, C.c_int, C.c_float, C.c_void_p,
                                           C.c_void_p, C.c_int, C.c_void_p, C.c_void_p]),
+    "aldm_groupnorm_partials_layout": (C.c_int, [C.c_void_p, C.c_int, C.c_int, C.c_int, C.c_int, C.c_void_p, C.c_void_p, C.c_int,
+                                                 C.c_void_p, C.c_void_p, C.c_void_p, C.c_int, C.c_int, C.c_float, C.c_void_p,
+                                                 C.c_void_p, C.c_int, C.c_void_p, C.c_int, C.c_void_p]),
+    "aldm_igemm_slab_offset": (C.c_longlong, [C.c_int, C.c_int, C.c_int, C.c_int, C.c_int, C.c_int, C.c_int]),
     "aldm_groupnorm": (C.c_int, [C.c_void_p, C.c_void_p, C.c_int, C.c_int, C.c_int, C.c_int, C.c_int, C.c_float,
                                  C.c_void_p, C.c_void_p, C.c_int, C.c_void_p, C.c_void_p]),
     "aldm_groupnorm_apply": (C.c_int, [C.c_void_p, C.c_void_p, C.c_int, C.c_int, C.c_void_p, C.c_void_p, C.c_int, C.c_int, C.c_int,
diff --git a/audioldm_with_lora_amd/csrc/igemm.hip b/audioldm_with_lora_amd/csrc/igemm.hip
--- a/audioldm_with_lora_amd/csrc/igemm.hip
+++ b/audioldm_with_lora_amd/csrc/igemm.hip
@@ -30,17 +30,38 @@
   return (size_t)p->splits * M * p->Cout * sizeof(float);
 }
 
+static bool is_halo_tile(int tile) {
+  return tile == ALDM_TILE_HALO_128x128 || tile == ALDM_TILE_HALO_64x128 || tile == ALDM_TILE_HALO_128x128_WS || tile == ALDM_TILE_HALO_64x128_WS;
+}
+
+static void plan_splits(int want, int nkt, int nch, int taps, bool halo, int& splits, int& kt_per_split) {
+  splits = want > 1 ? want : 1;
+  if (splits > nkt) splits = nkt;
+  kt_per_split = cdiv(nkt, splits);
+  splits = cdiv(nkt, kt_per_split);
+  if (halo && splits > 1) {
+    const int cps = cdiv(nch, splits > nch ? nch : splits);
+    kt_per_split = taps * cps;
+    splits = cdiv(nch, cps);
+  }
+}
+
 extern "C" int aldm_igemm_effective_splits(const aldm_igemm_t* p) {
   if (!p || p->splits <= 1) return 1;
   const int nkt = cdiv(p->KH * p->KW * (p->Cin + p->Cin2), BK) + (p->x3 ? (p->Cin3 + (p->x4 ? p->Cin4 : 0)) / BK : 0);
-  if (p->tile == ALDM_TILE_HALO_128x128 || p->tile == ALDM_TILE_HALO_64x128 || p->tile == ALDM_TILE_HALO_128x128_WS ||
-      p->tile == ALDM_TILE_HALO_64x128_WS) {
-    const int nch = (p->Cin + p->Cin2) / BK;
-    return cdiv(nch, cdiv(nch, p->splits > nch ? nch : p->splits));
-  }
-  int splits = p->splits > nkt ? nkt : p->splits;
-  const int per = cdiv(nkt, splits);
-  return cdiv(nkt, per);
+  int splits, per;
+  plan_splits(p->splits, nkt, (p->Cin + p->Cin2) / BK, p->KH * p->KW, is_halo_tile(p->tile), splits, per);
+  return splits;
+}
+
+extern "C" long long aldm_igemm_slab_offset(int layout, int B, int HW, int C, int split, int m, int n) {
+  if (layout < 0 || layout > 1 || B <= 0 || HW <= 0 || C <= 0 || (C & 3) || split < 0 || m < 0 || n < 0 || n >= C ||
+      (long long)B * HW > 0x7fffffffll || m >= B * HW)
+    return -1;
+  const FastDiv fd = make_fastdiv((unsigned)HW);
+  const int b = (int)(((((unsigned long long)(unsigned)m * fd.mul) >> 32) + (unsigned)m) >> fd.shift);
+  const int pix = m - b * HW;
+  return (long long)split * B * HW * C + (layout ? igemm_slab_index(1, b, pix, n, C, HW) : igemm_slab_index(0, 0, m, n, C, 0));
 }
 
 extern "C" int aldm_igemm(const aldm_igemm_t* p, void* stream) {
@@ -73,6 +94,7 @@
   ALDM_CHECK_ARG(!p->vt || p->vt_col0 > 0 || p->out, "igemm: out required");
   ALDM_CHECK_ARG(p->splits <= 1 || (p->workspace && p->Cout % 4 == 0), "igemm: split-K needs workspace and Cout %% 4 == 0");
   ALDM_CHECK_ARG(p->out_ld > 0, "igemm: out_ld");
+  ALDM_CHECK_ARG(p->defer_reduce >= 0 && p->defer_reduce <= 7 && (!(p->defer_reduce & 6) || (p->defer_reduce & 1)), "igemm: defer_reduce is a set of ALDM_DEFER_* flags");
   ALDM_CHECK_ARG(!p->defer_reduce || (!p->geglu && !p->res2 && !p->out2 && p->out_act == ALDM_ACT_NONE && p->post_act == ALDM_ACT_NONE && p->alpha == 1.f),
                  "igemm: defer_reduce leaves bias / row bias / res to the consumer and supports nothing else in the epilogue");
   ALDM_CHECK_ARG(!(p->geglu && p->out2) || (p->Rp == 0 && p->splits <= 1 && !p->res && !p->res2 && p->out_dtype == ALDM_OUT_BF16 &&
@@ -109,11 +131,11 @@
   d.x3 = (const bf16*)p->x3; d.x4 = (const bf16*)p->x4; d.Cin3 = p->x3 ? p->Cin3 : 0; d.Cin4 = (p->x3 && p->x4) ? p->Cin4 : 0;
   d.C3tot = d.Cin3 + d.Cin4;
   d.nkt = cdiv(Ktot, BK) + d.C3tot / BK;
-  d.splits = p->splits > 1 ? p->splits : 1;
-  if (d.splits > d.nkt) d.splits = d.nkt;
-  d.kt_per_split = cdiv(d.nkt, d.splits);
-  d.splits = cdiv(d.nkt, d.kt_per_split);
+  const int tile = p->tile ? p->tile : pick_tile(p->B * p->OH * p->OW, p->Cout);
+  plan_splits(p->splits, d.nkt, Ctot / BK, p->KH * p->KW, is_halo_tile(tile), d.splits, d.kt_per_split);
   d.ws_rows = d.M;
+  d.ws_mode = (d.splits > 1 && p->defer_reduce) ? (p->defer_reduce >> 1) & 3 : 0;
+  if ((long long)p->B * p->OH * p->OW * p->Cout * 4 >= 0x80000000ll) d.ws_mode &= ~2;
   d.lora_gate = p->lora_gate; d.fd_gate = make_fastdiv((unsigned)(p->lora_gate ? p->gate_rows : 1)); d.gate_m1 = d.M - 1;
   d.tiles_n = 0; d.tiles_m = 0; d.nwg = 0;
   ALDM_CHECK_ARG(p->xcd_map >= 0 && p->xcd_map <= 2, "igemm: xcd_map must be 0 (auto), 1 (activation-stationary) or 2 (weight-stationary)");
@@ -150,7 +172,6 @@
   }
   hipStream_t st = (hipStream_t)stream;
 
-  int tile = p->tile ? p->tile : pick_tile(d.M, d.N);
   if (p->gnin_gamma) {
     ALDM_CHECK_ARG(tile == ALDM_TILE_HALO_128x128 || tile == ALDM_TILE_HALO_64x128 || tile == ALDM_TILE_HALO_128x128_WS || tile == ALDM_TILE_HALO_64x128_WS, "igemm: gnin_* (GroupNorm of the input inside the launch) needs a halo tile");
     const int Ct = p->Cin + p->Cin2;
@@ -183,12 +204,6 @@
         aldm_set_error("igemm: the halo tiles take no LoRA / V^T / row statistics (and a second-source segment only in the wave-specialised forms)");
         return ALDM_E_UNSUPPORTED;
       }
-      if (d.splits > 1) {
-        const int nch = (d.Cin + d.Cin2) / BK;
-        const int cps = cdiv(nch, d.splits > nch ? nch : d.splits);
-        d.kt_per_split = d.KH * d.KW * cps;
-        d.splits = cdiv(nch, cps);
-      }
       rc = aldm_launch_halo(d, tile, p->ring, st);
       break;
     default: aldm_set_error("igemm: unknown tile %d", tile); return ALDM_E_UNSUPPORTED;
diff --git a/audioldm_with_lora_amd/csrc/igemm_core.h b/audioldm_with_lora_amd/csrc/igemm_core.h
--- a/audioldm_with_lora_amd/csrc/igemm_core.h
+++ b/audioldm_with_lora_amd/csrc/igemm_core.h
@@ -53,7 +53,21 @@
   const float* lora_gate;
   FastDiv fd_gate;
   int gate_m1;
+  int ws_mode;
 };
+
+__host__ __device__ __forceinline__ long long igemm_slab_index(int planar, int b, int pix, int n, int N, int HW) {
+  return planar ? ((long long)(b * (N >> 2) + (n >> 2)) * HW + pix) * 4 + (n & 3) : ((long long)b * HW + pix) * N + n;
+}
+__device__ __forceinline__ void igemm_slab_store4(float* slab, long long idx, const f32x4 v, bool wt, unsigned slab_bytes) {
+  if (wt) {
+    typedef unsigned u32x4_t __attribute__((ext_vector_type(4)));
+    const __amdgpu_buffer_rsrc_t rs = __builtin_amdgcn_make_buffer_rsrc(slab, 0, slab_bytes, 0x00020000);
+    __builtin_amdgcn_raw_buffer_store_b128(__builtin_bit_cast(u32x4_t, v), rs, (int)(idx * 4), 0, 16);
+  } else {
+    *reinterpret_cast<f32x4*>(slab + idx) = v;
+  }
+}
 
 __device__ __forceinline__ int swz(int row, int chunk) { return chunk ^ ((row >> 1) & 7); }
 
@@ -239,13 +253,20 @@
   aldm_prefetch_next_kernargs<sizeof(IgemmDev)>(tid);
 #endif
   if constexpr (SLEAN) {
+    float* slab = p.ws + (long long)split * p.ws_rows * p.N;
+    const int planar = p.ws_mode & 1;
+    const bool wt = (p.ws_mode & 2) != 0;
+    const unsigned slab_bytes = (unsigned)p.ws_rows * (unsigned)p.N * 4u;
 #pragma unroll
     for (int i = 0; i < MI; ++i) {
       const int m = m0 + wm_off + i * 16 + lrow;
+      int b = 0, pix = m;
+      if (planar) { b = fdiv(m, p.fd_ohw); pix = m - b * p.OHW; }
 #pragma unroll
       for (int j = 0; j < NI; ++j) {
         const int n = n0 + wn_off + j * 16 + lq * 4;
-        if (m < p.M && n < p.N) *reinterpret_cast<f32x4*>(p.ws + ((long long)split * p.ws_rows + m) * p.N + n) = acc[i][j];
+        if (m < p.M && n < p.N)
+          igemm_slab_store4(slab, igemm_slab_index(planar, b, pix, n, p.N, planar ? p.OHW : 0), acc[i][j], wt, slab_bytes);
       }
     }
     return;
@@ -480,8 +501,20 @@
       const int r = g / (BN / 8), c = (g - r * (BN / 8)) * 8;
       const int m = m0 + r, n = n0 + c;
       if (m >= p.M || n >= p.N) continue;
+      const float* src = Cs + r * E::LD + c;
+      if (p.ws_mode) {
+        float* slab = p.ws + (long long)split * p.ws_rows * p.N;
+        const int planar = p.ws_mode & 1;
+        const bool wt = (p.ws_mode & 2) != 0;
+        const unsigned slab_bytes = (unsigned)p.ws_rows * (unsigned)p.N * 4u;
+        int b = 0, pix = m;
+        if (planar) { b = fdiv(m, p.fd_ohw); pix = m - b * p.OHW; }
+        igemm_slab_store4(slab, igemm_slab_index(planar, b, pix, n, p.N, planar ? p.OHW : 0), *reinterpret_cast<const f32x4*>(src), wt, slab_bytes);
+        if (n + 4 < p.N)
+          igemm_slab_store4(slab, igemm_slab_index(planar, b, pix, n + 4, p.N, planar ? p.OHW : 0), *reinterpret_cast<const f32x4*>(src + 4), wt, slab_bytes);
+        continue;
+      }
       float* o = p.ws + ((long long)split * p.ws_rows + m) * p.N + n;
-      const float* src = Cs + r * E::LD + c;
       if (n + 7 < p.N) {
         *reinterpret_cast<f32x4*>(o) = *reinterpret_cast<const f32x4*>(src);
         *reinterpret_cast<f32x4*>(o + 4) = *reinterpret_cast<const f32x4*>(src + 4);
diff --git a/audioldm_with_lora_amd/csrc/norm.hip b/audioldm_with_lora_amd/csrc/norm.hip
--- a/audioldm_with_lora_amd/csrc/norm.hip
+++ b/audioldm_with_lora_amd/csrc/norm.hip
@@ -157,7 +157,7 @@
   }
 }
 
-template <int QPT>
+template <int QPT, bool PLANAR>
 __global__ __launch_bounds__(GN_THREADS) void groupnorm_partials_kernel(const float* __restrict__ ws, int splits, long long sstride,
                                                                         int HW, int C, int groups, float eps,
                                                                         const float* __restrict__ bias,
@@ -194,7 +194,7 @@
 
   f32x4 v[QPT];
   bf16x4 rv[QPT];
-  long long off[QPT], yoff[QPT];
+  long long off[QPT], woff[QPT], yoff[QPT];
   int ch[QPT];
   const bool second = c0 >= C;
 #pragma unroll
@@ -204,6 +204,7 @@
     const int pix = aldm_div(qq, dqpp), j = qq - pix * qpp;
     ch[i] = c0 + 4 * j;
     off[i] = ((long long)b * HW + pix) * C + ch[i];
+    woff[i] = PLANAR ? (((long long)b * (C >> 2) + (ch[i] >> 2)) * HW + pix) * 4 : off[i];
     yoff[i] = ((long long)b * HW + pix) * Ct + ch[i];
     v[i] = f32x4{0.f, 0.f, 0.f, 0.f};
     rv[i] = bf16x4{0, 0, 0, 0};
@@ -219,7 +220,7 @@
 #pragma unroll
     for (int i = 0; i < QPT; ++i) {
       if (tid + i * GN_THREADS < nquads) {
-        const float* w0 = ws + off[i] + sp * sstride;
+        const float* w0 = ws + woff[i] + sp * sstride;
         const f32x4 a0 = *reinterpret_cast<const f32x4*>(w0), a1 = *reinterpret_cast<const f32x4*>(w0 + sstride);
         const f32x4 a2 = *reinterpret_cast<const f32x4*>(w0 + 2 * sstride), a3 = *reinterpret_cast<const f32x4*>(w0 + 3 * sstride);
 #pragma unroll
@@ -232,7 +233,7 @@
 #pragma unroll
     for (int i = 0; i < QPT; ++i) {
       if (tid + i * GN_THREADS < nquads) {
-        const float* w0 = ws + off[i] + sp * sstride;
+        const float* w0 = ws + woff[i] + sp * sstride;
         const f32x4 a0 = *reinterpret_cast<const f32x4*>(w0);
         const f32x4 a1 = *reinterpret_cast<const f32x4*>(w0 + (rem > 1 ? 1 : 0) * sstride);
         const f32x4 a2 = *reinterpret_cast<const f32x4*>(w0 + (rem > 2 ? 2 : 0) * sstride);
@@ -627,12 +628,13 @@
   return aldm_launch_status("groupnorm");
 }
 
-extern "C" int aldm_groupnorm_partials(const float* ws, int splits, int B, int HW, int C, const float* bias,
-                                       const float* rowbias, int rowbias_ld, const void* res, void* sum_out,
-                                       const void* x2, int C2, int groups, float eps, const float* gamma, const float* beta,
-                                       int act, void* y, void* stream) {
+extern "C" int aldm_groupnorm_partials_layout(const float* ws, int splits, int B, int HW, int C, const float* bias,
+                                              const float* rowbias, int rowbias_ld, const void* res, void* sum_out,
+                                              const void* x2, int C2, int groups, float eps, const float* gamma, const float* beta,
+                                              int act, void* y, int layout, void* stream) {
   ALDM_CHECK_ARG(ws && y && gamma && beta && splits >= 1, "groupnorm_partials: null pointer / bad splits");
   ALDM_CHECK_ARG(B > 0 && HW > 0 && C > 0 && C2 >= 0 && groups > 0 && (C2 == 0 || x2), "groupnorm_partials: bad dims");
+  ALDM_CHECK_ARG(layout == ALDM_SLAB_ROWMAJOR || layout == ALDM_SLAB_PLANAR, "groupnorm_partials: unknown slab layout %d", layout);
   const int Ct = C + C2;
   ALDM_CHECK_ARG(Ct % groups == 0 && (Ct / groups) % 4 == 0 && C % (Ct / groups) == 0,
                  "groupnorm_partials: group width %d must be a multiple of 4 and divide the first source's %d channels", Ct / groups, C);
@@ -642,16 +644,26 @@
   ALDM_CHECK_ARG(nquads <= 8 * GN_THREADS, "groupnorm_partials: strip of %lld quads exceeds the register-resident limit %d", nquads, 8 * GN_THREADS);
   const AldmDiv dq = aldm_make_div((unsigned)(Ct / groups / 4));
   const long long sstride = (long long)B * HW * C;
-#define ALDM_GNP(QPT)                                                                                                  \
-  hipLaunchKernelGGL(groupnorm_partials_kernel<QPT>, dim3(B * groups), dim3(GN_THREADS), 0, (hipStream_t)stream, ws,   \
+#define ALDM_GNP2(QPT, PL)                                                                                             \
+  hipLaunchKernelGGL((groupnorm_partials_kernel<QPT, PL>), dim3(B * groups), dim3(GN_THREADS), 0, (hipStream_t)stream, ws,   \
                      splits, sstride, HW, C, groups, eps, bias, rowbias, rowbias_ld, (const bf16*)res, (bf16*)sum_out,        \
                      (const bf16*)x2, C2, gamma, beta, act, (bf16*)y, dq)
+#define ALDM_GNP(QPT) do { if (layout == ALDM_SLAB_PLANAR) ALDM_GNP2(QPT, true); else ALDM_GNP2(QPT, false); } while (0)
   if (nquads <= GN_THREADS) ALDM_GNP(1);
   else if (nquads <= 2 * GN_THREADS) ALDM_GNP(2);
   else if (nquads <= 4 * GN_THREADS) ALDM_GNP(4);
   else ALDM_GNP(8);
 #undef ALDM_GNP
+#undef ALDM_GNP2
   return aldm_launch_status("groupnorm_partials");
+}
+
+extern "C" int aldm_groupnorm_partials(const float* ws, int splits, int B, int HW, int C, const float* bias,
+                                       const float* rowbias, int rowbias_ld, const void* res, void* sum_out,
+                                       const void* x2, int C2, int groups, float eps, const float* gamma, const float* beta,
+                                       int act, void* y, void* stream) {
+  return aldm_groupnorm_partials_layout(ws, splits, B, HW, C, bias, rowbias, rowbias_ld, res, sum_out, x2, C2, groups, eps, gamma, beta,
+                                        act, y, ALDM_SLAB_ROWMAJOR, stream);
 }
 
 extern "C" int aldm_layernorm(const void* x, int M, int C, const float* gamma, const float* beta, float eps, void* y,
diff --git a/audioldm_with_lora_amd/ops.py b/audioldm_with_lora_amd/ops.py
--- a/audioldm_with_lora_amd/ops.py
+++ b/audioldm_with_lora_amd/ops.py
@@ -267,12 +267,14 @@
                     cands += [(t, rg, sp) for sp in (2, 3, 4, 5, 6, 8, 10) for rg in (3, 4)
                               if sp <= nch and base * sp <= 2560 and sp * M * pw.N * 4 <= (1 << 28)]
         max_sp = max(c[2] for c in cands)
+        defer_flags = (_lib.DEFER_ROWMAJOR | (_lib.DEFER_PLANAR if SLAB_LAYOUT == _lib.SLAB_PLANAR else 0)
+                       | (_lib.DEFER_WRITE_THROUGH if SLAB_WT else 0))
         ws = _workspace(max_sp * M * pw.N * 4, device) if max_sp > 1 else None
         results = []
         for t, rg, sp in cands:
             a.tile, a.ring, a.splits = t, rg, sp
             a.workspace = ws.data_ptr() if sp > 1 else None
-            a.defer_reduce = 1 if (sp > 1 and key.endswith(" gn")) else 0
+            a.defer_reduce = defer_flags if (sp > 1 and key.endswith(" gn")) else 0
             if lib.aldm_igemm(C.byref(a), _stream()) != 0:
                 continue
             e0, e1 = torch.cuda.Event(enable_timing=True), torch.cuda.Event(enable_timing=True)
@@ -398,14 +400,19 @@
 XCD_MAP = int(os.environ.get("ALDM_XCD_MAP", "0"))
 
 
+SLAB_LAYOUT = _lib.SLAB_ROWMAJOR if os.environ.get("ALDM_NO_SLAB_PLANAR") == "1" else _lib.SLAB_PLANAR
+SLAB_WT = os.environ.get("ALDM_NO_SLAB_WT") != "1"
+
+
 class Deferred:
-    __slots__ = ("out", "ws", "eff", "bias", "rowbias", "rowbias_ld", "res", "keep")
-
-    def __init__(self, out, ws, eff, bias, rowbias, rowbias_ld, res, keep):
+    __slots__ = ("out", "ws", "eff", "bias", "rowbias", "rowbias_ld", "res", "keep", "layout")
+
+    def __init__(self, out, ws, eff, bias, rowbias, rowbias_ld, res, keep, layout=_lib.SLAB_ROWMAJOR):
         global DEFERRED_COUNT
         DEFERRED_COUNT += 1
         self.out, self.ws, self.eff, self.bias, self.rowbias, self.rowbias_ld, self.res = out, ws, eff, bias, rowbias, rowbias_ld, res
         self.keep = keep
+        self.layout = layout
 
     @property
     def shape(self):
@@ -452,7 +459,7 @@
          out_slope=0.0, res=None, res2=None, alpha=1.0, post_act=ACT_NONE, post_slope=0.0, out2=None, out=None, out_f32=False, out_ld=None, out_batch_stride=None,
          out_pix_stride=1, out_pix_offset=0, vt=None, vt_col0=0, vt_ld=0, vt_batch_stride=0, lora_t_out=None,
          splits=None, tile=0, ring=0, gn=None, gn_keep=False, defer=False, rowstats=False, ln_parts=None, x3=None, x4=None,
-         vt_dual=False, qstats=False, gn_in=None, lora_gate=None):
+         vt_dual=False, qstats=False, gn_in=None, lora_gate=None, slab_layout=None, slab_wt=None):
     _require_gpu(x)
     if _pending_get(x) is not None:
         raise _lib.AldmError("conv: a deferred split-K reduce is pending on this stream -- its consumer groupnorm() must be the next launch")
@@ -644,7 +651,11 @@
     a.xcd_map = XCD_MAP
     lib = _lib.load()
     eff = lib.aldm_igemm_effective_splits(C.byref(a)) if (gn_defer and splits > 1) else 1
-    a.defer_reduce = 1 if eff > 1 else 0
+    layout = _lib.SLAB_ROWMAJOR
+    if eff > 1:
+        layout = slab_layout if slab_layout is not None else (SLAB_LAYOUT if gn is not None else _lib.SLAB_ROWMAJOR)
+    a.defer_reduce = ((_lib.DEFER_ROWMAJOR | (_lib.DEFER_PLANAR if layout == _lib.SLAB_PLANAR else 0)
+                       | (_lib.DEFER_WRITE_THROUGH if (SLAB_WT if slab_wt is None else slab_wt) else 0)) if eff > 1 else 0)
     ktot = KH * KW * pw.Cin + pw.Cext
     flops = 2.0 * M * pw.N * ktot + (2.0 * M * pw.Rp * (ktot + pw.N) if pw.Rp else 0.0)
     nbytes = 2.0 * (B * IH * IW * pw.Cin + M * pw.Cext + pw.N * ktot + M * ncols)
@@ -659,7 +670,7 @@
     def finish():
         if gn is None:
             if eff > 1:
-                d = Deferred(out, a.workspace, eff, a.bias, a.rowbias, a.rowbias_ld, a.res, (pw, rowbias, res, x3, x4))
+                d = Deferred(out, a.workspace, eff, a.bias, a.rowbias, a.rowbias_ld, a.res, (pw, rowbias, res, x3, x4), layout)
                 _pending_set(out, d)
                 return d
             return (out, stats) if rowstats else out
@@ -669,9 +680,9 @@
             return (out, y) if gn_keep else y
         y = torch.empty(B, OH, OW, pw.N, dtype=torch.bfloat16, device=x.device)
         n = M * pw.N
-        check(_launch(f"groupnorm_partials|HW{OH * OW} C{pw.N} S{eff}", 10.0 * n, (4.0 * eff + 2.0) * n, lambda: lib.aldm_groupnorm_partials(
+        check(_launch(f"groupnorm_partials|HW{OH * OW} C{pw.N} S{eff}", 10.0 * n, (4.0 * eff + 2.0) * n, lambda: lib.aldm_groupnorm_partials_layout(
             a.workspace, eff, B, OH * OW, pw.N, a.bias, a.rowbias, a.rowbias_ld, a.res, (a.out if gn_keep else None), None, 0,
-            groups, eps, _p(gamma), _p(beta), act, _p(y), _stream())), "aldm_groupnorm_partials")
+            groups, eps, _p(gamma), _p(beta), act, _p(y), layout, _stream())), "aldm_groupnorm_partials")
         return (out, y) if gn_keep else y
 
     if tuning and TUNER.slot is not None:
@@ -792,9 +803,9 @@
         y = torch.empty(B, H, W, C1 + C2, dtype=torch.bfloat16, device=x.out.device)
         lib = _lib.load()
         n = B * H * W * (C1 + C2)
-        check(_launch(f"groupnorm_partials|HW{H * W} C{C1}+{C2} S{x.eff}", 10.0 * n, (4.0 * x.eff + 2.0) * n, lambda: lib.aldm_groupnorm_partials(
+        check(_launch(f"groupnorm_partials|HW{H * W} C{C1}+{C2} S{x.eff}", 10.0 * n, (4.0 * x.eff + 2.0) * n, lambda: lib.aldm_groupnorm_partials_layout(
             x.ws, x.eff, B, H * W, C1, x.bias, x.rowbias, x.rowbias_ld, x.res, _p(x.out), _p(x2), C2, groups, eps,
-            _p(gamma), _p(beta), act, _p(y), _stream())), "aldm_groupnorm_partials")
+            _p(gamma), _p(beta), act, _p(y), x.layout, _stream())), "aldm_groupnorm_partials")
         _pending_set(x.out, None)
         return y
     _require_gpu(x)
@@ -1322,6 +1333,8 @@
     if isinstance(dy, Deferred):
         if dy is not _pending_get(dy.out) or dy.bias is not None or dy.rowbias is not None or dy.res is not None:
             raise _lib.AldmError("groupnorm_bwd: deferred dY must be the pending split-K launch, without bias / residual")
+        if dy.layout != _lib.SLAB_ROWMAJOR:
+            raise _lib.AldmError("groupnorm_bwd: deferred dY must be left in row-major slabs (conv(..., slab_layout=_lib.SLAB_ROWMAJOR))")
         assert tuple(dy.out.shape) == (B, H, W, C1 + C2)
         check(_lib.load().aldm_groupnorm_bwd_partials(_p(x), _p(x2), dy.ws, dy.eff, B, H * W, C1, C2, groups, eps, _p(gamma), _p(beta),
                                                       act, _p(dx), _p(dx2), _p(a1), _p(a2), _stream()), "aldm_groupnorm_bwd_partials")
diff --git a/audioldm_with_lora_amd/unet.py b/audioldm_with_lora_amd/unet.py
--- a/audioldm_with_lora_amd/unet.py
+++ b/audioldm_with_lora_amd/unet.py
@@ -222,7 +222,7 @@
     if P.conv2s is not None and (x2 is None or x2.shape[3] % 64 == 0) and x.shape[3] % 64 == 0:
         if next_gn is not None:
             return ops.conv(h, P.conv2s, pad=(1, 1), x3=x, x4=x2, gn=next_gn, gn_keep=True, qstats=True)
-        return ops.conv(h, P.conv2s, pad=(1, 1), x3=x, x4=x2, defer=(defer or False), qstats=True)
+        return ops.conv(h, P.conv2s, pad=(1, 1), x3=x, x4=x2, defer=(defer or False), slab_layout=ops.SLAB_LAYOUT, qstats=True)
     if P.shortcut is not None:
         xs = ops.conv(x, P.shortcut, x2=x2)
     else:
@@ -231,7 +231,7 @@
     src, fold = (h1, dict(gn_in=gn2)) if h1 is not None else (h, {})
     if next_gn is not None:
         return ops.conv(src, P.conv2, pad=(1, 1), res=xs, gn=next_gn, gn_keep=True, qstats=True, **fold)
-    return ops.conv(src, P.conv2, pad=(1, 1), res=xs, defer=(defer or False), qstats=True, **fold)
+    return ops.conv(src, P.conv2, pad=(1, 1), res=xs, defer=(defer or False), slab_layout=ops.SLAB_LAYOUT, qstats=True, **fold)
 
 
 def run_attention(P, hn, h_res, B, N, fp8=False, ln_parts=None, rowstats=False):
@@ -276,9 +276,9 @@
         h, st = h
     g = ops.linear(h if f3 else ops.layernorm(h, *P.ln[2]), P.ff1, ln_parts=st)
     if P.ff2_proj is not None:
-        return ops.conv(g.view(B, H, W, 4 * C), P.ff2_proj, x2=h.view(B, H, W, C), res=x, defer=(defer or False), qstats=True)
+        return ops.conv(g.view(B, H, W, 4 * C), P.ff2_proj, x2=h.view(B, H, W, C), res=x, defer=(defer or False), slab_layout=ops.SLAB_LAYOUT, qstats=True)
     h = ops.linear(g, P.ff2, res=h)
-    return ops.conv(h.view(B, H, W, C), P.proj_out, res=x, defer=(defer or False), qstats=True)
+    return ops.conv(h.view(B, H, W, C), P.proj_out, res=x, defer=(defer or False), slab_layout=ops.SLAB_LAYOUT, qstats=True)
 
 
 class UNet2DConditionModel(AdapterRouting, nn.Module):
@@ -483,7 +483,7 @@
                     h = run_resnet(r, h, None, rowbias, ld, defer=nxt)
                 skips.append(ops.tensor_of(h))
             if blk.down is not None:
-                h = ops.conv(h, blk.down, stride=(2, 2), pad=(1, 1), defer=norm1_of(P.down[bi + 1].resnets[0]), qstats=True)
+                h = ops.conv(h, blk.down, stride=(2, 2), pad=(1, 1), defer=norm1_of(P.down[bi + 1].resnets[0]), slab_layout=ops.SLAB_LAYOUT, qstats=True)
                 skips.append(ops.tensor_of(h))
         h, hn = run_resnet(P.mid.resnets[0], h, None, rowbias, ld, next_gn=transformer_gn(P.mid.attns[0]))
         h = run_transformer(P.mid.attns[0], h, fp8, xn=hn, defer=norm1_of(P.mid.resnets[1]))
@@ -507,7 +507,7 @@
                     size = (skips[-1].shape[1], skips[-1].shape[2])
                 else:
                     size = (h.shape[1] * 2, h.shape[2] * 2)
-                h = ops.conv(h, blk.up, pad=(1, 1), up_size=size, defer=norm1_of(P.up[bi + 1].resnets[0]), qstats=True)
+                h = ops.conv(h, blk.up, pad=(1, 1), up_size=size, defer=norm1_of(P.up[bi + 1].resnets[0]), slab_layout=ops.SLAB_LAYOUT, qstats=True)
         if ops.gn_silu_conv_out_ok(h, P.conv_out, groups):
             return ops.gn_silu_conv_out(h, P.gn_out[0], P.gn_out[1], groups, eps, P.conv_out)
         h = ops.groupnorm(h, P.gn_out[0], P.gn_out[1], groups, eps, ACT_SILU)
diff --git a/include/aldm_hip.h b/include/aldm_hip.h
--- a/include/aldm_hip.h
+++ b/include/aldm_hip.h
@@ -70,9 +70,13 @@
        ALDM_TILE_64x128_WS = 13, ALDM_TILE_128x64_WS = 14 ,
        ALDM_TILE_64x128_W8 = 10, ALDM_TILE_128x64_W8 = 11  };
 
+enum { ALDM_DEFER_ROWMAJOR = 1, ALDM_DEFER_PLANAR = 2, ALDM_DEFER_WRITE_THROUGH = 4 };
+enum { ALDM_SLAB_ROWMAJOR = 0, ALDM_SLAB_PLANAR = 1 };
+
 int aldm_igemm(const aldm_igemm_t* p, void* stream);
 size_t aldm_igemm_workspace_bytes(const aldm_igemm_t* p);
 int aldm_igemm_effective_splits(const aldm_igemm_t* p);
+long long aldm_igemm_slab_offset(int layout, int B, int HW, int C, int split, int m, int n);
 
 typedef struct {
   const void* x;
@@ -118,6 +122,9 @@
                             int rowbias_ld, const void* res, void* sum_out, const void* x2, int C2, int groups, float eps,
                             const float* gamma, const float* beta, int act, void* y,
                             void* stream);
+int aldm_groupnorm_partials_layout(const float* ws, int splits, int B, int HW, int C, const float* bias, const float* rowbias,
+                                   int rowbias_ld, const void* res, void* sum_out, const void* x2, int C2, int groups, float eps,
+                                   const float* gamma, const float* beta, int act, void* y, int layout, void* stream);
 int aldm_embed_layernorm(const long long* ids, int B, int L, int C, const float* word, int vocab, const float* pos,
                          int npos, const float* type0, const float* gamma, const float* beta, float eps, int pad_idx,
                          void* y, void* stream);
```

Measured after the change: 345.9 denoise_steps/s, median of 6. 1.9% higher.
